# biagiom/spark-network-traffic-classifier

Measured on NVIDIA H100. Metric: flow-records/sec fit+transform, higher is better.
Workload: dtype u8 bins / uint32 histograms / f64 split scoring (f32 records)

## Files before the change

include/b200flow.h:

```cpp
#ifndef B200FLOW_H
#define B200FLOW_H

#include <stdint.h>

#ifdef __cplusplus
extern "C" {
#endif

#define B200FLOW_OK            0
#define B200FLOW_ERR_ARG      -1
#define B200FLOW_ERR_CUDA     -2
#define B200FLOW_ERR_LIMIT    -3

#define B200FLOW_F32 0
#define B200FLOW_F64 1

#define B200FLOW_SRC_F32    0
#define B200FLOW_SRC_F64    1
#define B200FLOW_SRC_I32    2
#define B200FLOW_SRC_INDEX  3
#define B200FLOW_SRC_ONEHOT 4

typedef struct b200flow_slot {
    int32_t kind;
    int32_t src_off;
    int32_t lut_off;
    int32_t lut_len;
    int32_t hot;
    int32_t reserved;
    double  mean;
    double  scale;
} b200flow_slot;

const char* b200flow_last_error(void);
int  b200flow_version(void);

int b200flow_category_counts(const void* records, int64_t n_rows, int32_t row_bytes,
                             int32_t src_off, int32_t K, int64_t* counts, void* stream);

int b200flow_category_counts_multi(const void* records, int64_t n_rows, int32_t row_bytes, int32_t n_cols,
                                   const int32_t* src_offs_host, const int32_t* Ks_host, int64_t* counts, void* stream);

int b200flow_encode(const void* records, int64_t n_rows, int32_t row_bytes,
                    const b200flow_slot* plan, int32_t n_out,
                    const int32_t* lut, int32_t lut_total,
                    int32_t label_off, int32_t label_lut_off, int32_t label_lut_len,
                    int32_t check_nan,
                    void* out, int32_t out_dtype, int32_t* label_out, uint8_t* valid_out,
                    void* stream);

int b200flow_sample_records(const void* records, int64_t n_rows, int32_t row_bytes,
                            const b200flow_slot* plan, int32_t F, const int32_t* lut, int32_t round_f32,
                            uint64_t seed, uint64_t keep_threshold, int64_t row_offset,
                            double* sample, int64_t cap, int32_t* n_sampled, void* stream);

int b200flow_encode_bins(const void* records, int64_t n_rows, int32_t row_bytes,
                         const b200flow_slot* plan, int32_t F, const int32_t* lut, int32_t lut_total,
                         int32_t label_off, int32_t label_lut_off, int32_t label_lut_len,
                         int32_t check_nan, int32_t round_f32,
                         int32_t thr_f32 ,
                         const double* thresholds, const int32_t* n_thr, const int32_t* arity, int32_t max_bins,
                         uint8_t* tp, int32_t tp_stride, int32_t* label_out, int32_t* bad, void* stream);

int b200flow_column_moments(const void* x, int32_t dtype, int64_t n_rows, int32_t D, int64_t ld,
                            const double* shift, double* sum, double* sumsq, void* stream);

int b200flow_sample_rows(const void* x, int32_t dtype, int64_t n_rows, int32_t F, int64_t ld,
                         uint64_t seed, uint64_t keep_threshold, int64_t row_offset,
                         double* sample, int64_t cap, int32_t* n_sampled, void* stream);

int b200flow_find_splits(double* sample, int64_t cap, int32_t n_s, int32_t F,
                         const int32_t* arity, int32_t max_bins,
                         double* thresholds, int32_t* n_thr,
                         const int32_t* n_s_dev ,
                         void* stream);

int b200flow_bin_rows(const void* x, int32_t dtype, int64_t n_rows, int32_t F, int64_t ld,
                      const double* thresholds, const int32_t* n_thr, const int32_t* arity,
                      int32_t max_bins, const int32_t* labels,
                      uint8_t* tp, int32_t tp_stride, int32_t* bad_rows, void* stream);

int b200flow_dedup_rows(const uint8_t* tp, int64_t n_rows, int32_t tp_stride, int32_t key_bytes,
                        int32_t* table, int32_t* minrow, int64_t table_cap, int32_t* slot_of, int32_t* rep,
                        int32_t* flag, int64_t* pos, int64_t* n_unique, int32_t* uid, uint8_t* tp_unique, void* stream);

int b200flow_bag_weights(uint64_t seed, int32_t T, int64_t row_offset, int64_t n_rows,
                         const uint32_t* poisson_cdf, const uint32_t* poisson_cdf_host,
                         const int32_t* uid, const int32_t* perm, int64_t n_unique, uint32_t* W, void* stream);

int b200flow_group_rows(const int32_t* uid, int64_t n_rows, int64_t n_unique, int32_t* gsize, int64_t* goff,
                        int32_t* cursor, int32_t* perm, int32_t* uperm, void* stream);

int b200flow_bag_count(const uint32_t* W, int32_t T, int64_t n_unique, int32_t* blk_cnt, void* stream);

int b200flow_bag_fill(const uint32_t* W, int32_t T, int64_t n_unique, const int64_t* blk_off, void* ent, void* stream);

int b200flow_exclusive_scan_i32_to_i64(const int32_t* in, int64_t n, int64_t* out,
                                       int64_t* total, void* stream);


int b200flow_feature_subsets(uint64_t seed, int32_t n_slots, const int32_t* slot_tree,
                             const uint32_t* slot_nid, int32_t F, int32_t m,
                             uint16_t* subset, void* stream);

int b200flow_hist_level(const uint8_t* tp, int32_t tp_stride, int32_t F,
                        const void* ent,
                        int32_t n_slots, const int64_t* seg_begin, const int64_t* seg_end,
                        const int64_t* chunk_off, int64_t n_chunks, int32_t chunk_rows,
                        const uint16_t* subset, int32_t m, int32_t n_bins, int32_t C,
                        uint32_t* hist, void* stream);

typedef struct b200flow_split {
    int32_t  feat;
    int32_t  kind;
    int32_t  bin_thr;
    int32_t  flags;
    double   gain;
    double   impurity;
    uint64_t mask[4];
} b200flow_split;

int b200flow_score_level(const uint32_t* hist, int32_t n_slots, const uint16_t* subset,
                         int32_t m, int32_t n_bins, int32_t C,
                         const int32_t* feat_bins, const int32_t* feat_kind,
                         int32_t level, int32_t max_depth, int32_t min_instances,
                         double min_info_gain,
                         b200flow_split* split, uint32_t* node_counts,
                         uint32_t* left_counts, uint32_t* right_counts, void* stream);

typedef struct b200flow_node {
    int32_t feat;
    int32_t kind_bin;
    int32_t left;
    uint32_t nid;
} b200flow_node;

int b200flow_grow_level(int32_t n_slots, const int32_t* slot_tree, const uint32_t* slot_nid,
                        const int32_t* slot_node, const b200flow_split* split,
                        const uint32_t* node_counts, const uint32_t* left_counts,
                        const uint32_t* right_counts, int32_t C,
                        b200flow_node* nodes, uint64_t* node_mask, uint32_t* pool_counts,
                        int32_t* node_tree, int64_t pool_capacity,
                        int32_t* next_tree, uint32_t* next_nid, int32_t* next_node,
                        int32_t* next_parent, int32_t* child_slot, int64_t* counters, void* stream);

int b200flow_partition_level(const uint8_t* tp, int32_t tp_stride,
                             const void* ent, void* ent_out,
                             int32_t n_slots, const int64_t* seg_begin, const int64_t* seg_end,
                             const int64_t* chunk_off, int64_t n_chunks, int32_t chunk_rows,
                             const b200flow_split* split, int32_t* cursors, void* stream);

int b200flow_route_hist_config(int32_t F, int32_t m, int32_t n_bins, int32_t C,
                               int32_t rec_bytes , int32_t* chunk_rows, int32_t* m_pass);
int b200flow_route_hist_level(const uint8_t* tp, int32_t tp_stride, int32_t F,
                              const int32_t* field_desc ,
                              const void* ent, void* ent_out,
                              int32_t n_slots, const int64_t* seg_begin, const int64_t* seg_end,
                              const int64_t* chunk_off, const int64_t* n_chunks_dev ,
                              int64_t n_chunks_max ,
                              int32_t chunk_rows,
                              const b200flow_split* split, const int32_t* child_slot, int32_t* cursors,
                              void* chunk_scratch ,
                              const uint16_t* subset_next, int32_t m, int32_t n_bins, int32_t C,
                              uint32_t* hist_next, int32_t flags, void* stream);

int b200flow_packed_layout(int32_t F, const int32_t* feat_bins, int32_t C, int32_t* desc, int32_t* rec_bytes);
int b200flow_pack_records(const uint8_t* tp, int32_t tp_stride, int64_t n_rows, int32_t F, const int32_t* desc,
                          int32_t rec_bytes, uint32_t* packed, void* stream);

int b200flow_plan_route(int32_t n_slots, const b200flow_split* split, const int64_t* seg_begin, const int64_t* seg_end,
                        int32_t chunk_rows, const int32_t* slot_node, double* node_gain, int32_t* n_chunks,
                        int32_t* cursors , void* stream);

int b200flow_next_segments(int32_t n_next , const int64_t* n_next_dev ,
                           const int32_t* next_parent,
                           const int64_t* seg_begin, const int64_t* seg_end,
                           const int32_t* cursors, int64_t* next_begin, int64_t* next_end,
                           void* stream);

int b200flow_finalize_forest(int64_t n_nodes, const uint32_t* pool_counts, int32_t C,
                             double* leaf_prob, void* stream);

int b200flow_predict(const uint8_t* tp, int32_t tp_stride, int64_t n_rows,
                     const b200flow_node* nodes, const uint64_t* node_mask,
                     const double* leaf_prob, const uint32_t* pool_counts,
                     int32_t T, int32_t C, int32_t dt_mode,
                     const void* top_nodes , int32_t top_levels,
                     double* raw, double* prob, double* pred, void* stream);

int b200flow_build_top_nodes(const b200flow_node* nodes, const int32_t* node_tree, int64_t n_nodes, int32_t T,
                             int32_t top_levels, void* top, void* stream);

int b200flow_gather_rows(const void* src, int32_t row_bytes, const int32_t* idx, int64_t n_rows, void* out, void* stream);

int b200flow_confusion(const double* pred, const double* label, int64_t n_rows, int32_t C,
                       int64_t* cm, void* stream);

int b200flow_predict_grid_confusion(const uint8_t* tp, int32_t tp_stride, int32_t F, int64_t n_rows, const int32_t* mult,
                                    const b200flow_node* nodes, const uint64_t* node_mask, const double* leaf_prob,
                                    const uint32_t* pool_counts, int32_t T, int32_t C, int32_t dt_mode,
                                    const void* top_nodes, int32_t top_levels, const int32_t* tree_cuts_host,
                                    int32_t n_tree_cuts, const int32_t* depth_cuts_host, int32_t n_depth_cuts,
                                    int32_t cm_side, int32_t max_depth_cuts_per_launch, int64_t* cm, void* stream);
int b200flow_predict_grid_scores(const uint8_t* tp, int32_t tp_stride, int32_t F, int64_t n_rows,
                                 const b200flow_node* nodes, const uint64_t* node_mask, const double* leaf_prob,
                                 const uint32_t* pool_counts, int32_t T, int32_t C, int32_t dt_mode,
                                 const void* top_nodes, int32_t top_levels, const int32_t* tree_cuts_host,
                                 int32_t n_tree_cuts, const int32_t* depth_cuts_host, int32_t n_depth_cuts,
                                 int32_t max_depth_cuts_per_launch, double* scores, void* stream);

int b200flow_binary_counts_scratch(int32_t S, int64_t n, int64_t* scratch_bytes);
int b200flow_binary_counts(const double* scores, int64_t score_stride, const int32_t* pos, const int32_t* neg,
                           int64_t count_stride, int32_t S, int64_t n, void* scratch, int64_t scratch_bytes,
                           double* d_score, int64_t* d_pos, int64_t* d_neg, int64_t cap, int64_t* n_distinct,
                           int64_t* n_nan, void* stream);
int b200flow_binary_curve(const double* d_score, const int64_t* d_pos, const int64_t* d_neg, int64_t cap,
                          const int64_t* n_distinct, int32_t S, int32_t num_bins, double* auc, double* c_score,
                          int64_t* c_tp, int64_t* c_fp, int64_t* c_n, double* work, void* stream);

int b200flow_kmeans_assign(const double* x, int64_t n_rows, int32_t D, int64_t ld, const double* centers, int32_t k,
                           int32_t* cluster, double* dist, void* stream);
int b200flow_group_sums_chunks(int64_t row_offset, int64_t n_rows, int64_t* n_chunks);
int b200flow_group_sums(const double* values, int64_t ld, const int32_t* ids, int64_t n_rows, int32_t W, int32_t G,
                        int64_t row_offset, double* partials, int64_t* counts, void* stream);
int b200flow_group_sums_chain(const double* partials, int64_t n_chunks, int32_t G, int32_t W, double* totals, void* stream);
int b200flow_kmeans_row_keys(uint64_t seed, int64_t row_offset, int64_t n_rows, int64_t* keys, void* stream);
int b200flow_kmeans_select(uint64_t seed, int64_t row_offset, int64_t n_rows, int32_t step, const double* cost, int32_t k,
                           double sum_cost, uint8_t* flag, void* stream);
int b200flow_silhouette_rows(const double* x, int64_t n_rows, int32_t D, int64_t ld, const double* norms, const int32_t* cluster,
                             const double* Y, const double* psi, const int64_t* N, int32_t G, double* out, void* stream);

int b200flow_mlp_config(const int32_t* layers, int32_t n_layers, int64_t* n_params, int64_t* smem_bytes);
int b200flow_mlp_loss_grad(const void* x, int32_t x_dtype, int64_t n_rows, int64_t ld, const int32_t* labels,
                           const int32_t* layers, int32_t n_layers, const double* weights, int64_t row_offset,
                           double* partials, void* stream);
int b200flow_mlp_forward(const void* x, int32_t x_dtype, int64_t n_rows, int64_t ld, const int32_t* layers, int32_t n_layers,
                         const double* weights, double* raw, void* stream);

int b200flow_random_split(uint64_t seed, int64_t row_offset, int64_t n_rows,
                          const double* cum_bounds_host, int32_t n_splits, uint8_t* split_id,
                          void* stream);

int b200flow_compact_rows(const void* rows, int64_t n_rows, int32_t row_bytes,
                          const uint8_t* flag, int32_t want, void* out_rows,
                          int64_t* scratch, int64_t* n_kept, void* stream);

#define B200FLOW_CSV_NULL   0
#define B200FLOW_CSV_INT32  1
#define B200FLOW_CSV_INT64  2
#define B200FLOW_CSV_DOUBLE 3
#define B200FLOW_CSV_STRING 4
typedef struct b200flow_csv_col {
    int32_t type;
    int32_t rec_off;
    int32_t str_index;
    int32_t reserved;
} b200flow_csv_col;

int b200flow_csv_count_lines(const uint8_t* text, int64_t n_bytes, int32_t* counts, unsigned long long* flags, void* stream);
int b200flow_csv_line_starts(const uint8_t* text, int64_t n_bytes, const int64_t* bases, int64_t* row_starts, void* stream);
int b200flow_csv_infer(const uint8_t* text, int64_t n_bytes, const int64_t* row_starts, int64_t n_rows, int32_t n_cols,
                       int32_t flags, int32_t* col_class, int32_t* col_null, unsigned long long* bad, void* stream);
int b200flow_csv_dictionary(const uint8_t* text, int64_t n_bytes, const int64_t* row_starts, int64_t n_rows, int32_t n_cols,
                            int32_t flags, const b200flow_csv_col* cols, unsigned long long* keys, long long* pos_len,
                            int32_t cap_log2, unsigned long long* bad, void* stream);
int b200flow_csv_parse(const uint8_t* text, int64_t n_bytes, const int64_t* row_starts, int64_t n_rows, int32_t n_cols,
                       int32_t flags, const b200flow_csv_col* cols, const unsigned long long* keys, const long long* pos_len,
                       const int32_t* slot_code, int32_t cap_log2, void* records, int32_t row_bytes, unsigned long long* bad,
                       void* stream);

#ifdef __cplusplus
}
#endif
#endif
```

spark-network-traffic-classifier_b200/b200flow/_lib.py:

```python
import ctypes as C
import os

import numpy as np
import torch

_HERE = os.path.dirname(os.path.abspath(__file__))
LIB_PATH = os.path.join(_HERE, "libb200flow.so")

F32, F64 = 0, 1
SRC_F32, SRC_F64, SRC_I32, SRC_INDEX, SRC_ONEHOT = 0, 1, 2, 3, 4

SLOT_DTYPE = np.dtype([("kind", "<i4"), ("src_off", "<i4"), ("lut_off", "<i4"), ("lut_len", "<i4"),
                       ("hot", "<i4"), ("reserved", "<i4"), ("mean", "<f8"), ("scale", "<f8")])
SPLIT_DTYPE = np.dtype([("feat", "<i4"), ("kind", "<i4"), ("bin_thr", "<i4"), ("flags", "<i4"),
                        ("gain", "<f8"), ("impurity", "<f8"), ("mask", "<u8", (4,))])
NODE_DTYPE = np.dtype([("feat", "<i4"), ("kind_bin", "<i4"), ("left", "<i4"), ("nid", "<u4")])
assert SLOT_DTYPE.itemsize == 40 and SPLIT_DTYPE.itemsize == 64 and NODE_DTYPE.itemsize == 16


class B200FlowError(RuntimeError):
    pass


class UnsupportedParamError(B200FlowError, ValueError):
    """a parameter value MLlib accepts but the CUDA path does not implement (entropy impurity, maxBins > 256, ...): a
    ValueError, so the pyspark shim reports it as IllegalArgumentException; CUDA/runtime failures stay B200FlowError."""


_P, _I32, _I64, _U64, _F64 = C.c_void_p, C.c_int32, C.c_int64, C.c_uint64, C.c_double

_SIGNATURES = {
    "b200flow_category_counts": [_P, _I64, _I32, _I32, _I32, _P, _P],
    "b200flow_category_counts_multi": [_P, _I64, _I32, _I32, _P, _P, _P, _P],
    "b200flow_encode": [_P, _I64, _I32, _P, _I32, _P, _I32, _I32, _I32, _I32, _I32, _P, _I32, _P, _P, _P],
    "b200flow_sample_records": [_P, _I64, _I32, _P, _I32, _P, _I32, _U64, _U64, _I64, _P, _I64, _P, _P],
    "b200flow_encode_bins": [_P, _I64, _I32, _P, _I32, _P, _I32, _I32, _I32, _I32, _I32, _I32, _I32, _P, _P, _P, _I32, _P, _I32, _P, _P, _P],
    "b200flow_column_moments": [_P, _I32, _I64, _I32, _I64, _P, _P, _P, _P],
    "b200flow_sample_rows": [_P, _I32, _I64, _I32, _I64, _U64, _U64, _I64, _P, _I64, _P, _P],
    "b200flow_find_splits": [_P, _I64, _I32, _I32, _P, _I32, _P, _P, _P, _P],
    "b200flow_bin_rows": [_P, _I32, _I64, _I32, _I64, _P, _P, _P, _I32, _P, _P, _I32, _P, _P],
    "b200flow_dedup_rows": [_P, _I64, _I32, _I32, _P, _P, _I64, _P, _P, _P, _P, _P, _P, _P, _P],
    "b200flow_bag_weights": [_U64, _I32, _I64, _I64, _P, _P, _P, _P, _I64, _P, _P],
    "b200flow_group_rows": [_P, _I64, _I64, _P, _P, _P, _P, _P, _P],
    "b200flow_bag_count": [_P, _I32, _I64, _P, _P],
    "b200flow_bag_fill": [_P, _I32, _I64, _P, _P, _P],
    "b200flow_exclusive_scan_i32_to_i64": [_P, _I64, _P, _P, _P],
    "b200flow_feature_subsets": [_U64, _I32, _P, _P, _I32, _I32, _P, _P],
    "b200flow_hist_level": [_P, _I32, _I32, _P, _I32, _P, _P, _P, _I64, _I32, _P, _I32, _I32, _I32, _P, _P],
    "b200flow_score_level": [_P, _I32, _P, _I32, _I32, _I32, _P, _P, _I32, _I32, _I32, _F64, _P, _P, _P, _P, _P],
    "b200flow_grow_level": [_I32, _P, _P, _P, _P, _P, _P, _P, _I32, _P, _P, _P, _P, _I64, _P, _P, _P, _P, _P, _P, _P],
    "b200flow_route_hist_level": [_P, _I32, _I32, _P, _P, _P, _I32, _P, _P, _P, _P, _I64, _I32, _P, _P, _P, _P, _P, _I32, _I32,
                                  _I32, _P, _I32, _P],
    "b200flow_pack_records": [_P, _I32, _I64, _I32, _P, _I32, _P, _P],
    "b200flow_partition_level": [_P, _I32, _P, _P, _I32, _P, _P, _P, _I64, _I32, _P, _P, _P],
    "b200flow_plan_route": [_I32, _P, _P, _P, _I32, _P, _P, _P, _P, _P],
    "b200flow_next_segments": [_I32, _P, _P, _P, _P, _P, _P, _P, _P],
    "b200flow_finalize_forest": [_I64, _P, _I32, _P, _P],
    "b200flow_predict": [_P, _I32, _I64, _P, _P, _P, _P, _I32, _I32, _I32, _P, _I32, _P, _P, _P, _P],
    "b200flow_build_top_nodes": [_P, _P, _I64, _I32, _I32, _P, _P],
    "b200flow_gather_rows": [_P, _I32, _P, _I64, _P, _P],
    "b200flow_confusion": [_P, _P, _I64, _I32, _P, _P],
    "b200flow_predict_grid_confusion": [_P, _I32, _I32, _I64, _P, _P, _P, _P, _P, _I32, _I32, _I32, _P, _I32, _P, _I32, _P, _I32,
                                        _I32, _I32, _P, _P],
    "b200flow_predict_grid_scores": [_P, _I32, _I32, _I64, _P, _P, _P, _P, _I32, _I32, _I32, _P, _I32, _P, _I32, _P, _I32, _I32,
                                     _P],
    "b200flow_binary_counts": [_P, _I64, _P, _P, _I64, _I32, _I64, _P, _I64, _P, _P, _P, _I64, _P, _P, _P],
    "b200flow_binary_curve": [_P, _P, _P, _I64, _P, _I32, _I32, _P, _P, _P, _P, _P, _P, _P],
    "b200flow_kmeans_assign": [_P, _I64, _I32, _I64, _P, _I32, _P, _P, _P],
    "b200flow_group_sums": [_P, _I64, _P, _I64, _I32, _I32, _I64, _P, _P, _P],
    "b200flow_group_sums_chain": [_P, _I64, _I32, _I32, _P, _P],
    "b200flow_kmeans_row_keys": [_U64, _I64, _I64, _P, _P],
    "b200flow_kmeans_select": [_U64, _I64, _I64, _I32, _P, _I32, _F64, _P, _P],
    "b200flow_silhouette_rows": [_P, _I64, _I32, _I64, _P, _P, _P, _P, _P, _I32, _P, _P],
    "b200flow_mlp_loss_grad": [_P, _I32, _I64, _I64, _P, _P, _I32, _P, _I64, _P, _P],
    "b200flow_mlp_forward": [_P, _I32, _I64, _I64, _P, _I32, _P, _P, _P],
    "b200flow_random_split": [_U64, _I64, _I64, _P, _I32, _P, _P],
    "b200flow_compact_rows": [_P, _I64, _I32, _P, _I32, _P, _P, _P, _P],
    "b200flow_csv_count_lines": [_P, _I64, _P, _P, _P],
    "b200flow_csv_line_starts": [_P, _I64, _P, _P, _P],
    "b200flow_csv_infer": [_P, _I64, _P, _I64, _I32, _I32, _P, _P, _P, _P],
    "b200flow_csv_dictionary": [_P, _I64, _P, _I64, _I32, _I32, _P, _P, _P, _I32, _P, _P],
    "b200flow_csv_parse": [_P, _I64, _P, _I64, _I32, _I32, _P, _P, _P, _P, _I32, _P, _I32, _P, _P],
}
EXPORTS = sorted(list(_SIGNATURES) + ["b200flow_last_error", "b200flow_version", "b200flow_route_hist_config",
                                       "b200flow_packed_layout", "b200flow_binary_counts_scratch",
                                       "b200flow_group_sums_chunks", "b200flow_mlp_config"])

_lib = None
launches = 0
_KERNELS_PER_CALL = {"b200flow_grow_level": 3, "b200flow_compact_rows": 3, "b200flow_route_hist_level": 2, "b200flow_dedup_rows": 5, "b200flow_group_rows": 3}


def load():
    global _lib
    if _lib is None:
        if not os.path.exists(LIB_PATH):
            raise B200FlowError("libb200flow.so is not built (%s missing): run `python -c 'import __graft_entry__ as g; "
                                "g.build()'` or `make -C spark-network-traffic-classifier_b200/csrc`. There is no CPU "
                                "fallback for the product path." % LIB_PATH)
        lib = C.CDLL(LIB_PATH)
        for name, args in _SIGNATURES.items():
            fn = getattr(lib, name)
            fn.argtypes = args
            fn.restype = C.c_int
        lib.b200flow_last_error.restype = C.c_char_p
        lib.b200flow_version.restype = C.c_int
        lib.b200flow_route_hist_config.argtypes = [_I32] * 5 + [C.POINTER(_I32), C.POINTER(_I32)]
        lib.b200flow_route_hist_config.restype = C.c_int
        lib.b200flow_packed_layout.argtypes = [_I32, _P, _I32, _P, C.POINTER(_I32)]
        lib.b200flow_packed_layout.restype = C.c_int
        lib.b200flow_binary_counts_scratch.argtypes = [_I32, _I64, C.POINTER(_I64)]
        lib.b200flow_binary_counts_scratch.restype = C.c_int
        lib.b200flow_group_sums_chunks.argtypes = [_I64, _I64, C.POINTER(_I64)]
        lib.b200flow_group_sums_chunks.restype = C.c_int
        lib.b200flow_mlp_config.argtypes = [_P, _I32, C.POINTER(_I64), C.POINTER(_I64)]
        lib.b200flow_mlp_config.restype = C.c_int
        _lib = lib
    return _lib


def route_hist_config(F, m, n_bins, n_classes, rec_bytes=0):
    ch, mp = _I32(0), _I32(0)
    ok = load().b200flow_route_hist_config(int(F), int(m), int(n_bins), int(n_classes), int(rec_bytes), C.byref(ch), C.byref(mp))
    return (int(ch.value), int(mp.value)) if ok else None


def packed_layout(feat_bins, n_classes):
    fb = np.ascontiguousarray(feat_bins, dtype=np.int32)
    desc = np.zeros(fb.shape[0] + 1, np.int32)
    rb = _I32(0)
    lib = load()
    if lib.b200flow_packed_layout(int(fb.shape[0]), fb.ctypes.data, int(n_classes), desc.ctypes.data, C.byref(rb)) != 0:
        raise B200FlowError("b200flow_packed_layout failed: %s" % lib.b200flow_last_error().decode())
    return desc, int(rb.value)


def binary_counts_scratch(S, n):
    out = _I64(0)
    lib = load()
    if lib.b200flow_binary_counts_scratch(int(S), int(n), C.byref(out)) != 0:
        raise B200FlowError("b200flow_binary_counts_scratch failed: %s" % lib.b200flow_last_error().decode())
    return int(out.value)


def group_sums_chunks(row_offset, n_rows):
    out = _I64(0)
    lib = load()
    if lib.b200flow_group_sums_chunks(int(row_offset), int(n_rows), C.byref(out)) != 0:
        raise B200FlowError("b200flow_group_sums_chunks failed: %s" % lib.b200flow_last_error().decode())
    return int(out.value)


def mlp_config(layers):
    la = np.ascontiguousarray(layers, dtype=np.int32)
    P, sm = _I64(0), _I64(0)
    lib = load()
    if lib.b200flow_mlp_config(la.ctypes.data, int(la.shape[0]), C.byref(P), C.byref(sm)) != 0:
        raise UnsupportedParamError("layers %s: %s" % (list(map(int, la)), lib.b200flow_last_error().decode()))
    return int(P.value), int(sm.value)


def ptr(t):
    if t is None:
        return None
    if not t.is_cuda:
        raise B200FlowError("b200flow kernels need CUDA tensors (got %s); there is no CPU fallback" % t.device)
    if not t.is_contiguous():
        raise B200FlowError("b200flow kernels need contiguous tensors")
    return t.data_ptr()


def stream():
    return torch.cuda.current_stream().cuda_stream


def call(name, *args):
    global launches
    lib = load()
    rc = getattr(lib, name)(*args, stream())
    launches += _KERNELS_PER_CALL.get(name, 1)
    if rc != 0:
        raise B200FlowError("%s failed (%d): %s" % (name, rc, lib.b200flow_last_error().decode()))


def h2d(a, device):
    t = torch.from_numpy(np.ascontiguousarray(a))
    if torch.device(device).type != "cuda":
        return t.clone()
    return t.pin_memory().to(device, non_blocking=True)


def require_cuda():
    if not torch.cuda.is_available():
        raise B200FlowError("no CUDA device: the b200flow product path has no CPU fallback")
    load()


def dtype_code(t):
    if t.dtype == torch.float32:
        return F32
    if t.dtype == torch.float64:
        return F64
    raise B200FlowError("dense matrices must be float32 or float64, got %s" % t.dtype)
```

spark-network-traffic-classifier_b200/b200flow/forest.py:

```python
import math
from dataclasses import dataclass

import numpy as np
import torch

from . import _lib
from ._lib import NODE_DTYPE, SPLIT_DTYPE, B200FlowError, UnsupportedParamError, call, ptr

import os as _os
CHUNK_ROWS = 2048
FUSED = True
TOP_LEVELS = int(_os.environ.get("B200FLOW_TOP_LEVELS", "8"))
DEDUP = True
_PIN = True
PROFILE = None


def _timed(name, fn, *args):
    if PROFILE is None:
        return call(fn, *args)
    e0, e1 = torch.cuda.Event(enable_timing=True), torch.cuda.Event(enable_timing=True)
    e0.record()
    call(fn, *args)
    e1.record()
    PROFILE.setdefault(name, []).append((e0, e1))


def profile_totals():
    torch.cuda.synchronize()
    return {k: (len(v), sum(a.elapsed_time(b) for a, b in v)) for k, v in (PROFILE or {}).items()
            if not k.startswith("_")}


ENTRY_BOUND_BYTES = 8 << 30
HIST_BUDGET_BYTES = int(_os.environ.get("B200FLOW_HIST_BUDGET_GB", "10")) << 30
RS_MIN_BYTES = int(_os.environ.get("B200FLOW_RS_MIN_BYTES", str(8 << 20)))
RS_CHUNKS = int(_os.environ.get("B200FLOW_RS_CHUNKS", "1"))


@dataclass
class ForestParams:
    num_trees: int = 20
    max_depth: int = 5
    max_bins: int = 32
    min_instances_per_node: int = 1
    min_info_gain: float = 0.0
    feature_subset_strategy: str = "auto"
    subsampling_rate: float = 1.0
    impurity: str = "gini"
    seed: int = 0
    bootstrap: bool = True


def tp_stride(F):
    return (F + 1 + 63) // 64 * 64


def poisson_cdf_table(rate=1.0):
    out = np.empty(32, np.uint32)
    term = math.exp(-rate); cdf = 0.0
    for k in range(32):
        cdf += term
        out[k] = min(int(math.floor(cdf * 4294967296.0)), 0xFFFFFFFF)
        term = term * rate / (k + 1)
    if out[30] != 0xFFFFFFFF:
        raise UnsupportedParamError("subsamplingRate %.3f too large: bag weights must stay below 31" % rate)
    return out


def build_metadata(n_rows, F, num_classes, arity, max_bins, num_trees, strategy="auto"):
    arity = np.asarray(arity, np.int32)
    mpb = int(min(max_bins, n_rows))
    if mpb > 256:
        raise UnsupportedParamError("maxBins > 256 is not supported (bins are stored as uint8)")
    if arity.size and int(arity.max()) > mpb:
        raise ValueError("DecisionTree requires maxBins (= %d) to be at least as large as the number of values in each "
                         "categorical feature, but a categorical feature has %d values. Consider removing this and other "
                         "categorical features with a large number of values, or add more training examples."
                         % (mpb, int(arity.max())))
    if arity.size and int(arity.max()) > 255:
        raise UnsupportedParamError("a categorical feature with %d categories is not supported: bins are stored as uint8, and "
                                    "with 256 categories no bin is left for a value unseen at fit time (at most 255)"
                                    % int(arity.max()))
    kind = np.zeros(F, np.int32)
    U = int(math.floor(math.log(mpb // 2 + 1) / math.log(2.0) + 1)) if num_classes > 2 else 0
    for f in range(F):
        if arity[f] > 1:
            kind[f] = 2 if (num_classes > 2 and arity[f] <= U) else 1
        elif arity[f] == 1:
            kind[f] = 1
    s = str(strategy)
    if s == "auto":
        s = "all" if num_trees == 1 else "sqrt"
    if s == "all": m = F
    elif s == "sqrt": m = int(math.ceil(math.sqrt(F)))
    elif s == "log2": m = max(1, int(math.ceil(math.log(F) / math.log(2))))
    elif s == "onethird": m = int(math.ceil(F / 3.0))
    else:
        try:
            v = float(s)
        except ValueError:
            raise ValueError("Supported featureSubsetStrategy values: auto, all, onethird, sqrt, log2, (0.0-1.0], [1-n]; got %r" % strategy)
        m = int(v) if ("." not in s and v >= 1) else int(math.ceil(v * F))
    return mpb, kind, max(1, min(m, F))


def pack_records(tp, F, field_desc, rec_bytes):
    packed = torch.empty((max(tp.shape[0], 1), rec_bytes), dtype=torch.uint8, device=tp.device)
    call("b200flow_pack_records", ptr(tp), tp.shape[1], tp.shape[0], F, ptr(field_desc), rec_bytes, ptr(packed))
    return packed


def dedup_rows(tp, key_bytes, sync=True):
    n, stride = tp.shape
    dev = tp.device
    cap_tab = 1
    while cap_tab < 2 * n:
        cap_tab <<= 1
    table = torch.empty(cap_tab, dtype=torch.int32, device=dev); minrow = torch.empty(cap_tab, dtype=torch.int32, device=dev)
    slot_of = torch.empty(n, dtype=torch.int32, device=dev); rep = torch.empty(n, dtype=torch.int32, device=dev)
    flag = torch.empty(n, dtype=torch.int32, device=dev); pos = torch.empty(n + 1, dtype=torch.int64, device=dev)
    uid = torch.empty(n, dtype=torch.int32, device=dev); total = torch.zeros(1, dtype=torch.int64, device=dev)
    tpu = torch.empty_like(tp)
    _timed("dedup_rows", "b200flow_dedup_rows", ptr(tp), n, stride, key_bytes, ptr(table), ptr(minrow), cap_tab, ptr(slot_of), ptr(rep),
           ptr(flag), ptr(pos), ptr(total), ptr(uid), ptr(tpu))
    if not sync:
        return tpu, uid, total
    U = int(total.item())
    return tpu[:U], uid, U


def _i32(a, dev):
    return _lib.h2d(np.ascontiguousarray(a, np.int32), dev)


class InvalidRowsError(ValueError):
    """NaN / null numeric cells or unseen dictionary codes met while assembling rows (VectorAssembler / StringIndexerModel
    handleInvalid="error"); raised when the fused record path meets them — Spark raises at the same point: the action."""


class _DenseSource:

    def __init__(self, x, labels=None):
        self.x, self.labels = x, (labels.to(torch.int32).contiguous() if labels is not None else None)
        self.n, self.F = x.shape
        self.device = x.device

    def sample(self, seed, keep, row_offset, sample, cap, n_s_dev):
        call("b200flow_sample_rows", ptr(self.x), _lib.dtype_code(self.x), self.n, self.F, self.x.stride(0), seed, keep, int(row_offset),
             ptr(sample), cap, ptr(n_s_dev))

    def bin(self, thresholds, n_thr, arity_dev, mpb, bad, want_label_out=False):
        stride = tp_stride(self.F)
        tp = torch.empty((self.n, stride), dtype=torch.uint8, device=self.device)
        _timed("bin_rows", "b200flow_bin_rows", ptr(self.x), _lib.dtype_code(self.x), self.n, self.F, self.x.stride(0), ptr(thresholds), ptr(n_thr),
               ptr(arity_dev), mpb, ptr(self.labels), ptr(tp), stride, ptr(bad[0:1]))
        return tp, self.labels


class _RecordSource:

    def __init__(self, rec, plan, round_f32=False, with_label=True):
        if rec.dtype != torch.uint8 or rec.dim() != 2 or rec.shape[1] != plan.schema.row_bytes:
            raise ValueError("records must be uint8 [n, %d]" % plan.schema.row_bytes)
        self.rec, self.plan, self.round_f32 = rec, plan, 1 if round_f32 else 0
        self.n, self.F = rec.shape[0], plan.n_out
        self.device = rec.device
        self.with_label = with_label and plan.label is not None

    def _thr_f32(self, arity_dev):
        if self.round_f32:
            return 1
        return 1 if all(s[0] in (_lib.SRC_F32, _lib.SRC_INDEX, _lib.SRC_ONEHOT) and s[5] == 0.0 and s[6] == 1.0 for s in self.plan.slots) else 0

    def sample(self, seed, keep, row_offset, sample, cap, n_s_dev):
        _, slots, lut_t, _ = self.plan._device_tables(self.device)
        call("b200flow_sample_records", ptr(self.rec), self.n, self.plan.schema.row_bytes, ptr(slots), self.F, ptr(lut_t), self.round_f32,
             seed, keep, int(row_offset), ptr(sample), cap, ptr(n_s_dev))

    def bin(self, thresholds, n_thr, arity_dev, mpb, bad, want_label_out=False):
        _, slots, lut_t, lut_total = self.plan._device_tables(self.device)
        stride = tp_stride(self.F)
        tp = torch.empty((self.n, stride), dtype=torch.uint8, device=self.device)
        loff, llo, lln = self.plan.label if self.with_label else (-1, 0, 0)
        lab = torch.empty(self.n, dtype=torch.int32, device=self.device) if (want_label_out and self.with_label) else None
        _timed("encode_bins", "b200flow_encode_bins", ptr(self.rec), self.n, self.plan.schema.row_bytes, ptr(slots), self.F, ptr(lut_t), lut_total,
               loff, llo, lln, int(self.plan.check_nan), self.round_f32, self._thr_f32(arity_dev), ptr(thresholds), ptr(n_thr), ptr(arity_dev), mpb, ptr(tp), stride,
               ptr(lab), ptr(bad))
        return tp, lab


class ForestModel:

    def __init__(self, T, C, F, arity, max_bins, thresholds, n_thr, nodes, node_mask, pool_counts, node_tree,
                 leaf_prob, node_gain, n_nodes, dt_mode):
        self.T, self.C, self.F, self.max_bins, self.dt_mode = T, C, F, max_bins, dt_mode
        self.arity = np.asarray(arity, np.int32)
        self.thresholds, self.n_thr = thresholds, n_thr
        self.nodes, self.node_mask, self.pool_counts = nodes, node_mask, pool_counts
        self.node_tree, self.leaf_prob, self.node_gain, self.n_nodes = node_tree, leaf_prob, node_gain, n_nodes
        self._arity_dev = _i32(self.arity, thresholds.device)

    def bin(self, x, labels=None):
        n, F = x.shape
        if F != self.F:
            raise ValueError("expected %d features, got %d" % (self.F, F))
        bad = torch.zeros(2, dtype=torch.int32, device=x.device)
        tp, _ = _DenseSource(x, labels).bin(self.thresholds, self.n_thr, self._arity_dev, self.max_bins, bad)
        return tp, bad[0:1]

    def _top_table(self):
        if TOP_LEVELS <= 0:
            return None, 0
        if getattr(self, "_top", None) is None:
            self._top = torch.zeros((self.T << TOP_LEVELS, 4), dtype=torch.int32, device=self.nodes.device)
            call("b200flow_build_top_nodes", ptr(self.nodes), ptr(self.node_tree), self.n_nodes, self.T, TOP_LEVELS, ptr(self._top))
        return self._top, TOP_LEVELS

    def predict_binned(self, tp, want_raw=True, want_prob=True):
        n = tp.shape[0]
        dev = tp.device
        raw = torch.empty((n, self.C), dtype=torch.float64, device=dev) if want_raw else None
        prob = torch.empty((n, self.C), dtype=torch.float64, device=dev) if want_prob else None
        pred = torch.empty(n, dtype=torch.float64, device=dev)
        top, K = self._top_table()
        _timed("predict", "b200flow_predict", ptr(tp), tp.shape[1], n, ptr(self.nodes), ptr(self.node_mask), ptr(self.leaf_prob),
             ptr(self.pool_counts), self.T, self.C, 1 if self.dt_mode else 0, ptr(top), K, ptr(raw), ptr(prob), ptr(pred))
        return raw, prob, pred

    def predict(self, x, want_raw=True, want_prob=True):
        tp, _ = self.bin(x)
        return self._predict_tp(tp, want_raw, want_prob)

    def predict_records(self, rec, plan, want_raw=True, want_prob=True, round_f32=False, want_label=False, on_invalid="ignore"):
        src = _RecordSource(rec, plan, round_f32, with_label=want_label)
        if src.F != self.F:
            raise ValueError("expected %d features, got %d" % (self.F, src.F))
        bad = torch.zeros(2, dtype=torch.int32, device=rec.device)
        tp, lab = src.bin(self.thresholds, self.n_thr, self._arity_dev, self.max_bins, bad, want_label_out=want_label)
        out = self._predict_tp(tp, want_raw, want_prob, bad if on_invalid == "error" else None)
        return out + (lab,)

    def _predict_tp(self, tp, want_raw=True, want_prob=True, bad=None):
        n = tp.shape[0]
        if not DEDUP or n == 0:
            if bad is not None and int(bad[1].item()):
                raise InvalidRowsError("%d NaN/null cells or unseen labels in the rows to transform" % int(bad[1].item()))
            return self.predict_binned(tp, want_raw, want_prob)
        tpu, uid, u_dev = dedup_rows(tp, self.F, sync=False)
        head = (torch.cat([u_dev, bad.to(torch.int64)]) if bad is not None else u_dev).cpu()
        if bad is not None and int(head[2]):
            raise InvalidRowsError("%d NaN/null cells or unseen labels in the rows to transform" % int(head[2]))
        U = int(head[0])
        raw_u, prob_u, pred_u = self.predict_binned(tpu[:U], want_raw, want_prob)

        def spread(src, width):
            if src is None:
                return None
            out = torch.empty((n, width) if width > 1 else (n,), dtype=torch.float64, device=tp.device)
            call("b200flow_gather_rows", ptr(src), 8 * width, ptr(uid), n, ptr(out))
            return out
        return spread(raw_u, self.C), spread(prob_u, self.C), spread(pred_u, 1)

    def grid_confusion(self, x_or_records, tree_cuts, depth_cuts, labels=None, plan=None, round_f32=False, cm_side=None,
                       group=None, max_depth_cuts_per_launch=0):
        from . import dist as bdist
        tree_cuts = np.ascontiguousarray(sorted(set(int(t) for t in tree_cuts)), np.int32)
        depth_cuts = np.ascontiguousarray(sorted(set(int(d) for d in depth_cuts)), np.int32)
        if plan is None:
            if labels is None:
                raise ValueError("grid_confusion: the dense path needs the labels")
            src = _DenseSource(x_or_records, labels)
        else:
            if plan.label is None:
                raise ValueError("grid_confusion: the encode plan has no label column (EncodePlan.set_label)")
            src = _RecordSource(x_or_records, plan, round_f32)
        if src.F != self.F:
            raise ValueError("expected %d features, got %d" % (self.F, src.F))
        S = max(self.C, int(cm_side or 0))
        dev = src.device
        cm = torch.zeros((len(tree_cuts), len(depth_cuts), S, S), dtype=torch.int64, device=dev)
        n = src.n
        if n > 0:
            bad = torch.zeros(2, dtype=torch.int32, device=dev)
            tp, _ = src.bin(self.thresholds, self.n_thr, self._arity_dev, self.max_bins, bad)
            tpu, uid, U = dedup_rows(tp, self.F + 1)
            gsize = torch.empty(U, dtype=torch.int32, device=dev); cursor = torch.empty(U, dtype=torch.int32, device=dev)
            goff = torch.empty(U + 1, dtype=torch.int64, device=dev)
            perm = torch.empty(n, dtype=torch.int32, device=dev); uperm = torch.empty(n, dtype=torch.int32, device=dev)
            _timed("group_rows", "b200flow_group_rows", ptr(uid), n, U, ptr(gsize), ptr(goff), ptr(cursor), ptr(perm), ptr(uperm))
            top, K = self._top_table()
            _timed("predict_grid", "b200flow_predict_grid_confusion", ptr(tpu), tpu.shape[1], self.F, U, ptr(gsize), ptr(self.nodes),
                   ptr(self.node_mask), ptr(self.leaf_prob), ptr(self.pool_counts), self.T, self.C, 1 if self.dt_mode else 0,
                   ptr(top), K, tree_cuts.ctypes.data, len(tree_cuts), depth_cuts.ctypes.data, len(depth_cuts), S,
                   int(max_depth_cuts_per_launch), ptr(cm))
        return bdist.all_reduce_sum_(cm, group).cpu()

    GRID_SCORE_BUDGET = 2 << 30

    def grid_binary_metrics(self, x_or_records, tree_cuts, depth_cuts, labels=None, plan=None, num_bins=1000, group=None,
                            round_f32=False, max_depth_cuts_per_launch=0):
        from . import dist as bdist
        from .metrics import binary_metrics
        if self.C < 2:
            raise ValueError("grid_binary_metrics: the score is rawPrediction[1], the forest has %d class(es)" % self.C)
        tree_cuts = np.ascontiguousarray(sorted(set(int(t) for t in tree_cuts)), np.int32)
        depth_cuts = np.ascontiguousarray(sorted(set(int(d) for d in depth_cuts)), np.int32)
        if plan is None:
            if labels is None:
                raise ValueError("grid_binary_metrics: the dense path needs the labels")
            src = _DenseSource(x_or_records, labels)
        else:
            if plan.label is None:
                raise ValueError("grid_binary_metrics: the encode plan has no label column (EncodePlan.set_label)")
            src = _RecordSource(x_or_records, plan, round_f32)
        if src.F != self.F:
            raise ValueError("expected %d features, got %d" % (self.F, src.F))
        dev = src.device
        I, J = len(tree_cuts), len(depth_cuts)
        U = 0
        if src.n > 0:
            bad = torch.zeros(2, dtype=torch.int32, device=dev)
            tp, _ = src.bin(self.thresholds, self.n_thr, self._arity_dev, self.max_bins, bad)
            tpu, uid, U = dedup_rows(tp, self.F + 1)
            tpu = tpu.contiguous()
            gsize = torch.empty(U, dtype=torch.int32, device=dev); cursor = torch.empty(U, dtype=torch.int32, device=dev)
            goff = torch.empty(U + 1, dtype=torch.int64, device=dev)
            perm = torch.empty(src.n, dtype=torch.int32, device=dev); uperm = torch.empty(src.n, dtype=torch.int32, device=dev)
            _timed("group_rows", "b200flow_group_rows", ptr(uid), src.n, U, ptr(gsize), ptr(goff), ptr(cursor), ptr(perm), ptr(uperm))
            positive = tpu[:, self.F] >= 1
            pos = torch.where(positive, gsize, 0).contiguous()
            neg = torch.where(positive, 0, gsize).contiguous()
        else:
            pos = neg = torch.zeros(0, dtype=torch.int32, device=dev)
        mx = torch.tensor([U], dtype=torch.int64, device=dev)
        grp = group if group is not None else bdist.group()
        if grp is not None:
            import torch.distributed as dist
            bdist.all_reduce_(mx, grp, op=dist.ReduceOp.MAX)
        per_cut = J * max(int(mx.item()), 1) * 8
        step = max(1, min(I, self.GRID_SCORE_BUDGET // per_cut))
        out = np.empty((I, J, 2), np.float64)
        top, K = self._top_table()
        for i0 in range(0, I, step):
            cuts = np.ascontiguousarray(tree_cuts[i0:i0 + step])
            scores = torch.empty((len(cuts), J, U), dtype=torch.float64, device=dev)
            if U > 0:
                _timed("predict_grid", "b200flow_predict_grid_scores", ptr(tpu), tpu.shape[1], self.F, U, ptr(self.nodes),
                       ptr(self.node_mask), ptr(self.leaf_prob), ptr(self.pool_counts), self.T, self.C, 1 if self.dt_mode else 0,
                       ptr(top), K, cuts.ctypes.data, len(cuts), depth_cuts.ctypes.data, J, int(max_depth_cuts_per_launch),
                       ptr(scores))
            r = binary_metrics(scores.reshape(len(cuts) * J, U), pos=pos, neg=neg, num_bins=num_bins, group=grp)
            out[i0:i0 + len(cuts), :, 0] = np.asarray(r["areaUnderROC"]).reshape(len(cuts), J)
            out[i0:i0 + len(cuts), :, 1] = np.asarray(r["areaUnderPR"]).reshape(len(cuts), J)
        return out

    def export(self):
        n = self.n_nodes
        nodes = self.nodes[:n].cpu().numpy().view(NODE_DTYPE).reshape(-1)
        tree = self.node_tree[:n].cpu().numpy()
        counts = self.pool_counts[:n].cpu().numpy().view(np.uint32).astype(np.int64)
        mask = (self.node_mask[:n].cpu().numpy().view(np.uint64) if self.node_mask is not None
                else np.zeros((n, 4), np.uint64))
        gain = self.node_gain[:n].cpu().numpy()
        order = np.lexsort((nodes["nid"], tree))
        is_leaf = (nodes["feat"] < 0).astype(np.int32)
        kind = np.where(is_leaf == 1, 0, nodes["kind_bin"] >> 16).astype(np.int32)
        bin_thr = np.where(is_leaf == 1, 0, nodes["kind_bin"] & 0xffff).astype(np.int32)
        mask = np.where(is_leaf[:, None] == 1, 0, mask).astype(np.uint64)
        return dict(tree=tree[order], nid=nodes["nid"][order], feat=nodes["feat"][order], kind=kind[order],
                    bin_thr=bin_thr[order], is_leaf=is_leaf[order], gain=gain[order], mask=mask[order],
                    counts=counts[order])

    def feature_importances(self):
        ex = self.export()
        imp = np.zeros(self.F)
        for t in range(self.T):
            sel = (ex["tree"] == t) & (ex["is_leaf"] == 0)
            v = np.zeros(self.F)
            np.add.at(v, ex["feat"][sel], ex["gain"][sel] * ex["counts"][sel].sum(1))
            if v.sum() > 0:
                imp += v / v.sum()
        return imp / imp.sum() if imp.sum() > 0 else imp


def _gather_sample(sample, n_s, cap, F, group):
    import torch.distributed as dist
    world = dist.get_world_size(group)
    from . import dist as bdist
    counts = [int(c.item()) for c in bdist.all_gather_list(torch.tensor([n_s], dtype=torch.int64, device=sample.device), group)]
    mx = max(max(counts), 1)
    mine = torch.zeros((F, mx), dtype=torch.float64, device=sample.device)
    if n_s > 0:
        mine[:, :n_s] = sample.view(F, cap)[:, :n_s]
    parts = bdist.all_gather_list(mine, group)
    tot = sum(counts)
    new_cap = 1
    while new_cap < max(tot, 2):
        new_cap <<= 1
    out = torch.empty((F, new_cap), dtype=torch.float64, device=sample.device)
    pos = 0
    for p, c in zip(parts, counts):
        out[:, pos:pos + c] = p[:, :c]; pos += c
    return out.view(-1), tot, new_cap


def fit_forest(x, labels, num_classes, arity, params, row_offset=0, group=None):
    return _fit(_DenseSource(x, labels), num_classes, arity, params, row_offset, group)


def fit_forest_records(rec, plan, num_classes, arity, params, row_offset=0, group=None, round_f32=False):
    if plan.label is None:
        raise ValueError("fit_forest_records: the encode plan has no label column (EncodePlan.set_label)")
    return _fit(_RecordSource(rec, plan, round_f32), num_classes, arity, params, row_offset, group)


def _fit(src, num_classes, arity, params, row_offset=0, group=None):
    import torch.distributed as dist
    from . import dist as bdist
    _lib.require_cuda()
    p = params
    if p.impurity != "gini":
        raise UnsupportedParamError("impurity=%r: only 'gini' is implemented on the CUDA path" % p.impurity)
    if not (0 <= p.max_depth <= 30):
        raise ValueError("maxDepth must be in [0, 30], got %d" % p.max_depth)
    dev = src.device
    n, F = src.n, src.F
    C = int(num_classes)
    if not (1 <= C <= 256):
        raise ValueError("numClasses must be in [1, 256] (labels are stored as one byte), got %d" % C)
    T = int(p.num_trees)
    seed = int(p.seed) & 0xFFFFFFFFFFFFFFFF
    n_global = n
    if group is not None:
        t = torch.tensor([n], dtype=torch.int64, device=dev)
        bdist.all_reduce_(t, group)
        n_global = int(t.item())
    mpb, kind, m = build_metadata(n_global, F, C, arity, p.max_bins, T, p.feature_subset_strategy)
    arity = np.asarray(arity, np.int32)
    arity_dev = _i32(arity, dev)

    has_cont = bool((arity == 0).any())
    frac = min(1.0, max(mpb * mpb, 10000) / float(max(n_global, 1))) if has_cont else 1.0
    keep = int(frac * 4294967296.0)
    expect = n if frac >= 1.0 else int(n * frac + 6.0 * math.sqrt(max(n * frac, 1.0)) + 64)
    cap = 1
    while cap < max(min(expect, n), 2):
        cap <<= 1
    sample = torch.empty(F * cap, dtype=torch.float64, device=dev)
    n_s_dev = torch.zeros(1, dtype=torch.int32, device=dev)
    thresholds = torch.zeros((F, mpb - 1), dtype=torch.float64, device=dev)
    n_thr = torch.zeros(F, dtype=torch.int32, device=dev)
    if has_cont:
        src.sample(seed, keep, row_offset, sample, cap, n_s_dev)
        if group is not None:
            n_s = int(n_s_dev.item())
            if n_s > cap:
                raise B200FlowError("findSplits sample overflow (%d > %d)" % (n_s, cap))
            sample, n_s, cap = _gather_sample(sample, n_s, cap, F, group)
            call("b200flow_find_splits", ptr(sample), cap, n_s, F, ptr(arity_dev), mpb, ptr(thresholds), ptr(n_thr), None)
        else:
            call("b200flow_find_splits", ptr(sample), cap, cap, F, ptr(arity_dev), mpb, ptr(thresholds), ptr(n_thr), ptr(n_s_dev))
    del sample

    stride = tp_stride(F)
    bad = torch.zeros(2, dtype=torch.int32, device=dev)
    tp, _ = src.bin(thresholds, n_thr, arity_dev, mpb, bad)
    feat_bins = torch.where(arity_dev > 0, arity_dev, n_thr + 1).to(torch.int32).contiguous()
    feat_kind = _i32(kind, dev)
    total = torch.zeros(1, dtype=torch.int64, device=dev)
    dedup = n > 0 and DEDUP
    if dedup:
        tp, uid, u_dev = dedup_rows(tp, F + 1, sync=False)
    else:
        uid, u_dev = None, torch.full((1,), n, dtype=torch.int64, device=dev)
    bagging = p.bootstrap and T > 1
    cdf_host = np.ascontiguousarray(poisson_cdf_table(p.subsampling_rate)) if bagging else None
    cdf = _lib.h2d(cdf_host.view(np.int32), dev) if bagging else None
    cap_nodes = max(4096, 4 * T, min(T << (min(p.max_depth, 18) + 1), 1 << 20))
    nodes = torch.zeros((cap_nodes, 16), dtype=torch.uint8, device=dev)
    use_mask = bool((kind > 0).any())
    node_mask = torch.zeros((cap_nodes, 4), dtype=torch.int64, device=dev) if use_mask else None
    pool_counts = torch.zeros((cap_nodes, C), dtype=torch.int32, device=dev)
    node_tree = torch.zeros(cap_nodes, dtype=torch.int32, device=dev)
    node_gain = torch.zeros(cap_nodes, dtype=torch.float64, device=dev)
    root = np.zeros(T, NODE_DTYPE); root["feat"] = -1; root["left"] = -1; root["nid"] = 1
    nodes[:T] = _lib.h2d(root.view(np.uint8).reshape(T, 16), dev)
    node_tree[:T] = torch.arange(T, dtype=torch.int32, device=dev)
    pool_size = T

    def grow_pool(need):
        nonlocal nodes, node_mask, pool_counts, node_tree, node_gain, cap_nodes
        if need <= cap_nodes:
            return
        new_cap = cap_nodes
        while new_cap < need:
            new_cap *= 2
        def ext(t, shape_tail):
            nt = torch.zeros((new_cap,) + shape_tail, dtype=t.dtype, device=dev)
            nt[:cap_nodes] = t
            return nt
        nodes = ext(nodes, (16,)); pool_counts = ext(pool_counts, (C,)); node_tree = ext(node_tree, ())
        node_gain = ext(node_gain, ())
        if node_mask is not None:
            node_mask = ext(node_mask, (4,))
        cap_nodes = new_cap

    head = torch.cat([bad.to(torch.int64), feat_bins.max().reshape(1).to(torch.int64), n_s_dev.to(torch.int64), u_dev,
                      feat_bins.to(torch.int64)]).cpu()
    if int(head[1]) != 0:
        raise InvalidRowsError("%d NaN/null cells or unseen labels in the training rows" % int(head[1]))
    if int(head[0]) != 0:
        raise ValueError("categorical feature value outside [0, arity) or non-integral in %d cells" % int(head[0]))
    if has_cont and group is None and int(head[3]) > cap:
        raise B200FlowError("findSplits sample overflow (%d > %d)" % (int(head[3]), cap))
    n_bins, U = int(head[2]), int(head[4])
    if dedup:
        tp = tp[:U]
    if tp.shape[0] == 0:
        tp = torch.zeros((1, stride), dtype=torch.uint8, device=dev)
    desc_host, rec_bytes = _lib.packed_layout(head[5:5 + F].numpy(), C) if FUSED else (None, 0)
    cfg = _lib.route_hist_config(F, m, n_bins, C, rec_bytes) if FUSED else None
    fused = cfg is not None
    route_ch, m_pass = cfg if fused else (CHUNK_ROWS, m)
    route_passes = -(-m // m_pass)
    hsz = m * n_bins * C
    rec_tp, rec_stride, field_desc = tp, stride, None
    if fused and rec_bytes:
        field_desc = _lib.h2d(desc_host, dev)
        rec_tp, rec_stride = pack_records(tp, F, field_desc, rec_bytes), rec_bytes
    nb = (U + 1023) // 1024
    W = torch.zeros(max(T * U, 1), dtype=torch.int32, device=dev)
    if n > 0:
        perm = uperm = None
        if uid is not None and bagging and U < n:
            gsize = torch.empty(U, dtype=torch.int32, device=dev); cursor = torch.empty(U, dtype=torch.int32, device=dev)
            goff = torch.empty(U + 1, dtype=torch.int64, device=dev)
            perm = torch.empty(n, dtype=torch.int32, device=dev); uperm = torch.empty(n, dtype=torch.int32, device=dev)
            _timed("group_rows", "b200flow_group_rows", ptr(uid), n, U, ptr(gsize), ptr(goff), ptr(cursor), ptr(perm), ptr(uperm))
        _timed("bag_weights", "b200flow_bag_weights", seed, T, int(row_offset), n, ptr(cdf),
               cdf_host.ctypes.data if bagging else None, ptr(uperm if perm is not None else uid), ptr(perm), U, ptr(W))
    blk_cnt = torch.zeros(max(T * nb, 1), dtype=torch.int32, device=dev)
    blk_off = torch.zeros(T * nb + 1, dtype=torch.int64, device=dev)
    if U > 0:
        call("b200flow_bag_count", ptr(W), T, U, ptr(blk_cnt))
    call("b200flow_exclusive_scan_i32_to_i64", ptr(blk_cnt), T * nb, ptr(blk_off), ptr(total))
    e_dev = total.clone()
    E = T * U if T * U * 16 <= ENTRY_BOUND_BYTES else int(total.item())
    ent = torch.empty((max(E, 1), 2), dtype=torch.int32, device=dev)
    ent2 = torch.empty_like(ent)
    if U > 0:
        call("b200flow_bag_fill", ptr(W), T, U, ptr(blk_off), ptr(ent))
    del W, uid

    slot_tree = torch.arange(T, dtype=torch.int32, device=dev)
    slot_nid = torch.ones(T, dtype=torch.int32, device=dev)
    slot_node = torch.arange(T, dtype=torch.int32, device=dev)
    idx = torch.arange(T, dtype=torch.int64, device=dev) * nb
    seg_begin = blk_off[idx].contiguous()
    seg_end = blk_off[idx + nb].contiguous()
    n_slots = T
    level = 0
    per_slot_hist = m * n_bins * C * 4
    group_slots = max(1, HIST_BUDGET_BYTES // per_slot_hist)
    stats = dict(levels=0, slots=0, entries=0, hist_launches=0, rows=n, unique_rows=U)

    stats["route_chunk"], stats["route_passes"] = route_ch if fused else 0, route_passes if fused else 0
    stats["record_format"], stats["record_bytes"] = ("packed", rec_bytes) if field_desc is not None else ("bytes", stride)

    def chunk_table(nch):
        off = torch.empty(nch.shape[0] + 1, dtype=torch.int64, device=dev)
        call("b200flow_exclusive_scan_i32_to_i64", ptr(nch), nch.shape[0], ptr(off), ptr(total))
        return off, int(total.item())

    def level_subsets(ns, s_tree, s_nid):
        sub = torch.empty((ns, m), dtype=torch.int16, device=dev)
        call("b200flow_feature_subsets", seed, ns, ptr(s_tree), ptr(s_nid), F, m, ptr(sub))
        return sub

    def plan_route(ns, split_, begin_, end_, total_out, s_node=None, gain_out=None, cursors_=None):
        nch = torch.empty(ns, dtype=torch.int32, device=dev)
        call("b200flow_plan_route", ns, ptr(split_), ptr(begin_), ptr(end_), route_ch, ptr(s_node), ptr(gain_out), ptr(nch), ptr(cursors_))
        roff = torch.empty(ns + 1, dtype=torch.int64, device=dev)
        call("b200flow_exclusive_scan_i32_to_i64", ptr(nch), ns, ptr(roff), ptr(total_out))
        if PROFILE is not None:
            PROFILE.setdefault("_route_entries", []).append(torch.where(nch > 0, end_ - begin_, torch.zeros_like(end_)).sum())
        return roff

    route_chunks_max = E // route_ch + 1

    world = dist.get_world_size(group) if group is not None else 1
    rank = dist.get_rank(group) if group is not None else 0
    REC = 64 + 12 * C
    use_rs = world > 1 and bdist.is_nccl(group)

    def score_sharded(h_full, gs, sub, lvl, split_, nc_, lc_, rc_):
        K = int(max(1, min(RS_CHUNKS, gs, (gs * hsz * 4) // max(RS_MIN_BYTES, 1))))
        bounds = [gs * i // K for i in range(K + 1)]
        ev0 = None
        if PROFILE is not None:
            ev0 = torch.cuda.Event(enable_timing=True); ev0.record()
        jobs = []
        for k in range(K):
            s0, g = bounds[k], bounds[k + 1] - bounds[k]
            per = -(-g // world)
            mine = torch.empty(per * hsz, dtype=torch.int32, device=dev)
            w = dist.reduce_scatter_tensor(mine, h_full[s0 * hsz:(s0 + world * per) * hsz], group=group, async_op=True)
            jobs.append((s0, g, per, mine, w))
        gathers = []
        for s0, g, per, mine, w in jobs:
            w.wait()
            lo = rank * per
            cnt = max(0, min(per, g - lo))
            local = torch.empty(per * REC, dtype=torch.uint8, device=dev)
            sec = [local[:per * 64], local[per * 64:per * (64 + 4 * C)], local[per * (64 + 4 * C):per * (64 + 8 * C)], local[per * (64 + 8 * C):]]
            if cnt > 0:
                _timed("score_level", "b200flow_score_level", ptr(mine), cnt, ptr(sub[s0 + lo:s0 + lo + cnt]), m, n_bins, C, ptr(feat_bins),
                       ptr(feat_kind), lvl, p.max_depth, int(p.min_instances_per_node), float(p.min_info_gain), ptr(sec[0]), ptr(sec[1]),
                       ptr(sec[2]), ptr(sec[3]))
            gathered = torch.empty((world, per * REC), dtype=torch.uint8, device=dev)
            gw = dist.all_gather_into_tensor(gathered, local, group=group, async_op=True)
            gathers.append((s0, per, gathered, gw))
        for s0, per, gathered, gw in gathers:
            gw.wait()
            o = 0
            for dst, width in ((split_, 64), (nc_.view(torch.uint8), 4 * C), (lc_.view(torch.uint8), 4 * C), (rc_.view(torch.uint8), 4 * C)):
                dst.view(-1)[s0 * width:(s0 + world * per) * width].view(world, per * width).copy_(gathered[:, o:o + per * width])
                o += per * width
        if ev0 is not None:
            ev1 = torch.cuda.Event(enable_timing=True); ev1.record()
            PROFILE.setdefault("level_exchange", []).append((ev0, ev1))

    def run_route(roff, rch_dev, n_parents, split_, child_slot_, cursors_, next_subset_, n_next_cap, route=True):
        hist_next = torch.zeros((n_next_cap + world - 1) * hsz, dtype=torch.int32, device=dev)
        cmax = route_chunks_max + n_parents
        scratch = torch.empty(cmax * 4, dtype=torch.int32, device=dev)
        _timed("route_hist_level", "b200flow_route_hist_level", ptr(rec_tp), rec_stride, F, ptr(field_desc), ptr(ent), ptr(ent2), n_parents,
               ptr(seg_begin), ptr(seg_end), ptr(roff), ptr(rch_dev), cmax, route_ch, ptr(split_), ptr(child_slot_), ptr(cursors_),
               ptr(scratch), ptr(next_subset_), m, n_bins, C, ptr(hist_next), 1 if route else 0)
        _lib.launches += route_passes - 1
        stats["hist_launches"] += route_passes
        return hist_next

    side_stream = torch.cuda.Stream(device=dev)
    host_cnt = torch.empty(5, dtype=torch.int64).pin_memory() if _PIN else None
    subset = level_subsets(n_slots, slot_tree, slot_nid)
    hist_ready = None
    counters = None
    if fused and n_slots * hsz * 4 <= HIST_BUDGET_BYTES:
        pseudo = np.zeros(T, SPLIT_DTYPE); pseudo["bin_thr"] = 255; pseudo["flags"] = 4
        pseudo_t = _lib.h2d(pseudo.view(np.uint8).reshape(T, 64), dev)
        child0 = torch.stack([torch.arange(T, dtype=torch.int32, device=dev),
                              torch.full((T,), -1, dtype=torch.int32, device=dev)], 1).contiguous().view(-1)
        cursors0 = torch.zeros(2 * T, dtype=torch.int32, device=dev)
        roff0 = plan_route(T, pseudo_t, seg_begin, seg_end, total)
        hist_full = run_route(roff0, total, T, pseudo_t, child0, cursors0, subset, T, route=False)
        hist_ready = hist_full[:T * hsz]
    while n_slots > 0:
        grow_pool(pool_size + 2 * n_slots)
        lens = (seg_end - seg_begin) if hist_ready is None else None
        n_alloc = n_slots + world - 1
        split = torch.empty((n_alloc, 64), dtype=torch.uint8, device=dev)
        node_counts = torch.empty((n_alloc, C), dtype=torch.int32, device=dev)
        left_counts = torch.empty((n_alloc, C), dtype=torch.int32, device=dev)
        right_counts = torch.empty((n_alloc, C), dtype=torch.int32, device=dev)
        chunk_off = None
        if hist_ready is None:
            nch = ((lens + (CHUNK_ROWS - 1)) // CHUNK_ROWS).to(torch.int32).contiguous()
            chunk_off, n_chunks = chunk_table(nch)
        groups = [(0, n_slots)] if hist_ready is not None else \
            [(g0, min(n_slots, g0 + group_slots)) for g0 in range(0, n_slots, group_slots)]
        for g0, g1 in groups:
            gs = g1 - g0
            if hist_ready is not None:
                h = hist_ready
            else:
                h = torch.zeros(gs * hsz, dtype=torch.int32, device=dev)
                if g0 == 0 and g1 == n_slots:
                    coff, gch = chunk_off, n_chunks
                else:
                    coff = (chunk_off[g0:g1 + 1] - chunk_off[g0]).contiguous()
                    gch = int((chunk_off[g1] - chunk_off[g0]).item())
                _timed("hist_level", "b200flow_hist_level", ptr(tp), stride, F, ptr(ent), gs,
                       ptr(seg_begin[g0:g1]), ptr(seg_end[g0:g1]), ptr(coff), gch, CHUNK_ROWS, ptr(subset[g0:g1]), m, n_bins, C, ptr(h))
                stats["hist_launches"] += 1
                if PROFILE is not None:
                    PROFILE.setdefault("_hist_entries", []).append(lens[g0:g1].sum())
            if use_rs and hist_ready is not None and gs * hsz * 4 >= RS_MIN_BYTES:
                score_sharded(hist_full, gs, subset, level, split, node_counts, left_counts, right_counts)
                del h
                continue
            if group is not None:
                if PROFILE is not None:
                    ev0 = torch.cuda.Event(enable_timing=True); ev0.record()
                bdist.all_reduce_(h, group)
                if PROFILE is not None:
                    ev1 = torch.cuda.Event(enable_timing=True); ev1.record()
                    PROFILE.setdefault("level_exchange", []).append((ev0, ev1))
            _timed("score_level", "b200flow_score_level", ptr(h), gs, ptr(subset[g0:g1]), m, n_bins, C, ptr(feat_bins), ptr(feat_kind),
                   level, p.max_depth, int(p.min_instances_per_node), float(p.min_info_gain), ptr(split[g0:g1]),
                   ptr(node_counts[g0:g1]), ptr(left_counts[g0:g1]), ptr(right_counts[g0:g1]))
            del h
        split, node_counts, left_counts, right_counts = split[:n_slots], node_counts[:n_slots], left_counts[:n_slots], right_counts[:n_slots]
        hist_ready = None
        nblk = (n_slots + 255) // 256
        if counters is None or counters.numel() < 8 + nblk + 1:
            fresh = torch.zeros(8 + 2 * nblk + 1024, dtype=torch.int64, device=dev)
            if counters is None:
                fresh[0:1].fill_(pool_size)
            else:
                fresh[:8] = counters[:8]
            counters = fresh
        next_tree = torch.empty(2 * n_slots, dtype=torch.int32, device=dev)
        next_nid = torch.empty(2 * n_slots, dtype=torch.int32, device=dev)
        next_node = torch.empty(2 * n_slots, dtype=torch.int32, device=dev)
        next_parent = torch.empty(2 * n_slots, dtype=torch.int32, device=dev)
        child_slot = torch.empty(2 * n_slots, dtype=torch.int32, device=dev)
        _timed("grow_level", "b200flow_grow_level", n_slots, ptr(slot_tree), ptr(slot_nid), ptr(slot_node), ptr(split), ptr(node_counts),
               ptr(left_counts), ptr(right_counts), C, ptr(nodes), ptr(node_mask), ptr(pool_counts), ptr(node_tree),
               cap_nodes, ptr(next_tree), ptr(next_nid), ptr(next_node), ptr(next_parent), ptr(child_slot), ptr(counters))
        n_cap = 2 * n_slots
        speculative = fused and n_cap * hsz * 4 <= HIST_BUDGET_BYTES and level + 1 < p.max_depth
        if not speculative:
            node_gain[slot_node.long()] = split.view(torch.float64)[:, 2]
        if speculative:
            cursors = torch.empty(2 * n_slots, dtype=torch.int32, device=dev)
            roff = plan_route(n_slots, split, seg_begin, seg_end, counters[4:5], slot_node, node_gain, cursors)
            ev_planned = torch.cuda.Event(); ev_planned.record()
            with torch.cuda.stream(side_stream):
                side_stream.wait_event(ev_planned)
                cnt = counters[:5].to("cpu", non_blocking=True) if host_cnt is None else host_cnt.copy_(counters[:5], non_blocking=True)
                ev_read = torch.cuda.Event(); ev_read.record(side_stream)
            next_subset = level_subsets(n_cap, next_tree, next_nid)
            hist_next = run_route(roff, counters[4:5], n_slots, split, child_slot, cursors, next_subset, n_cap,
                                  route=level + 2 < p.max_depth)
            next_begin = torch.empty(n_cap, dtype=torch.int64, device=dev)
            next_end = torch.empty(n_cap, dtype=torch.int64, device=dev)
            call("b200flow_next_segments", n_cap, ptr(counters[1:2]), ptr(next_parent), ptr(seg_begin), ptr(seg_end), ptr(cursors),
                 ptr(next_begin), ptr(next_end))
            ev_read.synchronize()
        else:
            cnt = counters[:5].cpu()
        if int(cnt[2]) != 0:
            raise B200FlowError("node pool overflow (capacity %d)" % cap_nodes)
        pool_size, n_next = int(cnt[0]), int(cnt[1])
        stats["levels"] += 1; stats["slots"] += n_slots
        if n_next == 0:
            break
        next_tree, next_nid, next_node = next_tree[:n_next], next_nid[:n_next], next_node[:n_next]
        if speculative:
            hist_ready = hist_next[:n_next * hsz]
            hist_full = hist_next
            next_subset, next_begin, next_end = next_subset[:n_next], next_begin[:n_next], next_end[:n_next]
        else:
            next_subset = level_subsets(n_next, next_tree, next_nid)
            cursors = torch.zeros(2 * n_slots, dtype=torch.int32, device=dev)
            if chunk_off is None:
                lens = seg_end - seg_begin
                nch = ((lens + (CHUNK_ROWS - 1)) // CHUNK_ROWS).to(torch.int32).contiguous()
                chunk_off, n_chunks = chunk_table(nch)
            _timed("partition_level", "b200flow_partition_level", ptr(tp), stride, ptr(ent), ptr(ent2),
                   n_slots, ptr(seg_begin), ptr(seg_end), ptr(chunk_off), n_chunks, CHUNK_ROWS, ptr(split), ptr(cursors))
            next_begin = torch.empty(n_next, dtype=torch.int64, device=dev)
            next_end = torch.empty(n_next, dtype=torch.int64, device=dev)
            call("b200flow_next_segments", n_next, None, ptr(next_parent), ptr(seg_begin), ptr(seg_end), ptr(cursors),
                 ptr(next_begin), ptr(next_end))
        ent, ent2 = ent2, ent
        slot_tree, slot_nid, slot_node, subset = next_tree, next_nid, next_node, next_subset
        seg_begin, seg_end = next_begin, next_end
        n_slots = n_next
        level += 1

    leaf_prob = torch.empty((pool_size, C), dtype=torch.float64, device=dev)
    call("b200flow_finalize_forest", pool_size, ptr(pool_counts), C, ptr(leaf_prob))
    stats["entries"] = int(e_dev.item())
    model = ForestModel(T, C, F, arity, mpb, thresholds, n_thr, nodes, node_mask, pool_counts, node_tree, leaf_prob,
                        node_gain, pool_size, dt_mode=(T == 1 and not p.bootstrap))
    model.train_stats = stats
    model.feat_kind, model.feat_bins, model.n_bins, model.m = kind, feat_bins, n_bins, m
    return model


def confusion_matrix(pred, label, C):
    cm = torch.zeros((C, C), dtype=torch.int64, device=pred.device)
    call("b200flow_confusion", ptr(pred.contiguous()), ptr(label.contiguous()), pred.shape[0], C, ptr(cm))
    return cm


def metrics_from_confusion(cm, metric_label=0.0, beta=1.0):
    cm = np.asarray(cm, np.float64)
    N = cm.sum()
    sup = cm.sum(1); predl = cm.sum(0); tp = np.diag(cm)
    labs = sup > 0
    with np.errstate(divide="ignore", invalid="ignore"):
        p = np.where(predl > 0, tp / predl, 0.0)
        r = np.where(sup > 0, tp / sup, 0.0)
        f1 = np.where(p + r > 0, 2 * p * r / (p + r), 0.0)
        b2 = beta * beta
        fb = np.where(p + r > 0, (1 + b2) * p * r / (b2 * p + r), 0.0)
        fpr = (predl - tp) / (N - sup)
    w = sup / N if N else sup
    out = dict(accuracy=float(tp[labs].sum() / N) if N else 0.0,
               weightedPrecision=float((p * w)[labs].sum()), weightedRecall=float((r * w)[labs].sum()),
               f1=float((f1 * w)[labs].sum()), macroF1=float(f1[labs].mean()) if labs.any() else 0.0)
    out.update(weightedTruePositiveRate=out["weightedRecall"], weightedFalsePositiveRate=float((fpr * w)[labs].sum()),
               weightedFMeasure=float((fb * w)[labs].sum()),
               hammingLoss=float((N - tp.sum()) / N) if N else 0.0)
    ml = float(metric_label)
    li = int(ml) if np.isfinite(ml) and ml == int(ml) else -1
    if 0 <= li < cm.shape[0] and labs[li]:
        out.update(truePositiveRateByLabel=float(r[li]), falsePositiveRateByLabel=float(fpr[li]), precisionByLabel=float(p[li]),
                   recallByLabel=float(r[li]), fMeasureByLabel=float(fb[li]))
    return out
```

spark-network-traffic-classifier_b200/csrc/forest.cu:

```cuda
#include <float.h>
#include <stdlib.h>
#include <string.h>

#include "common.cuh"

namespace b200flow {

constexpr int kMaxSubset = 128;

__global__ void __launch_bounds__(128) feature_subsets_kernel(uint64_t seed, int n_slots, const int32_t* __restrict__ slot_tree,
                                                              const uint32_t* __restrict__ slot_nid, int F, int m,
                                                              uint16_t* subset) {
    int s = blockIdx.x * blockDim.x + threadIdx.x;
    if (s >= n_slots) return;
    uint16_t* out = subset + (int64_t)s * m;
    if (m >= F) { for (int i = 0; i < F; ++i) out[i] = (uint16_t)i; return; }
    uint16_t pos[kMaxSubset], val[kMaxSubset], pick[kMaxSubset];
    int nt = 0;
    const int tree = slot_tree[s]; const uint32_t nid = slot_nid[s];
    uint4 r = make_uint4(0, 0, 0, 0);
    for (int i = 0; i < m; ++i) {
        if ((i & 3) == 0) r = philox_keyed(seed, PURPOSE_FEAT, (uint32_t)tree, nid, (uint32_t)(i >> 2), 0u);
        uint32_t w = (i & 3) == 0 ? r.x : (i & 3) == 1 ? r.y : (i & 3) == 2 ? r.z : r.w;
        int j = i + (int)(w % (uint32_t)(F - i));
        int vi = i, vj = j, ki = -1, kj = -1;
        for (int k = 0; k < nt; ++k) { if (pos[k] == i) { vi = val[k]; ki = k; } if (pos[k] == j) { vj = val[k]; kj = k; } }
        pick[i] = (uint16_t)vj;
        if (j != i) {
            if (kj >= 0) val[kj] = (uint16_t)vi; else { pos[nt] = (uint16_t)j; val[nt] = (uint16_t)vi; ++nt; }
        }
        (void)ki;
    }
    for (int i = 1; i < m; ++i) {
        uint16_t x = pick[i]; int k = i - 1;
        while (k >= 0 && pick[k] > x) { pick[k + 1] = pick[k]; --k; }
        pick[k + 1] = x;
    }
    for (int i = 0; i < m; ++i) out[i] = pick[i];
}

__device__ __forceinline__ int find_slot(const int64_t* __restrict__ chunk_off, int n_slots, int64_t c) {
    int lo = 0, hi = n_slots;
    while (hi - lo > 1) { int mid = (lo + hi) >> 1; if (__ldg(chunk_off + mid) <= c) lo = mid; else hi = mid; }
    return lo;
}

__global__ void __launch_bounds__(256) hist_level_kernel(const uint8_t* __restrict__ tp, int stride, int F,
                                                         const b2f_entry* __restrict__ ent, int n_slots, const int64_t* __restrict__ seg_begin,
                                                         const int64_t* __restrict__ seg_end, const int64_t* __restrict__ chunk_off,
                                                         int chunk_rows, const uint16_t* __restrict__ subset, int m, int n_bins,
                                                         int C, int m_pass, uint32_t* hist) {
    extern __shared__ uint32_t sh_hist[];
    __shared__ int sh_feat[256];
    const int64_t c = blockIdx.x;
    const int s = find_slot(chunk_off, n_slots, c);
    const int64_t b = seg_begin[s] + (c - chunk_off[s]) * chunk_rows;
    const int64_t e = min(seg_end[s], b + chunk_rows);
    const int nbC = n_bins * C;
    for (int j = threadIdx.x; j < m; j += blockDim.x) sh_feat[j] = subset[(int64_t)s * m + j];
    uint32_t* gh = hist + (int64_t)s * m * nbC;
    for (int j0 = 0; j0 < m; j0 += m_pass) {
        const int mp = min(m_pass, m - j0);
        const int hsz = mp * nbC;
        __syncthreads();
        for (int i = threadIdx.x; i < hsz; i += blockDim.x) sh_hist[i] = 0;
        __syncthreads();
        for (int64_t i = b + threadIdx.x; i < e; i += blockDim.x) {
            const b2f_entry en = ent[i];
            const uint32_t w = en.y;
            const uint8_t* rec = tp + (int64_t)en.x * stride;
            const int lab = rec[F];
            for (int j = 0; j < mp; ++j) {
                const int bin = rec[sh_feat[j0 + j]];
                atomicAdd(&sh_hist[j * nbC + bin * C + lab], w);
            }
        }
        __syncthreads();
        for (int i = threadIdx.x; i < hsz; i += blockDim.x) {
            uint32_t v = sh_hist[i];
            if (v) atomicAdd(gh + (int64_t)j0 * nbC + i, v);
        }
    }
}

__device__ __forceinline__ double div_rn(double a, double b, double y) {
    const double q = __dmul_rn(a, y);
    return __fma_rn(__fma_rn(-b, q, a), y, q);
}

__device__ __forceinline__ double gini_u32(const uint32_t* c, int C, double tot) {
    if (tot == 0.0) return 0.0;
    const double y = __drcp_rn(tot);
    double imp = 1.0;
    for (int k = 0; k < C; ++k) { double f = div_rn((double)c[k], tot, y); imp -= f * f; }
    return imp;
}

__device__ __forceinline__ double split_gain(const uint32_t* L, const uint32_t* tot, int C, double parent_imp,
                                             int min_inst, double min_gain) {
    double lc = 0.0, rc = 0.0;
    for (int k = 0; k < C; ++k) { lc += (double)L[k]; rc += (double)(tot[k] - L[k]); }
    if (lc < (double)min_inst || rc < (double)min_inst) return -DBL_MAX;
    const double t = lc + rc;
    double gl = 1.0, gr = 1.0;
    if (lc == 0.0) gl = 0.0; else { const double y = __drcp_rn(lc); for (int k = 0; k < C; ++k) { double f = div_rn((double)L[k], lc, y); gl -= f * f; } }
    if (rc == 0.0) gr = 0.0; else { const double y = __drcp_rn(rc); for (int k = 0; k < C; ++k) { double f = div_rn((double)(tot[k] - L[k]), rc, y); gr -= f * f; } }
    const double yt = __drcp_rn(t);
    const double lw = div_rn(lc, t, yt), rw = div_rn(rc, t, yt);
    const double gain = parent_imp - lw * gl - rw * gr;
    if (gain < min_gain) return -DBL_MAX;
    return gain;
}

constexpr int kScoreThreads = 128;

__global__ void __launch_bounds__(kScoreThreads) score_level_kernel(
    const uint32_t* __restrict__ hist, int n_slots, const uint16_t* __restrict__ subset, int m, int n_bins, int C,
    const int32_t* __restrict__ feat_bins, const int32_t* __restrict__ feat_kind, int level, int max_depth, int min_inst,
    double min_gain, int batch, b200flow_split* split, uint32_t* node_counts, uint32_t* left_counts, uint32_t* right_counts) {
    extern __shared__ __align__(8) uint8_t sm_raw[];
    const int s = blockIdx.x;
    const int tid = threadIdx.x, w = warp_id(), lane = lane_id(), nw = kScoreThreads / 32;
    const int nbC = n_bins * C;
    uint32_t* tot = (uint32_t*)sm_raw;
    uint32_t* bestL = tot + C;
    const size_t per_warp = ((size_t)n_bins * 8 + (size_t)nbC * 4 + 7) & ~(size_t)7;
    uint8_t* wbase = (uint8_t*)(bestL + C);
    double* cen = (double*)(wbase + per_warp * w);
    uint32_t* raw = (uint32_t*)(cen + n_bins);
    uint32_t* cum_all = (uint32_t*)(wbase + per_warp * nw);
    int* order_all = (int*)(cum_all + (size_t)batch * nbC);
    uint8_t* cand_all = (uint8_t*)(order_all + (size_t)batch * n_bins);
    __shared__ int sh_ncand[64], sh_kind[64], sh_nb[64];
    __shared__ double sh_wg[kScoreThreads / 32];
    __shared__ int sh_wj[kScoreThreads / 32], sh_ws[kScoreThreads / 32];
    __shared__ double sh_best_gain; __shared__ int sh_best_j, sh_best_s, sh_best_kind;
    __shared__ unsigned long long sh_best_mask[4];

    const uint32_t* h0 = hist + (int64_t)s * m * nbC;
    if (tid == 0) { sh_best_gain = -DBL_MAX; sh_best_j = -1; sh_best_s = -1; sh_best_kind = 0; }
    double parent_imp = 0.0;

    for (int j0 = 0; j0 < m; j0 += batch) {
        const int nb_feats = min(batch, m - j0);
        {
            const uint32_t* src = h0 + (int64_t)j0 * nbC;
            const int nwords = nb_feats * nbC;
            for (int i = tid; i < nwords; i += kScoreThreads) cum_all[i] = __ldg(src + i);
        }
        __syncthreads();
        for (int jj = w; jj < nb_feats; jj += nw) {
            const int f = subset[(int64_t)s * m + j0 + jj];
            const int nb = feat_bins[f], kind = feat_kind[f];
            uint32_t* cum = cum_all + (size_t)jj * nbC;
            int* order = order_all + (size_t)jj * n_bins;
            if (lane == 0) { sh_kind[jj] = kind; sh_nb[jj] = nb; }
            if (kind == 1) {
                for (int i = lane; i < nb * C; i += 32) raw[i] = cum[i];
                __syncwarp();
                for (int c = lane; c < nb; c += 32) {
                    double cnt = 0.0;
                    for (int k = 0; k < C; ++k) cnt += (double)raw[c * C + k];
                    cen[c] = cnt == 0.0 ? DBL_MAX : (C > 2 ? gini_u32(raw + c * C, C, cnt) : (double)raw[c * C + 1]);
                }
                __syncwarp();
                for (int c = lane; c < nb; c += 32) {
                    const double ce = cen[c]; int rk = 0;
                    for (int c2 = 0; c2 < nb; ++c2) { const double o = cen[c2]; rk += (o < ce || (o == ce && c2 < c)) ? 1 : 0; }
                    order[rk] = c;
                }
                __syncwarp();
                for (int k = lane; k < C; k += 32) { uint32_t a = 0; for (int i = 0; i < nb; ++i) { a += raw[order[i] * C + k]; cum[i * C + k] = a; } }
            } else if (kind == 0) {
                if (C <= 16) {
                    const int nseg = 32 / C, seg_len = (nb + nseg - 1) / nseg;
                    const int k = lane % C, seg = lane / C;
                    const bool act = seg < nseg;
                    const int b0 = min(nb, seg * seg_len), b1 = act ? min(nb, b0 + seg_len) : b0;
                    uint32_t a = 0;
                    for (int b = b0; b < b1; ++b) a += cum[b * C + k];
                    uint32_t run = 0;
                    for (int s2 = 0; s2 < nseg; ++s2) { const uint32_t v = __shfl_sync(0xffffffffu, a, s2 * C + k); if (s2 < seg) run += v; }
                    for (int b = b0; b < b1; ++b) { run += cum[b * C + k]; cum[b * C + k] = run; }
                } else {
                    for (int k = lane; k < C; k += 32) { uint32_t a = 0; for (int b = 0; b < nb; ++b) { a += cum[b * C + k]; cum[b * C + k] = a; } }
                }
            }
            __syncwarp();
            if (j0 == 0 && jj == 0) {
                for (int k = lane; k < C; k += 32) {
                    uint32_t a;
                    if (kind == 2) { a = 0; for (int c = 0; c < nb; ++c) a += cum[c * C + k]; }
                    else a = cum[(nb - 1) * C + k];
                    tot[k] = a;
                }
            }
            uint8_t* cand = cand_all + (size_t)jj * n_bins;
            const int ns = kind == 2 ? (1 << (nb - 1)) - 1 : nb - 1;
            int n_cand = 0;
            for (int sp0 = 0; sp0 < ns; sp0 += 32) {
                const int sp = sp0 + lane;
                bool keep = sp < ns;
                if (keep && kind != 2 && sp > 0) {
                    keep = false;
                    for (int k = 0; k < C; ++k) keep |= cum[sp * C + k] != cum[(sp - 1) * C + k];
                }
                const uint32_t mk = __ballot_sync(0xffffffffu, keep);
                if (keep) cand[n_cand + __popc(mk & ((1u << lane) - 1u))] = (uint8_t)sp;
                n_cand += __popc(mk);
            }
            if (lane == 0) sh_ncand[jj] = n_cand;
        }
        __syncthreads();
        if (j0 == 0) {
            double pi = 0.0;
            if (lane == 0) { double ptot = 0.0; for (int k = 0; k < C; ++k) ptot += (double)tot[k]; pi = gini_u32(tot, C, ptot); }
            parent_imp = __shfl_sync(0xffffffffu, pi, 0);
        }
        int n_items = 0;
        for (int jj = 0; jj < nb_feats; ++jj) n_items += sh_ncand[jj];
        double tbest = -DBL_MAX; int tj = -1, ts = -1;
        for (int it = tid; it < n_items; it += kScoreThreads) {
            int jj = 0, o = 0;
            while (it >= o + sh_ncand[jj]) { o += sh_ncand[jj]; ++jj; }
            const int sp = cand_all[(size_t)jj * n_bins + (it - o)];
            const uint32_t* cum = cum_all + (size_t)jj * nbC;
            double g;
            if (sh_kind[jj] != 2) {
                g = split_gain(cum + sp * C, tot, C, parent_imp, min_inst, min_gain);
            } else {
                const unsigned bits = (unsigned)(sp + 1); const int nb = sh_nb[jj];
                double lc = 0.0, rc = 0.0;
                for (int k = 0; k < C; ++k) { uint32_t a = 0; for (int c = 0; c < nb; ++c) if ((bits >> c) & 1u) a += cum[c * C + k]; lc += (double)a; rc += (double)(tot[k] - a); }
                if (lc < (double)min_inst || rc < (double)min_inst) g = -DBL_MAX;
                else {
                    const double t = lc + rc; double gl = 1.0, gr = 1.0;
                    if (lc == 0.0) gl = 0.0; else { const double y = __drcp_rn(lc); for (int k = 0; k < C; ++k) { uint32_t a = 0; for (int c = 0; c < nb; ++c) if ((bits >> c) & 1u) a += cum[c * C + k]; const double fq = div_rn((double)a, lc, y); gl -= fq * fq; } }
                    if (rc == 0.0) gr = 0.0; else { const double y = __drcp_rn(rc); for (int k = 0; k < C; ++k) { uint32_t a = 0; for (int c = 0; c < nb; ++c) if ((bits >> c) & 1u) a += cum[c * C + k]; const double fq = div_rn((double)(tot[k] - a), rc, y); gr -= fq * fq; } }
                    const double yt = __drcp_rn(t);
                    const double lw = div_rn(lc, t, yt), rw = div_rn(rc, t, yt);
                    g = parent_imp - lw * gl - rw * gr;
                    if (g < min_gain) g = -DBL_MAX;
                }
            }
            if (g > tbest) { tbest = g; tj = j0 + jj; ts = sp; }
        }
        double g = tbest; int bj = tj, bs = ts;
#pragma unroll
        for (int o = 16; o > 0; o >>= 1) {
            const double og = __shfl_xor_sync(0xffffffffu, g, o); const int oj = __shfl_xor_sync(0xffffffffu, bj, o), os = __shfl_xor_sync(0xffffffffu, bs, o);
            if (oj >= 0 && (bj < 0 || og > g || (og == g && (oj < bj || (oj == bj && os < bs))))) { g = og; bj = oj; bs = os; }
        }
        if (lane == 0) { sh_wg[w] = g; sh_wj[w] = bj; sh_ws[w] = bs; }
        __syncthreads();
        if (tid == 0) {
            double bg = sh_best_gain; int gj = sh_best_j, gs = sh_best_s; bool improved = false;
            for (int q = 0; q < nw; ++q) {
                if (sh_wj[q] < 0) continue;
                if (sh_wg[q] > bg) { bg = sh_wg[q]; gj = sh_wj[q]; gs = sh_ws[q]; improved = true; }
                else if (improved && sh_wg[q] == bg && (sh_wj[q] < gj || (sh_wj[q] == gj && sh_ws[q] < gs))) { gj = sh_wj[q]; gs = sh_ws[q]; }
            }
            if (improved) {
                sh_best_gain = bg; sh_best_j = gj; sh_best_s = gs;
                const int jj = gj - j0; const int kind = sh_kind[jj], nb = sh_nb[jj];
                const uint32_t* cum = cum_all + (size_t)jj * nbC;
                sh_best_kind = kind;
                unsigned long long mk[4] = {0, 0, 0, 0};
                if (kind == 2) {
                    const unsigned bits = (unsigned)(gs + 1);
                    for (int k = 0; k < C; ++k) { uint32_t a = 0; for (int c = 0; c < nb; ++c) if ((bits >> c) & 1u) a += cum[c * C + k]; bestL[k] = a; }
                    mk[0] = bits;
                } else {
                    for (int k = 0; k < C; ++k) bestL[k] = cum[gs * C + k];
                    if (kind == 1) { const int* order = order_all + (size_t)jj * n_bins; for (int i = 0; i <= gs; ++i) { const int c = order[i]; mk[c >> 6] |= 1ull << (c & 63); } }
                }
                for (int q = 0; q < 4; ++q) sh_best_mask[q] = mk[q];
            }
        }
        __syncthreads();
    }
    const bool has = sh_best_j >= 0;
    for (int k = tid; k < C; k += kScoreThreads) {
        node_counts[(int64_t)s * C + k] = tot[k];
        const uint32_t l = has ? bestL[k] : 0u;
        left_counts[(int64_t)s * C + k] = l;
        right_counts[(int64_t)s * C + k] = has ? tot[k] - l : 0u;
    }
    if (tid == 0) {
        b200flow_split o;
        const double bg = sh_best_gain;
        o.gain = has ? bg : -DBL_MAX; o.impurity = parent_imp;
        const bool leaf = !(has && bg > 0.0) || level >= max_depth;
        int flags = leaf ? 1 : 0;
        o.feat = -1; o.kind = 0; o.bin_thr = 0;
        o.mask[0] = o.mask[1] = o.mask[2] = o.mask[3] = 0;
        if (!leaf) {
            o.feat = subset[(int64_t)s * m + sh_best_j]; o.kind = sh_best_kind == 0 ? 0 : 1; o.bin_thr = sh_best_s;
            for (int q = 0; q < 4; ++q) o.mask[q] = sh_best_mask[q];
            double lc = 0.0, rc = 0.0, gl = 1.0, gr = 1.0;
            for (int k = 0; k < C; ++k) { lc += (double)bestL[k]; rc += (double)(tot[k] - bestL[k]); }
            if (lc == 0.0) gl = 0.0; else for (int k = 0; k < C; ++k) { const double fq = (double)bestL[k] / lc; gl -= fq * fq; }
            if (rc == 0.0) gr = 0.0; else for (int k = 0; k < C; ++k) { const double fq = (double)(tot[k] - bestL[k]) / rc; gr -= fq * fq; }
            if (level + 1 == max_depth || gl == 0.0) flags |= 2;
            if (level + 1 == max_depth || gr == 0.0) flags |= 4;
        }
        o.flags = flags;
        split[s] = o;
    }
}

constexpr int kGrowBlock = 256;

__device__ __forceinline__ void grow_flags(const b200flow_split* __restrict__ split, int s, int n_slots, int* is_split, int* n_next) {
    int fl = s < n_slots ? split[s].flags : 1;
    *is_split = (fl & 1) ? 0 : 1;
    *n_next = (fl & 1) ? 0 : ((fl & 2) ? 0 : 1) + ((fl & 4) ? 0 : 1);
}

__global__ void __launch_bounds__(kGrowBlock) grow_count_kernel(int n_slots, const b200flow_split* __restrict__ split, int32_t* blk) {
    __shared__ int sh[2];
    if (threadIdx.x < 2) sh[threadIdx.x] = 0;
    __syncthreads();
    int is, nn; grow_flags(split, blockIdx.x * kGrowBlock + threadIdx.x, n_slots, &is, &nn);
    is = warp_sum(is); nn = warp_sum(nn);
    if (lane_id() == 0) { if (is) atomicAdd(&sh[0], is); if (nn) atomicAdd(&sh[1], nn); }
    __syncthreads();
    if (threadIdx.x < 2) blk[2 * blockIdx.x + threadIdx.x] = sh[threadIdx.x];
}

__global__ void __launch_bounds__(1024) grow_scan_kernel(int n_blocks, int32_t* blk, int64_t* counters, int64_t pool_capacity) {
    __shared__ int sh[33];
    __shared__ int carry[2];
    if (threadIdx.x < 2) carry[threadIdx.x] = 0;
    __syncthreads();
    for (int base = 0; base < n_blocks; base += 1024) {
        int i = base + threadIdx.x;
        int a = i < n_blocks ? blk[2 * i] : 0, b = i < n_blocks ? blk[2 * i + 1] : 0;
        int ta, tb;
        int ea = block_exclusive_scan(a, sh, &ta);
        __syncthreads();
        int eb = block_exclusive_scan(b, sh, &tb);
        if (i < n_blocks) { blk[2 * i] = carry[0] + ea; blk[2 * i + 1] = carry[1] + eb; }
        __syncthreads();
        if (threadIdx.x == 0) { carry[0] += ta; carry[1] += tb; }
        __syncthreads();
    }
    if (threadIdx.x == 0) {
        int64_t pool = counters[0];
        counters[3] = pool;
        int64_t grown = pool + 2 * (int64_t)carry[0];
        counters[2] = grown > pool_capacity ? 1 : 0;
        counters[0] = grown > pool_capacity ? pool : grown;
        counters[1] = grown > pool_capacity ? 0 : carry[1];
    }
}

__global__ void __launch_bounds__(kGrowBlock) grow_write_kernel(
    int n_slots, const int32_t* __restrict__ slot_tree, const uint32_t* __restrict__ slot_nid,
    const int32_t* __restrict__ slot_node, const b200flow_split* __restrict__ split,
    const uint32_t* __restrict__ node_counts, const uint32_t* __restrict__ left_counts,
    const uint32_t* __restrict__ right_counts, int C, b200flow_node* nodes, uint64_t* node_mask, uint32_t* pool_counts,
    int32_t* node_tree, const int32_t* __restrict__ blk, const int64_t* __restrict__ counters, int32_t* next_tree,
    uint32_t* next_nid, int32_t* next_node, int32_t* next_parent, int32_t* child_slot) {
    __shared__ int sh[33];
    if (counters[2]) return;
    const int s = blockIdx.x * kGrowBlock + threadIdx.x;
    int is, nn; grow_flags(split, s, n_slots, &is, &nn);
    int t0, t1;
    int e0 = block_exclusive_scan(is, sh, &t0);
    __syncthreads();
    int e1 = block_exclusive_scan(nn, sh, &t1);
    if (s >= n_slots) return;
    const b200flow_split sp = split[s];
    const int node = slot_node[s];
    const uint32_t nid = slot_nid[s];
    const int tree = slot_tree[s];
    b200flow_node nd;
    nd.nid = nid; nd.feat = -1; nd.kind_bin = 0; nd.left = -1;
    int csl = -1, csr = -1;
    for (int k = 0; k < C; ++k) pool_counts[(int64_t)node * C + k] = node_counts[(int64_t)s * C + k];
    if (is) {
        const int64_t child = counters[3] + 2 * ((int64_t)blk[2 * blockIdx.x] + e0);
        nd.feat = sp.feat; nd.kind_bin = (sp.kind << 16) | (sp.bin_thr & 0xffff); nd.left = (int32_t)child;
        if (node_mask) for (int q = 0; q < 4; ++q) node_mask[(int64_t)node * 4 + q] = sp.mask[q];
        b200flow_node ch; ch.feat = -1; ch.kind_bin = 0; ch.left = -1;
        ch.nid = nid * 2u;     nodes[child] = ch;
        ch.nid = nid * 2u + 1; nodes[child + 1] = ch;
        node_tree[child] = tree; node_tree[child + 1] = tree;
        for (int k = 0; k < C; ++k) {
            pool_counts[child * C + k] = left_counts[(int64_t)s * C + k];
            pool_counts[(child + 1) * C + k] = right_counts[(int64_t)s * C + k];
        }
        int64_t ns = (int64_t)blk[2 * blockIdx.x + 1] + e1;
        if (!(sp.flags & 2)) { next_tree[ns] = tree; next_nid[ns] = nid * 2u; next_node[ns] = (int32_t)child; next_parent[ns] = s * 2; csl = (int)ns; ++ns; }
        if (!(sp.flags & 4)) { next_tree[ns] = tree; next_nid[ns] = nid * 2u + 1; next_node[ns] = (int32_t)child + 1; next_parent[ns] = s * 2 + 1; csr = (int)ns; }
    }
    if (child_slot) { child_slot[2 * s] = csl; child_slot[2 * s + 1] = csr; }
    nodes[node] = nd;
}

__global__ void __launch_bounds__(256) plan_route_kernel(int n_slots, const b200flow_split* __restrict__ split,
                                                         const int64_t* __restrict__ seg_begin, const int64_t* __restrict__ seg_end,
                                                         int chunk_rows, const int32_t* __restrict__ slot_node, double* node_gain,
                                                         int32_t* n_chunks, int32_t* cursors) {
    const int s = blockIdx.x * blockDim.x + threadIdx.x;
    if (s >= n_slots) return;
    if (cursors) { cursors[2 * s] = 0; cursors[2 * s + 1] = 0; }
    const int flags = split[s].flags;
    const bool routed = !(flags & 1) && (flags & 6) != 6;
    const int64_t len = seg_end[s] - seg_begin[s];
    n_chunks[s] = routed ? (int32_t)((len + chunk_rows - 1) / chunk_rows) : 0;
    if (node_gain) node_gain[slot_node[s]] = split[s].gain;
}

constexpr int kPartPerThread = 8;

__global__ void __launch_bounds__(256) partition_level_kernel(
    const uint8_t* __restrict__ tp, int stride, const b2f_entry* __restrict__ ent, b2f_entry* ent_out, int n_slots,
    const int64_t* __restrict__ seg_begin, const int64_t* __restrict__ seg_end, const int64_t* __restrict__ chunk_off,
    int chunk_rows, const b200flow_split* __restrict__ split, int32_t* cursors) {
    const int64_t c = blockIdx.x;
    const int s = find_slot(chunk_off, n_slots, c);
    const b200flow_split sp = split[s];
    if (sp.flags & 1) return;
    const bool keepL = !(sp.flags & 2), keepR = !(sp.flags & 4);
    if (!keepL && !keepR) return;
    const int64_t sb = seg_begin[s], se = seg_end[s];
    const int64_t b = sb + (c - chunk_off[s]) * chunk_rows;
    const int64_t e = min(se, b + chunk_rows);
    const int lane = lane_id();
    b2f_entry ents[kPartPerThread]; uint32_t dec = 0;
    int nL = 0, nR = 0;
#pragma unroll
    for (int k = 0; k < kPartPerThread; ++k) {
        const int64_t i = b + threadIdx.x + (int64_t)k * blockDim.x;
        int d = 0; ents[k] = make_uint2(0u, 0u);
        if (i < e) {
            ents[k] = ent[i];
            const int bin = tp[(int64_t)ents[k].x * stride + sp.feat];
            const bool left = sp.kind == 0 ? (bin <= sp.bin_thr) : ((sp.mask[bin >> 6] >> (bin & 63)) & 1ull);
            d = left ? (keepL ? 1 : 0) : (keepR ? 2 : 0);
        }
        dec |= (uint32_t)d << (2 * k);
        nL += __popc(__ballot_sync(0xffffffffu, d == 1));
        nR += __popc(__ballot_sync(0xffffffffu, d == 2));
    }
    int baseL = 0, baseR = 0;
    if (lane == 0) { if (nL) baseL = atomicAdd(&cursors[2 * s], nL); if (nR) baseR = atomicAdd(&cursors[2 * s + 1], nR); }
    baseL = __shfl_sync(0xffffffffu, baseL, 0); baseR = __shfl_sync(0xffffffffu, baseR, 0);
#pragma unroll
    for (int k = 0; k < kPartPerThread; ++k) {
        const int d = (dec >> (2 * k)) & 3;
        const uint32_t mL = __ballot_sync(0xffffffffu, d == 1), mR = __ballot_sync(0xffffffffu, d == 2);
        const uint32_t lt = (1u << lane) - 1u;
        if (d == 1) ent_out[sb + baseL + __popc(mL & lt)] = ents[k];
        else if (d == 2) ent_out[se - 1 - (baseR + __popc(mR & lt))] = ents[k];
        baseL += __popc(mL); baseR += __popc(mR);
    }
}

#ifndef B2F_EVICT_FIRST
#define B2F_EVICT_FIRST 1
#endif
#ifndef B2F_GRAN
#define B2F_GRAN 16
#endif
constexpr int kGran = B2F_GRAN;
__host__ __device__ inline int route_granules(int F) { return (F + 1 + kGran - 1) / kGran; }
__host__ __device__ inline int route_pitch(int F) { return kGran == 16 ? route_granules(F) : (route_granules(F) | 1); }
constexpr bool kEvictFirst = B2F_EVICT_FIRST != 0;

constexpr int kPackedMaxBytes = 64;
__device__ __forceinline__ int packed_swizzle_words(int i, int nq) {
    return nq == 2 ? ((i >> 2) & 1) << 2 : nq == 4 ? ((i >> 1) & 3) << 2 : 0;
}

struct RouteChunk { int32_t slot; int32_t n; long long begin; };

__global__ void route_chunks_kernel(const int64_t* __restrict__ chunk_off, int n_slots, const int64_t* __restrict__ n_chunks_dev,
                                    const int64_t* __restrict__ seg_begin, const int64_t* __restrict__ seg_end, int CH,
                                    RouteChunk* out) {
    int64_t c = (int64_t)blockIdx.x * blockDim.x + threadIdx.x;
    if (c >= *n_chunks_dev) return;
    const int s = find_slot(chunk_off, n_slots, c);
    RouteChunk rc; rc.slot = s; rc.begin = seg_begin[s] + (c - chunk_off[s]) * CH;
    rc.n = (int)(min(seg_end[s], (int64_t)rc.begin + CH) - rc.begin);
    out[c] = rc;
}

struct RouteArgs {
    const uint8_t* tp; int stride; int F;
    const int32_t* field_desc;
    const b2f_entry* ent; b2f_entry* ent_out;
    const RouteChunk* chunks; const int64_t* n_chunks_dev;
    const int64_t* seg_begin; const int64_t* seg_end;
    const b200flow_split* split; const int32_t* child_slot; int32_t* cursors;
    const uint16_t* subset_next; int m_total;
    int j0; int m;
    int n_bins; int C; uint32_t* hist_next;
    int route;
};

__host__ __device__ inline size_t route_tab_bytes(int mp, bool packed) { return packed && mp <= 12 ? (size_t)2 * mp * 32 * 8 : 0; }

template <int M, int NW, int KS, int MERGE, int NQ>
__global__ void __launch_bounds__(NW * 32, NW == 8 ? 3 : (NW == 16 ? 2 : 1)) route_hist_level_kernel(const RouteArgs a) {
    extern __shared__ __align__(16) uint32_t sm_u32[];
    constexpr bool PACKED = NQ > 0;
    constexpr bool kTab = PACKED && M > 0 && MERGE == 2;
    constexpr int kThreads = NW * 32, kSub = KS * 32;
    constexpr int gran = PACKED ? 16 : kGran;
    const int m = M > 0 ? M : a.m;
    const int F = a.F;
    const int tid = threadIdx.x, lane = lane_id(), wid = warp_id();
    const int nq = PACKED ? NQ : route_granules(F);
    const int rs = PACKED ? NQ * 16 : route_pitch(F) * kGran;
    const int nbC = a.n_bins * a.C, hsz = m * nbC;
    const int tile_words = rs * kSub / 4;
    uint32_t* tile = sm_u32 + (size_t)wid * tile_words;
    uint32_t* sh_hist = sm_u32 + (size_t)NW * tile_words;
    int* sh_fpos = (int*)(sh_hist + 2 * hsz);
    uint2* sh_tab = (uint2*)(sh_fpos + 2 * m);
    __shared__ b200flow_split sh_split;
    __shared__ int sh_child[2], sh_route_field;

    const int64_t n_chunks = *a.n_chunks_dev;
    const int64_t c0 = n_chunks * blockIdx.x / gridDim.x, c1 = n_chunks * (blockIdx.x + 1) / gridDim.x;
    if (c0 >= c1) return;
    auto flush = [&]() {
        for (int side = 0; side < 2; ++side) {
            const int cs = sh_child[side];
            if (cs < 0) continue;
            uint32_t* gh = a.hist_next + ((int64_t)cs * a.m_total + a.j0) * nbC;
            uint32_t* sh = sh_hist + side * hsz;
            for (int i = tid; i < hsz; i += kThreads) { const uint32_t v = sh[i]; if (v) { atomicAdd(gh + i, v); sh[i] = 0; } }
        }
    };
    for (int i = tid; i < 2 * hsz; i += kThreads) sh_hist[i] = 0;
    auto desc_at = [&](int64_t c) { return c < c1 ? __ldg((const int4*)(a.chunks + c)) : make_int4(-1, 0, 0, 0); };
    auto count_of = [&](const int4& d) { return min(kSub, d.y - wid * kSub); };
    auto entries_of = [&](const int4& d, b2f_entry* x) {
        const int cn = count_of(d);
        const b2f_entry* ep = a.ent + (((long long)(uint32_t)d.z) | ((long long)d.w << 32)) + wid * kSub;
#pragma unroll
        for (int k = 0; k < KS; ++k) x[k] = lane + 32 * k < cn ? (kEvictFirst ? ld_evict_first_u2(ep + 32 * k + lane) : __ldg(ep + 32 * k + lane)) : make_uint2(0u, 0u);
    };
    constexpr int kNQ = PACKED ? NQ : 1;
    constexpr bool kPow2 = (kNQ & (kNQ - 1)) == 0;
    const int g_e0 = kPow2 ? lane / kNQ : 0, g_q0 = kPow2 ? lane % kNQ : 0;
    const int g_sw = packed_swizzle_words(g_e0, NQ) >> 2;
    const uint8_t* g_src = a.tp + g_q0 * 16;
    uint8_t* g_dst = (uint8_t*)tile + g_e0 * rs + (g_q0 ^ g_sw) * 16;
    const uint32_t inv_nq = (1u << 20) / (uint32_t)nq + 1u;
    auto issue_gather = [&](const int4& d, const b2f_entry* x) {
        const int cn = count_of(d);
        if (PACKED) {
#pragma unroll
            for (int it = 0; it < KS * kNQ; ++it) {
                const int k = it / kNQ;
                if (kPow2) {
                    const int e = it * (32 / kNQ) + g_e0;
                    const uint32_t r = __shfl_sync(0xffffffffu, x[k].x, e & 31);
                    if (e < cn) cp_async16(g_dst + it * 512, g_src + (size_t)r * (kNQ * 16));
                } else {
                    const int c = it * 32 + lane, e = c / kNQ, q = c - e * kNQ;
                    const uint32_t r = __shfl_sync(0xffffffffu, x[k].x, e & 31);
                    if (e < cn) cp_async16((uint8_t*)tile + e * rs + q * 16, a.tp + (size_t)r * (kNQ * 16) + q * 16);
                }
            }
        } else {
            for (int c = lane; c < kSub * nq; c += 32) {
                const int e = (int)(((uint32_t)c * inv_nq) >> 20), q = c - e * nq;
                uint32_t r = __shfl_sync(0xffffffffu, x[0].x, e & 31);
                if (KS == 2) { const uint32_t r1 = __shfl_sync(0xffffffffu, x[KS - 1].x, e & 31); r = e < 32 ? r : r1; }
                if (e < cn) {
                    uint8_t* dst = (uint8_t*)tile + e * rs + q * gran;
                    const uint8_t* src = a.tp + (int64_t)r * a.stride + q * gran;
                    if (gran == 16) cp_async16(dst, src); else if (gran == 8) cp_async8(dst, src); else cp_async4(dst, src);
                }
            }
        }
        cp_async_commit();
    };
    bool pending = false;
    b2f_entry p_e[KS]; uint32_t p_dec = 0; int p_bl = 0, p_br = 0; int64_t p_sb = 0, p_se = 0;
#pragma unroll
    for (int k = 0; k < KS; ++k) p_e[k] = make_uint2(0u, 0u);
    const uint32_t lt = (1u << lane) - 1u;
    auto write_pending = [&]() {
        int baseL = __shfl_sync(0xffffffffu, p_bl, 0), baseR = __shfl_sync(0xffffffffu, p_br, 0);
#pragma unroll
        for (int k = 0; k < KS; ++k) {
            const int d = (p_dec >> (2 * k)) & 3;
            const uint32_t mL = __ballot_sync(0xffffffffu, d == 1), mR = __ballot_sync(0xffffffffu, d == 2);
            if (d == 1) { if (kEvictFirst) st_evict_first_u2(a.ent_out + p_sb + baseL + __popc(mL & lt), p_e[k]); else a.ent_out[p_sb + baseL + __popc(mL & lt)] = p_e[k]; }
            else if (d == 2) { if (kEvictFirst) st_evict_first_u2(a.ent_out + p_se - 1 - (baseR + __popc(mR & lt)), p_e[k]); else a.ent_out[p_se - 1 - (baseR + __popc(mR & lt))] = p_e[k]; }
            baseL += __popc(mL); baseR += __popc(mR);
        }
        pending = false;
    };

    int4 d0 = desc_at(c0), d1 = desc_at(c0 + 1), d2 = desc_at(c0 + 2);
    b2f_entry e[KS], f[KS], g[KS];
    entries_of(d0, e);
    entries_of(d1, f);
    int cur_slot = -1;
    const int lab_pos = PACKED ? __ldg(a.field_desc + F) : F;
    const uint8_t* tile8 = (const uint8_t*)tile;
    auto field = [&](int i, int d) -> uint32_t {
        if (!PACKED) return tile8[d + i * rs];
        const uint32_t v = tile[i * (rs >> 2) + ((d & 0xff) ^ packed_swizzle_words(i, nq))];
        return (v >> ((d >> 8) & 0xff)) & (uint32_t)(d >> 16);
    };
    for (int64_t c = c0; c < c1; ++c) {
        entries_of(d2, g);
        const int4 d3 = desc_at(c + 3);
        issue_gather(d0, e);
        if (pending) write_pending();
        cp_async_wait_all();
        __syncwarp();
        const int s = d0.x;
        if (s != cur_slot) {
            __syncthreads();
            if (cur_slot >= 0) flush();
            __syncthreads();
            if (tid < 16) ((uint32_t*)&sh_split)[tid] = ((const uint32_t*)(a.split + s))[tid];
            if (tid < 2) sh_child[tid] = a.child_slot[2 * s + tid];
            if (tid == 0) { const int fs = max(a.split[s].feat, 0); sh_route_field = PACKED ? a.field_desc[fs] : fs; }
            if (kTab) {
                constexpr int kM = M > 0 ? M : 1;
                for (int idx = tid; idx < 2 * kM * 32; idx += kThreads) {
                    const int side = idx / (kM * 32), t = idx / 32 % kM, ln = idx % 32, j = (ln % kM + t) % kM;
                    const int cs = a.child_slot[2 * s + side];
                    const int fidx = cs >= 0 ? a.subset_next[(int64_t)cs * a.m_total + a.j0 + j] : 0;
                    const uint32_t d = (uint32_t)__ldg(a.field_desc + fidx);
                    const uint32_t word = (d & 0xffu) ^ (uint32_t)packed_swizzle_words(ln, NQ);
                    sh_tab[idx] = make_uint2(word * 4u, ((d >> 8) & 31u) | ((d >> 16) << 8) | ((uint32_t)(side * hsz + j * nbC) << 16));
                }
            } else {
                for (int j = tid; j < 2 * m; j += kThreads) {
                    const int cs = a.child_slot[2 * s + (j >= m)];
                    const int fidx = cs >= 0 ? a.subset_next[(int64_t)cs * a.m_total + a.j0 + (j < m ? j : j - m)] : 0;
                    sh_fpos[j] = PACKED ? a.field_desc[fidx] : fidx;
                }
            }
            cur_slot = s;
            __syncthreads();
        }
        const int cnt = count_of(d0);
        if (cnt > 0) {
            const int cl = sh_child[0], cr = sh_child[1];
            const int fs = sh_route_field, kind = sh_split.kind, thr = sh_split.bin_thr;
            int nL = 0, nR = 0;
            uint32_t dec = 0;
#pragma unroll
            for (int k = 0; k < KS; ++k) {
                const int i = k * 32 + lane;
                int d = 0;
                if (i < cnt) {
                    const int bin = (int)field(i, fs);
                    const bool left = kind == 0 ? (bin <= thr) : ((sh_split.mask[bin >> 6] >> (bin & 63)) & 1ull);
                    d = left ? (cl >= 0 ? 1 : 0) : (cr >= 0 ? 2 : 0);
                }
                dec |= (uint32_t)d << (2 * k);
                const uint32_t mL = __ballot_sync(0xffffffffu, d == 1), mR = __ballot_sync(0xffffffffu, d == 2);
                nL += __popc(mL); nR += __popc(mR);
                if (d != 0) {
                    const uint32_t active = mL | mR;
                    const int side = d - 1;
                    const int* fpos = sh_fpos + side * m;
                    uint32_t* hist = sh_hist + side * hsz;
                    const uint32_t lab = field(i, lab_pos);
                    const uint32_t w = e[k].y;
                    if (M > 0 && MERGE == 1) {
                        const uint32_t tag = (lab << 8) | ((uint32_t)side << 16);
#pragma unroll
                        for (int j = 0; j < M; ++j) {
                            const int fp = fpos[j];
                            const uint32_t bin = field(i, fp);
                            const uint32_t key = bin | tag;
                            uint32_t* addr = &hist[j * nbC + bin * a.C + lab];
                            const int l0 = __ffs(active) - 1;
                            const bool top = key == __shfl_sync(active, key, l0);
                            const uint32_t sum = __reduce_add_sync(active, top ? w : 0u);
                            if (!top || lane == l0) atomicAdd(addr, top ? sum : w);
                        }
                    } else if (kTab) {
                        const uint2* tab = sh_tab + side * (M * 32) + lane;
                        const uint8_t* rec = (const uint8_t*)tile + i * rs;
                        uint32_t* hl = sh_hist + lab;
#pragma unroll
                        for (int t = 0; t < M; ++t) {
                            const uint2 dd = tab[t * 32];
                            const uint32_t v = *(const uint32_t*)(rec + dd.x);
                            const uint32_t bin = __funnelshift_r(v, 0u, dd.y) & ((dd.y >> 8) & 0xffu);
                            atomicAdd(hl + (dd.y >> 16) + bin * a.C, w);
                        }
                    } else if (M > 0 && MERGE == 2) {
                        int j = lane % M;
#pragma unroll
                        for (int t = 0; t < M; ++t) {
                            const int fp = fpos[j];
                            const uint32_t bin = field(i, fp);
                            atomicAdd(&hist[j * nbC + bin * a.C + lab], w);
                            j = j + 1 == M ? 0 : j + 1;
                        }
                    } else {
                        for (int j = 0; j < m; ++j) {
                            const int fp = fpos[j];
                            const uint32_t bin = field(i, fp);
                            atomicAdd(&hist[j * nbC + bin * a.C + lab], w);
                        }
                    }
                }
            }
            __syncwarp();
            if (a.route && (nL | nR)) {
                if (lane == 0) {
                    const unsigned long long old = atomicAdd((unsigned long long*)(a.cursors + 2 * s), (unsigned long long)(uint32_t)nL | ((unsigned long long)(uint32_t)nR << 32));
                    p_bl = (int)(uint32_t)old; p_br = (int)(uint32_t)(old >> 32);
                }
#pragma unroll
                for (int k = 0; k < KS; ++k) p_e[k] = e[k];
                p_dec = dec; p_sb = a.seg_begin[s]; p_se = a.seg_end[s];
                pending = true;
            }
        }
        d0 = d1; d1 = d2; d2 = d3;
#pragma unroll
        for (int k = 0; k < KS; ++k) { e[k] = f[k]; f[k] = g[k]; }
    }
    if (pending) write_pending();
    cp_async_wait_all();
    __syncthreads();
    flush();
}

struct RouteCfg { int nw, ks, m_pass, per_sm; size_t smem; };
constexpr size_t kSmemPerSM = 227 * 1024;
constexpr size_t kSmemCtaOverhead = 1024 + 128;

static size_t route_hist_smem(int rs, bool packed, int mp, int n_bins, int C, int nw, int ks) {
    return (size_t)nw * ks * 32 * rs + 2 * (size_t)mp * n_bins * C * 4 + 2 * (size_t)mp * 4 + route_tab_bytes(mp, packed) + 64;
}
static int route_max_ctas(int nw) { return nw == 8 ? 3 : (nw == 16 ? 2 : 1); }

static bool route_cfg(int F, int rs, bool packed, int m, int n_bins, int C, RouteCfg* out) {
    static const int cand[5][2] = {{8, 2}, {8, 1}, {16, 2}, {16, 1}, {32, 1}};
    int force_nw = 0, force_ks = 0;
    { const char* e = getenv("B200FLOW_ROUTE_SHAPE"); if (e && sscanf(e, "%dx%d", &force_nw, &force_ks) != 2) force_nw = force_ks = 0; }
    if (F <= 0 || F > 255 || m <= 0 || n_bins <= 0 || C <= 0) return false;
    auto fits = [&](int mp, int nw, int ks) { return route_hist_smem(rs, packed, mp, n_bins, C, nw, ks) + kSmemCtaOverhead <= kSmemPerSM; };
    int mp = m;
    while (mp >= 1 && !fits(mp, 8, 1)) --mp;
    if (mp < 1) return false;
    const int passes = (m + mp - 1) / mp;
    mp = (m + passes - 1) / passes;
    int best = -1; long best_key = -1;
    for (int i = 0; i < 5; ++i) {
        const int nw = cand[i][0], ks = cand[i][1];
        if (force_nw > 0 && (nw != force_nw || ks != force_ks)) continue;
        if (!fits(mp, nw, ks)) continue;
        const size_t smem = route_hist_smem(rs, packed, mp, n_bins, C, nw, ks);
        int per_sm = (int)(kSmemPerSM / (smem + kSmemCtaOverhead));
        if (per_sm > route_max_ctas(nw)) per_sm = route_max_ctas(nw);
        const int warps = per_sm * nw > 32 ? 32 : per_sm * nw;
        const long key = ((long)(warps * ks < 48 ? warps * ks : 48) << 20) + ((long)(1023 - nw * ks) << 10) + warps;
        if (key > best_key) { best_key = key; best = i; }
    }
    if (best < 0) return false;
    out->nw = cand[best][0]; out->ks = cand[best][1]; out->m_pass = mp;
    out->smem = route_hist_smem(rs, packed, mp, n_bins, C, out->nw, out->ks);
    out->per_sm = (int)(kSmemPerSM / (out->smem + kSmemCtaOverhead));
    if (out->per_sm > route_max_ctas(out->nw)) out->per_sm = route_max_ctas(out->nw);
    return true;
}

static int route_hist_variant() {
    const char* e = getenv("B200FLOW_ROUTE_VARIANT");
    if (e && !strcmp(e, "merge")) return 1;
    if (e && !strcmp(e, "generic")) return 0;
    return 2;
}

template <int NW, int KS, int NQ>
static cudaError_t route_launch(int M, int merge, unsigned grid_cap, size_t smem, int per_sm_hint, int waves, int64_t n_chunks_max,
                                const RouteArgs& a, cudaStream_t st) {
    cudaError_t e = cudaSuccess;
#define B2F_ROUTE_GO(KERNEL)                                                                                                   \
    {                                                                                                                          \
        e = cudaFuncSetAttribute(KERNEL, cudaFuncAttributeMaxDynamicSharedMemorySize, (int)smem);                             \
        if (e != cudaSuccess) return e;                                                                                        \
        int per_sm = 0;                                                                                                        \
        e = cudaOccupancyMaxActiveBlocksPerMultiprocessor(&per_sm, KERNEL, NW * 32, smem);                                    \
        if (e != cudaSuccess) return e;                                                                                        \
        if (per_sm < 1) per_sm = per_sm_hint > 0 ? per_sm_hint : 1;                                                            \
        const int64_t want = (int64_t)kNumSMs * per_sm * waves;                                                                \
        unsigned grid = (unsigned)(n_chunks_max < want ? n_chunks_max : want);                                                 \
        if (grid_cap && grid > grid_cap) grid = grid_cap;                                                                      \
        KERNEL<<<grid, NW * 32, smem, st>>>(a);                                                                                \
    }
#define B2F_ROUTE_CASE(MM)                                                                                                     \
    case MM:                                                                                                                   \
        if (merge == 1) B2F_ROUTE_GO((route_hist_level_kernel<MM, NW, KS, 1, NQ>))                                         \
        else if (merge == 2) B2F_ROUTE_GO((route_hist_level_kernel<MM, NW, KS, 2, NQ>))                                    \
        else B2F_ROUTE_GO((route_hist_level_kernel<0, NW, KS, 0, NQ>))                                                     \
        break;
    switch (M) {
        B2F_ROUTE_CASE(1) B2F_ROUTE_CASE(2) B2F_ROUTE_CASE(3) B2F_ROUTE_CASE(4) B2F_ROUTE_CASE(5) B2F_ROUTE_CASE(6)
        B2F_ROUTE_CASE(7) B2F_ROUTE_CASE(8) B2F_ROUTE_CASE(9) B2F_ROUTE_CASE(10) B2F_ROUTE_CASE(11) B2F_ROUTE_CASE(12)
        default: B2F_ROUTE_GO((route_hist_level_kernel<0, NW, KS, 0, NQ>)) break;
    }
#undef B2F_ROUTE_CASE
#undef B2F_ROUTE_GO
    return cudaGetLastError();
}

template <int NQ>
static cudaError_t route_shape(const RouteCfg& cfg, int M, int merge, size_t smem, int waves, int64_t n_chunks_max, const RouteArgs& a,
                               cudaStream_t st) {
    if (cfg.nw == 8 && cfg.ks == 2) return route_launch<8, 2, NQ>(M, merge, 0, smem, cfg.per_sm, waves, n_chunks_max, a, st);
    if (cfg.nw == 8) return route_launch<8, 1, NQ>(M, merge, 0, smem, cfg.per_sm, waves, n_chunks_max, a, st);
    if (cfg.nw == 16 && cfg.ks == 2) return route_launch<16, 2, NQ>(M, merge, 0, smem, cfg.per_sm, waves, n_chunks_max, a, st);
    if (cfg.nw == 16) return route_launch<16, 1, NQ>(M, merge, 0, smem, cfg.per_sm, waves, n_chunks_max, a, st);
    return route_launch<32, 1, NQ>(M, merge, 0, smem, cfg.per_sm, waves, n_chunks_max, a, st);
}

__global__ void next_segments_kernel(int n_next, const int64_t* __restrict__ n_next_dev, const int32_t* __restrict__ next_parent,
                                     const int64_t* __restrict__ seg_begin, const int64_t* __restrict__ seg_end,
                                     const int32_t* __restrict__ cursors, int64_t* next_begin, int64_t* next_end) {
    int i = blockIdx.x * blockDim.x + threadIdx.x;
    if (i >= n_next || (n_next_dev && i >= *n_next_dev)) return;
    const int p = next_parent[i], ps = p >> 1;
    if ((p & 1) == 0) { next_begin[i] = seg_begin[ps]; next_end[i] = seg_begin[ps] + cursors[2 * ps]; }
    else { next_begin[i] = seg_end[ps] - cursors[2 * ps + 1]; next_end[i] = seg_end[ps]; }
}

__global__ void finalize_forest_kernel(int64_t n_nodes, const uint32_t* __restrict__ pool_counts, int C, double* leaf_prob) {
    int64_t i = (int64_t)blockIdx.x * blockDim.x + threadIdx.x;
    if (i >= n_nodes) return;
    double tot = 0.0;
    for (int k = 0; k < C; ++k) tot += (double)pool_counts[i * C + k];
    for (int k = 0; k < C; ++k) leaf_prob[i * C + k] = tot != 0.0 ? (double)pool_counts[i * C + k] / tot : 0.0;
}

}

using namespace b200flow;

extern "C" int b200flow_feature_subsets(uint64_t seed, int32_t n_slots, const int32_t* slot_tree, const uint32_t* slot_nid,
                                        int32_t F, int32_t m, uint16_t* subset, void* stream) {
    B2F_REQUIRE(slot_tree && slot_nid && subset && F > 0 && F < 65536 && m > 0 && m <= F, "feature_subsets: bad arguments");
    B2F_REQUIRE(m == F || m <= kMaxSubset, "feature_subsets: subset size %d > %d not supported", m, kMaxSubset);
    if (n_slots <= 0) return B200FLOW_OK;
    feature_subsets_kernel<<<(n_slots + 127) / 128, 128, 0, (cudaStream_t)stream>>>(seed, n_slots, slot_tree, slot_nid, F, m, subset);
    return check_launch("feature_subsets");
}

extern "C" int b200flow_hist_level(const uint8_t* tp, int32_t tp_stride, int32_t F, const void* ent,
                                   int32_t n_slots, const int64_t* seg_begin, const int64_t* seg_end, const int64_t* chunk_off,
                                   int64_t n_chunks, int32_t chunk_rows, const uint16_t* subset, int32_t m, int32_t n_bins,
                                   int32_t C, uint32_t* hist, void* stream) {
    B2F_REQUIRE(tp && ent && seg_begin && seg_end && chunk_off && subset && hist, "hist_level: null pointer");
    B2F_REQUIRE(m > 0 && m <= 256 && n_bins > 0 && n_bins <= 256 && C > 0 && C <= 256 && chunk_rows > 0, "hist_level: bad shape");
    const size_t per_feat = (size_t)n_bins * C * 4;
    B2F_REQUIRE(per_feat <= 200 * 1024, "hist_level: one feature's histogram (%zu B) exceeds shared memory", per_feat);
    int m_pass = (int)((64 * 1024) / per_feat);
    if (m_pass < 1) m_pass = 1;
    if (m_pass > m) m_pass = m;
    size_t smem = per_feat * m_pass;
    if (n_slots <= 0 || n_chunks <= 0) return B200FLOW_OK;
    B2F_REQUIRE(n_chunks < ((int64_t)1 << 31), "hist_level: too many chunks");
    cudaError_t e = cudaFuncSetAttribute(hist_level_kernel, cudaFuncAttributeMaxDynamicSharedMemorySize, (int)smem);
    if (e != cudaSuccess) { set_error("hist_level: %s", cudaGetErrorString(e)); return B200FLOW_ERR_CUDA; }
    hist_level_kernel<<<(unsigned)n_chunks, 256, smem, (cudaStream_t)stream>>>(tp, tp_stride, F, (const b2f_entry*)ent, n_slots, seg_begin,
                                                                             seg_end, chunk_off, chunk_rows, subset, m, n_bins, C, m_pass, hist);
    return check_launch("hist_level");
}

extern "C" int b200flow_score_level(const uint32_t* hist, int32_t n_slots, const uint16_t* subset, int32_t m, int32_t n_bins,
                                    int32_t C, const int32_t* feat_bins, const int32_t* feat_kind, int32_t level, int32_t max_depth,
                                    int32_t min_instances, double min_info_gain, b200flow_split* split, uint32_t* node_counts,
                                    uint32_t* left_counts, uint32_t* right_counts, void* stream) {
    B2F_REQUIRE(hist && subset && feat_bins && feat_kind && split && node_counts && left_counts && right_counts, "score_level: null pointer");
    B2F_REQUIRE(m > 0 && n_bins > 0 && n_bins <= 256 && C > 0 && C <= 256, "score_level: bad shape");
    if (n_slots <= 0) return B200FLOW_OK;
    const size_t per_feat = (size_t)n_bins * C * 4 + (size_t)n_bins * 4 + (size_t)n_bins;
    const size_t per_warp = ((size_t)n_bins * 8 + (size_t)n_bins * C * 4 + 7) & ~(size_t)7;
    const size_t fixed = (size_t)2 * C * 4 + 16 + per_warp * (kScoreThreads / 32) + 16;
    int batch = m < 64 ? m : 64;
    while (batch > 1 && fixed + per_feat * batch > 160 * 1024) --batch;
    const size_t smem = fixed + per_feat * batch;
    B2F_REQUIRE(smem <= 200 * 1024, "score_level: scratch exceeds shared memory");
    cudaError_t e = cudaFuncSetAttribute(score_level_kernel, cudaFuncAttributeMaxDynamicSharedMemorySize, (int)smem);
    if (e != cudaSuccess) { set_error("score_level: %s", cudaGetErrorString(e)); return B200FLOW_ERR_CUDA; }
    score_level_kernel<<<n_slots, kScoreThreads, smem, (cudaStream_t)stream>>>(hist, n_slots, subset, m, n_bins, C, feat_bins, feat_kind, level,
                                                                              max_depth, min_instances, min_info_gain, batch, split,
                                                                              node_counts, left_counts, right_counts);
    return check_launch("score_level");
}

extern "C" int b200flow_grow_level(int32_t n_slots, const int32_t* slot_tree, const uint32_t* slot_nid, const int32_t* slot_node,
                                   const b200flow_split* split, const uint32_t* node_counts, const uint32_t* left_counts,
                                   const uint32_t* right_counts, int32_t C, b200flow_node* nodes, uint64_t* node_mask,
                                   uint32_t* pool_counts, int32_t* node_tree, int64_t pool_capacity, int32_t* next_tree,
                                   uint32_t* next_nid, int32_t* next_node, int32_t* next_parent, int32_t* child_slot,
                                   int64_t* counters, void* stream) {
    B2F_REQUIRE(slot_tree && slot_nid && slot_node && split && node_counts && left_counts && right_counts && nodes && pool_counts &&
                    node_tree && next_tree && next_nid && next_node && next_parent && counters, "grow_level: null pointer");
    if (n_slots <= 0) return B200FLOW_OK;
    const int nb = (n_slots + kGrowBlock - 1) / kGrowBlock;
    int32_t* blk = (int32_t*)(counters + 8);
    grow_count_kernel<<<nb, kGrowBlock, 0, (cudaStream_t)stream>>>(n_slots, split, blk);
    grow_scan_kernel<<<1, 1024, 0, (cudaStream_t)stream>>>(nb, blk, counters, pool_capacity);
    grow_write_kernel<<<nb, kGrowBlock, 0, (cudaStream_t)stream>>>(n_slots, slot_tree, slot_nid, slot_node, split, node_counts, left_counts,
                                                                  right_counts, C, nodes, node_mask, pool_counts, node_tree, blk, counters,
                                                                  next_tree, next_nid, next_node, next_parent, child_slot);
    return check_launch("grow_level");
}

extern "C" int b200flow_plan_route(int32_t n_slots, const b200flow_split* split, const int64_t* seg_begin, const int64_t* seg_end,
                                   int32_t chunk_rows, const int32_t* slot_node, double* node_gain, int32_t* n_chunks, int32_t* cursors,
                                   void* stream) {
    if (n_slots <= 0) return B200FLOW_OK;
    B2F_REQUIRE(split && seg_begin && seg_end && n_chunks && chunk_rows > 0 && (!node_gain || slot_node), "plan_route: bad arguments");
    plan_route_kernel<<<(n_slots + 255) / 256, 256, 0, (cudaStream_t)stream>>>(n_slots, split, seg_begin, seg_end, chunk_rows, slot_node, node_gain, n_chunks, cursors);
    return check_launch("plan_route");
}

extern "C" int b200flow_partition_level(const uint8_t* tp, int32_t tp_stride, const void* ent, void* ent_out, int32_t n_slots,
                                        const int64_t* seg_begin, const int64_t* seg_end, const int64_t* chunk_off, int64_t n_chunks,
                                        int32_t chunk_rows, const b200flow_split* split, int32_t* cursors, void* stream) {
    B2F_REQUIRE(tp && ent && ent_out && seg_begin && seg_end && chunk_off && split && cursors, "partition_level: null pointer");
    B2F_REQUIRE(chunk_rows > 0 && chunk_rows <= 256 * kPartPerThread, "partition_level: chunk_rows must be <= %d", 256 * kPartPerThread);
    if (n_slots <= 0 || n_chunks <= 0) return B200FLOW_OK;
    partition_level_kernel<<<(unsigned)n_chunks, 256, 0, (cudaStream_t)stream>>>(tp, tp_stride, (const b2f_entry*)ent, (b2f_entry*)ent_out, n_slots, seg_begin, seg_end,
                                                                               chunk_off, chunk_rows, split, cursors);
    return check_launch("partition_level");
}

extern "C" int b200flow_next_segments(int32_t n_next, const int64_t* n_next_dev, const int32_t* next_parent, const int64_t* seg_begin,
                                      const int64_t* seg_end, const int32_t* cursors, int64_t* next_begin, int64_t* next_end, void* stream) {
    B2F_REQUIRE(next_parent && seg_begin && seg_end && cursors && next_begin && next_end, "next_segments: null pointer");
    if (n_next <= 0) return B200FLOW_OK;
    next_segments_kernel<<<(n_next + 255) / 256, 256, 0, (cudaStream_t)stream>>>(n_next, n_next_dev, next_parent, seg_begin, seg_end, cursors, next_begin, next_end);
    return check_launch("next_segments");
}

extern "C" int b200flow_finalize_forest(int64_t n_nodes, const uint32_t* pool_counts, int32_t C, double* leaf_prob, void* stream) {
    B2F_REQUIRE(pool_counts && leaf_prob && C > 0, "finalize_forest: bad arguments");
    if (n_nodes <= 0) return B200FLOW_OK;
    finalize_forest_kernel<<<(unsigned)((n_nodes + 255) / 256), 256, 0, (cudaStream_t)stream>>>(n_nodes, pool_counts, C, leaf_prob);
    return check_launch("finalize_forest");
}

extern "C" int b200flow_packed_layout(int32_t F, const int32_t* feat_bins, int32_t C, int32_t* desc, int32_t* rec_bytes) {
    B2F_REQUIRE(feat_bins && desc && rec_bytes && F > 0 && C > 0 && C <= 256, "packed_layout: bad arguments");
    *rec_bytes = 0;
    if (F > 255) return B200FLOW_OK;
    int width[256], order[256], used[256];
    auto bits = [](int v) { int b = 0; while (v > 0) { ++b; v >>= 1; } return b > 0 ? b : 1; };
    for (int f = 0; f <= F; ++f) {
        const int nb = f < F ? feat_bins[f] : C;
        B2F_REQUIRE(nb >= 1 && nb <= 256, "packed_layout: field %d has %d values", f, nb);
        width[f] = bits(nb - 1);
        order[f] = f;
    }
    for (int i = 1; i <= F; ++i) {
        const int f = order[i]; int k = i - 1;
        while (k >= 0 && width[order[k]] < width[f]) { order[k + 1] = order[k]; --k; }
        order[k + 1] = f;
    }
    int nw = 0;
    for (int i = 0; i <= F; ++i) {
        const int f = order[i];
        int w = 0;
        while (w < nw && used[w] + width[f] > 32) ++w;
        if (w == nw) used[nw++] = 0;
        desc[f] = w | (used[w] << 8) | (((1 << width[f]) - 1) << 16);
        used[w] += width[f];
    }
    const int bytes = (nw * 4 + 15) / 16 * 16;
    *rec_bytes = bytes <= kPackedMaxBytes && bytes + 16 <= route_pitch(F) * kGran ? bytes : 0;
    return B200FLOW_OK;
}

extern "C" int b200flow_route_hist_config(int32_t F, int32_t m, int32_t n_bins, int32_t C, int32_t rec_bytes, int32_t* chunk_rows,
                                          int32_t* m_pass) {
    RouteCfg cfg;
    if (rec_bytes < 0 || !route_cfg(F, rec_bytes > 0 ? rec_bytes : route_pitch(F) * kGran, rec_bytes > 0, m, n_bins, C, &cfg)) return 0;
    if (chunk_rows) *chunk_rows = cfg.nw * cfg.ks * 32;
    if (m_pass) *m_pass = cfg.m_pass;
    return 1;
}

extern "C" int b200flow_route_hist_level(const uint8_t* tp, int32_t tp_stride, int32_t F, const int32_t* field_desc,
                                         const void* ent, void* ent_out,
                                         int32_t n_slots, const int64_t* seg_begin, const int64_t* seg_end, const int64_t* chunk_off,
                                         const int64_t* n_chunks_dev, int64_t n_chunks_max, int32_t chunk_rows,
                                         const b200flow_split* split, const int32_t* child_slot,
                                         int32_t* cursors, void* chunk_scratch, const uint16_t* subset_next, int32_t m, int32_t n_bins,
                                         int32_t C, uint32_t* hist_next, int32_t flags, void* stream) {
    B2F_REQUIRE(tp && ent && seg_begin && seg_end && chunk_off && n_chunks_dev && split && child_slot && chunk_scratch &&
                    subset_next && hist_next, "route_hist_level: null pointer");
    const bool route = (flags & 1) != 0;
    B2F_REQUIRE(!route || (ent_out && cursors && ((uintptr_t)cursors & 7) == 0), "route_hist_level: routing needs ent_out and 8-byte aligned cursors");
    if (field_desc)
        B2F_REQUIRE((tp_stride & 15) == 0 && tp_stride > 0 && tp_stride <= kPackedMaxBytes && ((uintptr_t)tp & 15) == 0,
                    "route_hist_level: packed records must be 16-byte multiples up to %d bytes, 16-byte aligned", kPackedMaxBytes);
    else
        B2F_REQUIRE((tp_stride & 15) == 0 && tp_stride >= (F + 1 + 15) / 16 * 16 && ((uintptr_t)tp & 15) == 0, "route_hist_level: bad TreePoint stride/alignment");
    B2F_REQUIRE(((uintptr_t)chunk_scratch & 15) == 0, "route_hist_level: chunk_scratch must be 16-byte aligned");
    RouteCfg cfg;
    const int rs = field_desc ? tp_stride : route_pitch(F) * kGran;
    B2F_REQUIRE(route_cfg(F, rs, field_desc != nullptr, m, n_bins, C, &cfg), "route_hist_level: one feature's child histograms exceed shared memory (use partition_level + hist_level)");
    B2F_REQUIRE(chunk_rows == cfg.nw * cfg.ks * 32, "route_hist_level: chunk_rows must be the value of b200flow_route_hist_config (%d)", cfg.nw * cfg.ks * 32);
    if (n_slots <= 0 || n_chunks_max <= 0) return B200FLOW_OK;
    cudaStream_t st = (cudaStream_t)stream;
    RouteChunk* chunks = (RouteChunk*)chunk_scratch;
    route_chunks_kernel<<<(unsigned)((n_chunks_max + 255) / 256), 256, 0, st>>>(chunk_off, n_slots, n_chunks_dev, seg_begin,
                                                                             seg_end, chunk_rows, chunks);
    RouteArgs a;
    a.tp = tp; a.stride = tp_stride; a.F = F; a.field_desc = field_desc; a.ent = (const b2f_entry*)ent; a.ent_out = (b2f_entry*)ent_out; a.chunks = chunks; a.n_chunks_dev = n_chunks_dev;
    a.seg_begin = seg_begin; a.seg_end = seg_end; a.split = split; a.child_slot = child_slot; a.cursors = cursors;
    a.subset_next = subset_next; a.m_total = m; a.n_bins = n_bins; a.C = C; a.hist_next = hist_next;
    static int waves = -1;
    if (waves < 0) { const char* e = getenv("B200FLOW_ROUTE_WAVES"); waves = e ? atoi(e) : 2; if (waves < 1) waves = 1; }
    int merge = route_hist_variant();
    if (merge == 1 && C > 128) merge = 2;
    for (int j0 = 0, pass = 0; j0 < m; j0 += cfg.m_pass, ++pass) {
        a.j0 = j0; a.m = m - j0 < cfg.m_pass ? m - j0 : cfg.m_pass; a.route = (route && pass == 0) ? 1 : 0;
        const int M = a.m <= 12 ? a.m : 0;
        const size_t smem = route_hist_smem(rs, field_desc != nullptr, a.m, n_bins, C, cfg.nw, cfg.ks);
        cudaError_t e;
        switch (field_desc ? tp_stride / 16 : 0) {
            case 1: e = route_shape<1>(cfg, M, merge, smem, waves, n_chunks_max, a, st); break;
            case 2: e = route_shape<2>(cfg, M, merge, smem, waves, n_chunks_max, a, st); break;
            case 3: e = route_shape<3>(cfg, M, merge, smem, waves, n_chunks_max, a, st); break;
            case 4: e = route_shape<4>(cfg, M, merge, smem, waves, n_chunks_max, a, st); break;
            default: e = route_shape<0>(cfg, M, merge, smem, waves, n_chunks_max, a, st); break;
        }
        if (e != cudaSuccess) { set_error("route_hist_level: %s", cudaGetErrorString(e)); return B200FLOW_ERR_CUDA; }
    }
    return check_launch("route_hist_level");
}
```

Measured before the change: 156.8 million.

## Add warp-per-slot scoring, fuse subset draw into grow, recycle zeroed histograms

```diff
diff --git a/include/b200flow.h b/include/b200flow.h
--- a/include/b200flow.h
+++ b/include/b200flow.h
@@ -120,13 +120,16 @@
     uint64_t mask[4];
 } b200flow_split;
 
-int b200flow_score_level(const uint32_t* hist, int32_t n_slots, const uint16_t* subset,
+#define B200FLOW_SCORE_ZERO_HIST 1
+int b200flow_score_level(uint32_t* hist, int32_t n_slots, const uint16_t* subset,
                          int32_t m, int32_t n_bins, int32_t C,
                          const int32_t* feat_bins, const int32_t* feat_kind,
                          int32_t level, int32_t max_depth, int32_t min_instances,
                          double min_info_gain,
                          b200flow_split* split, uint32_t* node_counts,
-                         uint32_t* left_counts, uint32_t* right_counts, void* stream);
+                         uint32_t* left_counts, uint32_t* right_counts, int32_t flags, void* stream);
+
+int b200flow_score_level_variant(int32_t m, int32_t n_bins, int32_t C);
 
 typedef struct b200flow_node {
     int32_t feat;
@@ -142,7 +145,8 @@
                         b200flow_node* nodes, uint64_t* node_mask, uint32_t* pool_counts,
                         int32_t* node_tree, int64_t pool_capacity,
                         int32_t* next_tree, uint32_t* next_nid, int32_t* next_node,
-                        int32_t* next_parent, int32_t* child_slot, int64_t* counters, void* stream);
+                        int32_t* next_parent, int32_t* child_slot, int64_t* counters,
+                        uint64_t seed, int32_t F, int32_t m, uint16_t* next_subset, void* stream);
 
 int b200flow_partition_level(const uint8_t* tp, int32_t tp_stride,
                              const void* ent, void* ent_out,
diff --git a/spark-network-traffic-classifier_b200/b200flow/_lib.py b/spark-network-traffic-classifier_b200/b200flow/_lib.py
--- a/spark-network-traffic-classifier_b200/b200flow/_lib.py
+++ b/spark-network-traffic-classifier_b200/b200flow/_lib.py
@@ -47,8 +47,9 @@
     "b200flow_exclusive_scan_i32_to_i64": [_P, _I64, _P, _P, _P],
     "b200flow_feature_subsets": [_U64, _I32, _P, _P, _I32, _I32, _P, _P],
     "b200flow_hist_level": [_P, _I32, _I32, _P, _I32, _P, _P, _P, _I64, _I32, _P, _I32, _I32, _I32, _P, _P],
-    "b200flow_score_level": [_P, _I32, _P, _I32, _I32, _I32, _P, _P, _I32, _I32, _I32, _F64, _P, _P, _P, _P, _P],
-    "b200flow_grow_level": [_I32, _P, _P, _P, _P, _P, _P, _P, _I32, _P, _P, _P, _P, _I64, _P, _P, _P, _P, _P, _P, _P],
+    "b200flow_score_level": [_P, _I32, _P, _I32, _I32, _I32, _P, _P, _I32, _I32, _I32, _F64, _P, _P, _P, _P, _I32, _P],
+    "b200flow_grow_level": [_I32, _P, _P, _P, _P, _P, _P, _P, _I32, _P, _P, _P, _P, _I64, _P, _P, _P, _P, _P, _P, _U64, _I32, _I32,
+                            _P, _P],
     "b200flow_route_hist_level": [_P, _I32, _I32, _P, _P, _P, _I32, _P, _P, _P, _P, _I64, _I32, _P, _P, _P, _P, _P, _I32, _I32,
                                   _I32, _P, _I32, _P],
     "b200flow_pack_records": [_P, _I32, _I64, _I32, _P, _I32, _P, _P],
@@ -84,7 +85,7 @@
 }
 EXPORTS = sorted(list(_SIGNATURES) + ["b200flow_last_error", "b200flow_version", "b200flow_route_hist_config",
                                        "b200flow_packed_layout", "b200flow_binary_counts_scratch",
-                                       "b200flow_group_sums_chunks", "b200flow_mlp_config"])
+                                       "b200flow_group_sums_chunks", "b200flow_mlp_config", "b200flow_score_level_variant"])
 
 _lib = None
 launches = 0
@@ -115,6 +116,8 @@
         lib.b200flow_group_sums_chunks.restype = C.c_int
         lib.b200flow_mlp_config.argtypes = [_P, _I32, C.POINTER(_I64), C.POINTER(_I64)]
         lib.b200flow_mlp_config.restype = C.c_int
+        lib.b200flow_score_level_variant.argtypes = [_I32, _I32, _I32]
+        lib.b200flow_score_level_variant.restype = C.c_int
         _lib = lib
     return _lib
 
@@ -133,6 +136,10 @@
     if lib.b200flow_packed_layout(int(fb.shape[0]), fb.ctypes.data, int(n_classes), desc.ctypes.data, C.byref(rb)) != 0:
         raise B200FlowError("b200flow_packed_layout failed: %s" % lib.b200flow_last_error().decode())
     return desc, int(rb.value)
+
+
+def score_level_variant(m, n_bins, n_classes):
+    return "warp" if load().b200flow_score_level_variant(int(m), int(n_bins), int(n_classes)) else "cta"
 
 
 def binary_counts_scratch(S, n):
diff --git a/spark-network-traffic-classifier_b200/b200flow/forest.py b/spark-network-traffic-classifier_b200/b200flow/forest.py
--- a/spark-network-traffic-classifier_b200/b200flow/forest.py
+++ b/spark-network-traffic-classifier_b200/b200flow/forest.py
@@ -36,6 +36,11 @@
 HIST_BUDGET_BYTES = int(_os.environ.get("B200FLOW_HIST_BUDGET_GB", "10")) << 30
 RS_MIN_BYTES = int(_os.environ.get("B200FLOW_RS_MIN_BYTES", str(8 << 20)))
 RS_CHUNKS = int(_os.environ.get("B200FLOW_RS_CHUNKS", "1"))
+SCORE_ZERO_HIST = 1
+
+
+def _hist_recycle():
+    return _os.environ.get("B200FLOW_HIST_RECYCLE", "1") != "0"
 
 
 @dataclass
@@ -567,6 +572,7 @@
 
     stats["route_chunk"], stats["route_passes"] = route_ch if fused else 0, route_passes if fused else 0
     stats["record_format"], stats["record_bytes"] = ("packed", rec_bytes) if field_desc is not None else ("bytes", stride)
+    stats["score_variant"] = _lib.score_level_variant(m, n_bins, C)
 
     def chunk_table(nch):
         off = torch.empty(nch.shape[0] + 1, dtype=torch.int64, device=dev)
@@ -617,7 +623,7 @@
             if cnt > 0:
                 _timed("score_level", "b200flow_score_level", ptr(mine), cnt, ptr(sub[s0 + lo:s0 + lo + cnt]), m, n_bins, C, ptr(feat_bins),
                        ptr(feat_kind), lvl, p.max_depth, int(p.min_instances_per_node), float(p.min_info_gain), ptr(sec[0]), ptr(sec[1]),
-                       ptr(sec[2]), ptr(sec[3]))
+                       ptr(sec[2]), ptr(sec[3]), 0)
             gathered = torch.empty((world, per * REC), dtype=torch.uint8, device=dev)
             gw = dist.all_gather_into_tensor(gathered, local, group=group, async_op=True)
             gathers.append((s0, per, gathered, gw))
@@ -631,8 +637,24 @@
             ev1 = torch.cuda.Event(enable_timing=True); ev1.record()
             PROFILE.setdefault("level_exchange", []).append((ev0, ev1))
 
-    def run_route(roff, rch_dev, n_parents, split_, child_slot_, cursors_, next_subset_, n_next_cap, route=True):
-        hist_next = torch.zeros((n_next_cap + world - 1) * hsz, dtype=torch.int32, device=dev)
+    recycle = fused and not use_rs and _hist_recycle()
+    hist_bufs, hist_clean = [None, None], [0, 0]
+
+    def level_hist(n_next_cap, parity):
+        need = (n_next_cap + world - 1) * hsz
+        if not recycle:
+            return torch.zeros(need, dtype=torch.int32, device=dev)
+        if hist_bufs[parity] is None or hist_bufs[parity].numel() < need:
+            hist_bufs[parity] = torch.empty(max(need, min(4 * need, HIST_BUDGET_BYTES // 4)), dtype=torch.int32, device=dev)
+            hist_clean[parity] = 0
+        buf = hist_bufs[parity]
+        if hist_clean[parity] < need:
+            buf[hist_clean[parity]:need].zero_()
+            hist_clean[parity] = need
+        return buf[:need]
+
+    def run_route(roff, rch_dev, n_parents, split_, child_slot_, cursors_, next_subset_, n_next_cap, parity, route=True):
+        hist_next = level_hist(n_next_cap, parity)
         cmax = route_chunks_max + n_parents
         scratch = torch.empty(cmax * 4, dtype=torch.int32, device=dev)
         _timed("route_hist_level", "b200flow_route_hist_level", ptr(rec_tp), rec_stride, F, ptr(field_desc), ptr(ent), ptr(ent2), n_parents,
@@ -654,7 +676,7 @@
                               torch.full((T,), -1, dtype=torch.int32, device=dev)], 1).contiguous().view(-1)
         cursors0 = torch.zeros(2 * T, dtype=torch.int32, device=dev)
         roff0 = plan_route(T, pseudo_t, seg_begin, seg_end, total)
-        hist_full = run_route(roff0, total, T, pseudo_t, child0, cursors0, subset, T, route=False)
+        hist_full = run_route(roff0, total, T, pseudo_t, child0, cursors0, subset, T, 0, route=False)
         hist_ready = hist_full[:T * hsz]
     while n_slots > 0:
         grow_pool(pool_size + 2 * n_slots)
@@ -699,7 +721,8 @@
                     PROFILE.setdefault("level_exchange", []).append((ev0, ev1))
             _timed("score_level", "b200flow_score_level", ptr(h), gs, ptr(subset[g0:g1]), m, n_bins, C, ptr(feat_bins), ptr(feat_kind),
                    level, p.max_depth, int(p.min_instances_per_node), float(p.min_info_gain), ptr(split[g0:g1]),
-                   ptr(node_counts[g0:g1]), ptr(left_counts[g0:g1]), ptr(right_counts[g0:g1]))
+                   ptr(node_counts[g0:g1]), ptr(left_counts[g0:g1]), ptr(right_counts[g0:g1]),
+                   SCORE_ZERO_HIST if (recycle and hist_ready is not None) else 0)
             del h
         split, node_counts, left_counts, right_counts = split[:n_slots], node_counts[:n_slots], left_counts[:n_slots], right_counts[:n_slots]
         hist_ready = None
@@ -716,9 +739,11 @@
         next_node = torch.empty(2 * n_slots, dtype=torch.int32, device=dev)
         next_parent = torch.empty(2 * n_slots, dtype=torch.int32, device=dev)
         child_slot = torch.empty(2 * n_slots, dtype=torch.int32, device=dev)
+        next_subset = torch.empty((2 * n_slots, m), dtype=torch.int16, device=dev)
         _timed("grow_level", "b200flow_grow_level", n_slots, ptr(slot_tree), ptr(slot_nid), ptr(slot_node), ptr(split), ptr(node_counts),
                ptr(left_counts), ptr(right_counts), C, ptr(nodes), ptr(node_mask), ptr(pool_counts), ptr(node_tree),
-               cap_nodes, ptr(next_tree), ptr(next_nid), ptr(next_node), ptr(next_parent), ptr(child_slot), ptr(counters))
+               cap_nodes, ptr(next_tree), ptr(next_nid), ptr(next_node), ptr(next_parent), ptr(child_slot), ptr(counters),
+               seed, F, m, ptr(next_subset))
         n_cap = 2 * n_slots
         speculative = fused and n_cap * hsz * 4 <= HIST_BUDGET_BYTES and level + 1 < p.max_depth
         if not speculative:
@@ -731,8 +756,7 @@
                 side_stream.wait_event(ev_planned)
                 cnt = counters[:5].to("cpu", non_blocking=True) if host_cnt is None else host_cnt.copy_(counters[:5], non_blocking=True)
                 ev_read = torch.cuda.Event(); ev_read.record(side_stream)
-            next_subset = level_subsets(n_cap, next_tree, next_nid)
-            hist_next = run_route(roff, counters[4:5], n_slots, split, child_slot, cursors, next_subset, n_cap,
+            hist_next = run_route(roff, counters[4:5], n_slots, split, child_slot, cursors, next_subset, n_cap, (level + 1) & 1,
                                   route=level + 2 < p.max_depth)
             next_begin = torch.empty(n_cap, dtype=torch.int64, device=dev)
             next_end = torch.empty(n_cap, dtype=torch.int64, device=dev)
@@ -753,7 +777,7 @@
             hist_full = hist_next
             next_subset, next_begin, next_end = next_subset[:n_next], next_begin[:n_next], next_end[:n_next]
         else:
-            next_subset = level_subsets(n_next, next_tree, next_nid)
+            next_subset = next_subset[:n_next]
             cursors = torch.zeros(2 * n_slots, dtype=torch.int32, device=dev)
             if chunk_off is None:
                 lens = seg_end - seg_begin
diff --git a/spark-network-traffic-classifier_b200/csrc/forest.cu b/spark-network-traffic-classifier_b200/csrc/forest.cu
--- a/spark-network-traffic-classifier_b200/csrc/forest.cu
+++ b/spark-network-traffic-classifier_b200/csrc/forest.cu
@@ -8,16 +8,52 @@
 
 constexpr int kMaxSubset = 128;
 
-__global__ void __launch_bounds__(128) feature_subsets_kernel(uint64_t seed, int n_slots, const int32_t* __restrict__ slot_tree,
-                                                              const uint32_t* __restrict__ slot_nid, int F, int m,
-                                                              uint16_t* subset) {
-    int s = blockIdx.x * blockDim.x + threadIdx.x;
-    if (s >= n_slots) return;
-    uint16_t* out = subset + (int64_t)s * m;
+constexpr int kRegSubset = 16;
+
+__device__ __forceinline__ void draw_feature_subset_reg(uint64_t seed, int tree, uint32_t nid, int F, int m, uint16_t* out) {
+    int pos[kRegSubset], val[kRegSubset], pick[kRegSubset];
+    int nt = 0;
+    uint4 r = make_uint4(0, 0, 0, 0);
+#pragma unroll
+    for (int i = 0; i < kRegSubset; ++i) {
+        pos[i] = -1; val[i] = 0; pick[i] = 0;
+        if (i < m) {
+            if ((i & 3) == 0) r = philox_keyed(seed, PURPOSE_FEAT, (uint32_t)tree, nid, (uint32_t)(i >> 2), 0u);
+            const uint32_t w = (i & 3) == 0 ? r.x : (i & 3) == 1 ? r.y : (i & 3) == 2 ? r.z : r.w;
+            const int j = i + (int)(w % (uint32_t)(F - i));
+            int vi = i, vj = j, kj = -1;
+#pragma unroll
+            for (int k = 0; k < i; ++k) {
+                if (pos[k] == i) vi = val[k];
+                if (pos[k] == j) { vj = val[k]; kj = k; }
+            }
+            pick[i] = vj;
+            if (j != i) {
+#pragma unroll
+                for (int k = 0; k <= i; ++k) {
+                    if (kj >= 0 ? k == kj : k == nt) { pos[k] = kj >= 0 ? pos[k] : j; val[k] = vi; }
+                }
+                if (kj < 0) ++nt;
+            }
+        }
+    }
+#pragma unroll
+    for (int i = 0; i < kRegSubset; ++i) {
+        if (i < m) {
+            int rank = 0;
+#pragma unroll
+            for (int k = 0; k < kRegSubset; ++k) rank += (k < m && pick[k] < pick[i]) ? 1 : 0;
+            out[rank] = (uint16_t)pick[i];
+        }
+    }
+}
+
+template <bool REG>
+__device__ __forceinline__ void draw_feature_subset(uint64_t seed, int tree, uint32_t nid, int F, int m, uint16_t* out) {
     if (m >= F) { for (int i = 0; i < F; ++i) out[i] = (uint16_t)i; return; }
+    if (REG) { draw_feature_subset_reg(seed, tree, nid, F, m, out); return; }
     uint16_t pos[kMaxSubset], val[kMaxSubset], pick[kMaxSubset];
     int nt = 0;
-    const int tree = slot_tree[s]; const uint32_t nid = slot_nid[s];
     uint4 r = make_uint4(0, 0, 0, 0);
     for (int i = 0; i < m; ++i) {
         if ((i & 3) == 0) r = philox_keyed(seed, PURPOSE_FEAT, (uint32_t)tree, nid, (uint32_t)(i >> 2), 0u);
@@ -37,6 +73,15 @@
         pick[k + 1] = x;
     }
     for (int i = 0; i < m; ++i) out[i] = pick[i];
+}
+
+template <bool REG>
+__global__ void __launch_bounds__(128) feature_subsets_kernel(uint64_t seed, int n_slots, const int32_t* __restrict__ slot_tree,
+                                                              const uint32_t* __restrict__ slot_nid, int F, int m,
+                                                              uint16_t* subset) {
+    int s = blockIdx.x * blockDim.x + threadIdx.x;
+    if (s >= n_slots) return;
+    draw_feature_subset<REG>(seed, slot_tree[s], slot_nid[s], F, m, subset + (int64_t)s * m);
 }
 
 __device__ __forceinline__ int find_slot(const int64_t* __restrict__ chunk_off, int n_slots, int64_t c) {
@@ -92,6 +137,7 @@
     if (tot == 0.0) return 0.0;
     const double y = __drcp_rn(tot);
     double imp = 1.0;
+#pragma unroll 4
     for (int k = 0; k < C; ++k) { double f = div_rn((double)c[k], tot, y); imp -= f * f; }
     return imp;
 }
@@ -99,25 +145,190 @@
 __device__ __forceinline__ double split_gain(const uint32_t* L, const uint32_t* tot, int C, double parent_imp,
                                              int min_inst, double min_gain) {
     double lc = 0.0, rc = 0.0;
+#pragma unroll 4
     for (int k = 0; k < C; ++k) { lc += (double)L[k]; rc += (double)(tot[k] - L[k]); }
     if (lc < (double)min_inst || rc < (double)min_inst) return -DBL_MAX;
     const double t = lc + rc;
+    const double yl = __drcp_rn(lc), yr = __drcp_rn(rc), yt = __drcp_rn(t);
     double gl = 1.0, gr = 1.0;
-    if (lc == 0.0) gl = 0.0; else { const double y = __drcp_rn(lc); for (int k = 0; k < C; ++k) { double f = div_rn((double)L[k], lc, y); gl -= f * f; } }
-    if (rc == 0.0) gr = 0.0; else { const double y = __drcp_rn(rc); for (int k = 0; k < C; ++k) { double f = div_rn((double)(tot[k] - L[k]), rc, y); gr -= f * f; } }
-    const double yt = __drcp_rn(t);
+#pragma unroll 4
+    for (int k = 0; k < C; ++k) {
+        const double fl = div_rn((double)L[k], lc, yl), fr = div_rn((double)(tot[k] - L[k]), rc, yr);
+        gl -= fl * fl; gr -= fr * fr;
+    }
+    if (lc == 0.0) gl = 0.0;
+    if (rc == 0.0) gr = 0.0;
     const double lw = div_rn(lc, t, yt), rw = div_rn(rc, t, yt);
     const double gain = parent_imp - lw * gl - rw * gr;
     if (gain < min_gain) return -DBL_MAX;
     return gain;
 }
 
+
+__device__ int feature_candidates(uint32_t* cum, int* order, uint8_t* cand, double* cen, uint32_t* raw, int nb, int kind, int C) {
+    const int lane = lane_id();
+    if (kind == 1) {
+        for (int i = lane; i < nb * C; i += 32) raw[i] = cum[i];
+        __syncwarp();
+        for (int c = lane; c < nb; c += 32) {
+            double cnt = 0.0;
+            for (int k = 0; k < C; ++k) cnt += (double)raw[c * C + k];
+            cen[c] = cnt == 0.0 ? DBL_MAX : (C > 2 ? gini_u32(raw + c * C, C, cnt) : (double)raw[c * C + 1]);
+        }
+        __syncwarp();
+        for (int c = lane; c < nb; c += 32) {
+            const double ce = cen[c]; int rk = 0;
+            for (int c2 = 0; c2 < nb; ++c2) { const double o = cen[c2]; rk += (o < ce || (o == ce && c2 < c)) ? 1 : 0; }
+            order[rk] = c;
+        }
+        __syncwarp();
+        for (int k = lane; k < C; k += 32) {
+            uint32_t a = 0;
+#pragma unroll 4
+            for (int i = 0; i < nb; ++i) { a += raw[order[i] * C + k]; cum[i * C + k] = a; }
+        }
+    } else if (kind == 0) {
+        if (C <= 16) {
+            const int nseg = 32 / C, seg_len = (nb + nseg - 1) / nseg;
+            const int k = lane % C, seg = lane / C;
+            const bool act = seg < nseg;
+            const int b0 = min(nb, seg * seg_len), b1 = act ? min(nb, b0 + seg_len) : b0;
+            uint32_t a = 0;
+#pragma unroll 4
+            for (int b = b0; b < b1; ++b) a += cum[b * C + k];
+            uint32_t run = 0;
+            for (int s2 = 0; s2 < nseg; ++s2) { const uint32_t v = __shfl_sync(0xffffffffu, a, s2 * C + k); if (s2 < seg) run += v; }
+#pragma unroll 4
+            for (int b = b0; b < b1; ++b) { run += cum[b * C + k]; cum[b * C + k] = run; }
+        } else {
+            for (int k = lane; k < C; k += 32) { uint32_t a = 0; for (int b = 0; b < nb; ++b) { a += cum[b * C + k]; cum[b * C + k] = a; } }
+        }
+    }
+    __syncwarp();
+    const int ns = kind == 2 ? (1 << (nb - 1)) - 1 : nb - 1;
+    int n_cand = 0;
+    for (int sp0 = 0; sp0 < ns; sp0 += 32) {
+        const int sp = sp0 + lane;
+        bool keep = sp < ns;
+        if (keep && kind != 2 && sp > 0) {
+            keep = false;
+            for (int k = 0; k < C; ++k) keep |= cum[sp * C + k] != cum[(sp - 1) * C + k];
+        }
+        const uint32_t mk = __ballot_sync(0xffffffffu, keep);
+        if (keep) cand[n_cand + __popc(mk & ((1u << lane) - 1u))] = (uint8_t)sp;
+        n_cand += __popc(mk);
+    }
+    return n_cand;
+}
+
+__device__ __forceinline__ void feature_totals(const uint32_t* cum, int nb, int kind, int C, uint32_t* tot) {
+    for (int k = lane_id(); k < C; k += 32) {
+        uint32_t a;
+        if (kind == 2) { a = 0; for (int c = 0; c < nb; ++c) a += cum[c * C + k]; }
+        else a = cum[(nb - 1) * C + k];
+        tot[k] = a;
+    }
+}
+
+__device__ __forceinline__ double candidate_gain(const uint32_t* cum, int kind, int nb, int sp, const uint32_t* tot, int C,
+                                                 double parent_imp, int min_inst, double min_gain) {
+    if (kind != 2) return split_gain(cum + sp * C, tot, C, parent_imp, min_inst, min_gain);
+    const unsigned bits = (unsigned)(sp + 1);
+    double lc = 0.0, rc = 0.0;
+    for (int k = 0; k < C; ++k) { uint32_t a = 0; for (int c = 0; c < nb; ++c) if ((bits >> c) & 1u) a += cum[c * C + k]; lc += (double)a; rc += (double)(tot[k] - a); }
+    if (lc < (double)min_inst || rc < (double)min_inst) return -DBL_MAX;
+    const double t = lc + rc; double gl = 1.0, gr = 1.0;
+    const double yl = __drcp_rn(lc), yr = __drcp_rn(rc), yt = __drcp_rn(t);
+#pragma unroll 2
+    for (int k = 0; k < C; ++k) {
+        uint32_t a = 0; for (int c = 0; c < nb; ++c) if ((bits >> c) & 1u) a += cum[c * C + k];
+        const double fl = div_rn((double)a, lc, yl), fr = div_rn((double)(tot[k] - a), rc, yr);
+        gl -= fl * fl; gr -= fr * fr;
+    }
+    if (lc == 0.0) gl = 0.0;
+    if (rc == 0.0) gr = 0.0;
+    const double lw = div_rn(lc, t, yt), rw = div_rn(rc, t, yt);
+    const double g = parent_imp - lw * gl - rw * gr;
+    return g < min_gain ? -DBL_MAX : g;
+}
+
+__device__ __forceinline__ void eval_candidates(int first, int stride, int nf, const int* ncand, const int* kinds, const int* nbs,
+                                                const uint8_t* cand_all, const uint32_t* cum_all, int n_bins, int nbC,
+                                                const uint32_t* tot, int C, double parent_imp, int min_inst, double min_gain, int j0,
+                                                double& best, int& bj, int& bs) {
+    int n_items = 0;
+    for (int jj = 0; jj < nf; ++jj) n_items += ncand[jj];
+    for (int it = first; it < n_items; it += stride) {
+        int jj = 0, o = 0;
+        while (it >= o + ncand[jj]) { o += ncand[jj]; ++jj; }
+        const int sp = cand_all[(size_t)jj * n_bins + (it - o)];
+        const double g = candidate_gain(cum_all + (size_t)jj * nbC, kinds[jj], nbs[jj], sp, tot, C, parent_imp, min_inst, min_gain);
+        if (g > best) { best = g; bj = j0 + jj; bs = sp; }
+    }
+}
+
+__device__ __forceinline__ void warp_argmax(double& g, int& bj, int& bs) {
+#pragma unroll
+    for (int o = 16; o > 0; o >>= 1) {
+        const double og = __shfl_xor_sync(0xffffffffu, g, o); const int oj = __shfl_xor_sync(0xffffffffu, bj, o), os = __shfl_xor_sync(0xffffffffu, bs, o);
+        if (oj >= 0 && (bj < 0 || og > g || (og == g && (oj < bj || (oj == bj && os < bs))))) { g = og; bj = oj; bs = os; }
+    }
+}
+
+__device__ __forceinline__ void split_left(const uint32_t* cum, const int* order, int kind, int nb, int sp, int C, uint32_t* L,
+                                           unsigned long long* mask) {
+    unsigned long long mk[4] = {0, 0, 0, 0};
+    if (kind == 2) {
+        const unsigned bits = (unsigned)(sp + 1);
+        for (int k = 0; k < C; ++k) { uint32_t a = 0; for (int c = 0; c < nb; ++c) if ((bits >> c) & 1u) a += cum[c * C + k]; L[k] = a; }
+        mk[0] = bits;
+    } else {
+        for (int k = 0; k < C; ++k) L[k] = cum[sp * C + k];
+        if (kind == 1) for (int i = 0; i <= sp; ++i) { const int c = order[i]; mk[c >> 6] |= 1ull << (c & 63); }
+    }
+    for (int q = 0; q < 4; ++q) mask[q] = mk[q];
+}
+
+__device__ __forceinline__ void write_split(int s, bool has, double best_gain, double parent_imp, int feat, int kind, int sp,
+                                            const unsigned long long* mask, const uint32_t* bestL, const uint32_t* tot, int C,
+                                            int level, int max_depth, b200flow_split* split) {
+    b200flow_split o;
+    o.gain = has ? best_gain : -DBL_MAX; o.impurity = parent_imp;
+    const bool leaf = !(has && best_gain > 0.0) || level >= max_depth;
+    int flags = leaf ? 1 : 0;
+    o.feat = -1; o.kind = 0; o.bin_thr = 0;
+    o.mask[0] = o.mask[1] = o.mask[2] = o.mask[3] = 0;
+    if (!leaf) {
+        o.feat = feat; o.kind = kind == 0 ? 0 : 1; o.bin_thr = sp;
+        for (int q = 0; q < 4; ++q) o.mask[q] = mask[q];
+        double lc = 0.0, rc = 0.0, gl = 1.0, gr = 1.0;
+        for (int k = 0; k < C; ++k) { lc += (double)bestL[k]; rc += (double)(tot[k] - bestL[k]); }
+        if (lc == 0.0) gl = 0.0; else for (int k = 0; k < C; ++k) { const double fq = (double)bestL[k] / lc; gl -= fq * fq; }
+        if (rc == 0.0) gr = 0.0; else for (int k = 0; k < C; ++k) { const double fq = (double)(tot[k] - bestL[k]) / rc; gr -= fq * fq; }
+        if (level + 1 == max_depth || gl == 0.0) flags |= 2;
+        if (level + 1 == max_depth || gr == 0.0) flags |= 4;
+    }
+    o.flags = flags;
+    split[s] = o;
+}
+
+__device__ __forceinline__ void write_counts(int first, int stride, int s, bool has, const uint32_t* bestL, const uint32_t* tot, int C,
+                                             uint32_t* node_counts, uint32_t* left_counts, uint32_t* right_counts) {
+    for (int k = first; k < C; k += stride) {
+        node_counts[(int64_t)s * C + k] = tot[k];
+        const uint32_t l = has ? bestL[k] : 0u;
+        left_counts[(int64_t)s * C + k] = l;
+        right_counts[(int64_t)s * C + k] = has ? tot[k] - l : 0u;
+    }
+}
+
 constexpr int kScoreThreads = 128;
 
 __global__ void __launch_bounds__(kScoreThreads) score_level_kernel(
-    const uint32_t* __restrict__ hist, int n_slots, const uint16_t* __restrict__ subset, int m, int n_bins, int C,
+    uint32_t* hist, int n_slots, const uint16_t* __restrict__ subset, int m, int n_bins, int C,
     const int32_t* __restrict__ feat_bins, const int32_t* __restrict__ feat_kind, int level, int max_depth, int min_inst,
-    double min_gain, int batch, b200flow_split* split, uint32_t* node_counts, uint32_t* left_counts, uint32_t* right_counts) {
+    double min_gain, int batch, int zero_hist, b200flow_split* split, uint32_t* node_counts, uint32_t* left_counts,
+    uint32_t* right_counts) {
     extern __shared__ __align__(8) uint8_t sm_raw[];
     const int s = blockIdx.x;
     const int tid = threadIdx.x, w = warp_id(), lane = lane_id(), nw = kScoreThreads / 32;
@@ -137,79 +348,26 @@
     __shared__ double sh_best_gain; __shared__ int sh_best_j, sh_best_s, sh_best_kind;
     __shared__ unsigned long long sh_best_mask[4];
 
-    const uint32_t* h0 = hist + (int64_t)s * m * nbC;
+    uint32_t* h0 = hist + (int64_t)s * m * nbC;
     if (tid == 0) { sh_best_gain = -DBL_MAX; sh_best_j = -1; sh_best_s = -1; sh_best_kind = 0; }
     double parent_imp = 0.0;
 
     for (int j0 = 0; j0 < m; j0 += batch) {
         const int nb_feats = min(batch, m - j0);
         {
-            const uint32_t* src = h0 + (int64_t)j0 * nbC;
+            uint32_t* src = h0 + (int64_t)j0 * nbC;
             const int nwords = nb_feats * nbC;
-            for (int i = tid; i < nwords; i += kScoreThreads) cum_all[i] = __ldg(src + i);
+            for (int i = tid; i < nwords; i += kScoreThreads) cum_all[i] = src[i];
+            if (zero_hist) for (int i = tid; i < nwords; i += kScoreThreads) src[i] = 0;
         }
         __syncthreads();
         for (int jj = w; jj < nb_feats; jj += nw) {
             const int f = subset[(int64_t)s * m + j0 + jj];
             const int nb = feat_bins[f], kind = feat_kind[f];
             uint32_t* cum = cum_all + (size_t)jj * nbC;
-            int* order = order_all + (size_t)jj * n_bins;
-            if (lane == 0) { sh_kind[jj] = kind; sh_nb[jj] = nb; }
-            if (kind == 1) {
-                for (int i = lane; i < nb * C; i += 32) raw[i] = cum[i];
-                __syncwarp();
-                for (int c = lane; c < nb; c += 32) {
-                    double cnt = 0.0;
-                    for (int k = 0; k < C; ++k) cnt += (double)raw[c * C + k];
-                    cen[c] = cnt == 0.0 ? DBL_MAX : (C > 2 ? gini_u32(raw + c * C, C, cnt) : (double)raw[c * C + 1]);
-                }
-                __syncwarp();
-                for (int c = lane; c < nb; c += 32) {
-                    const double ce = cen[c]; int rk = 0;
-                    for (int c2 = 0; c2 < nb; ++c2) { const double o = cen[c2]; rk += (o < ce || (o == ce && c2 < c)) ? 1 : 0; }
-                    order[rk] = c;
-                }
-                __syncwarp();
-                for (int k = lane; k < C; k += 32) { uint32_t a = 0; for (int i = 0; i < nb; ++i) { a += raw[order[i] * C + k]; cum[i * C + k] = a; } }
-            } else if (kind == 0) {
-                if (C <= 16) {
-                    const int nseg = 32 / C, seg_len = (nb + nseg - 1) / nseg;
-                    const int k = lane % C, seg = lane / C;
-                    const bool act = seg < nseg;
-                    const int b0 = min(nb, seg * seg_len), b1 = act ? min(nb, b0 + seg_len) : b0;
-                    uint32_t a = 0;
-                    for (int b = b0; b < b1; ++b) a += cum[b * C + k];
-                    uint32_t run = 0;
-                    for (int s2 = 0; s2 < nseg; ++s2) { const uint32_t v = __shfl_sync(0xffffffffu, a, s2 * C + k); if (s2 < seg) run += v; }
-                    for (int b = b0; b < b1; ++b) { run += cum[b * C + k]; cum[b * C + k] = run; }
-                } else {
-                    for (int k = lane; k < C; k += 32) { uint32_t a = 0; for (int b = 0; b < nb; ++b) { a += cum[b * C + k]; cum[b * C + k] = a; } }
-                }
-            }
-            __syncwarp();
-            if (j0 == 0 && jj == 0) {
-                for (int k = lane; k < C; k += 32) {
-                    uint32_t a;
-                    if (kind == 2) { a = 0; for (int c = 0; c < nb; ++c) a += cum[c * C + k]; }
-                    else a = cum[(nb - 1) * C + k];
-                    tot[k] = a;
-                }
-            }
-            uint8_t* cand = cand_all + (size_t)jj * n_bins;
-            const int ns = kind == 2 ? (1 << (nb - 1)) - 1 : nb - 1;
-            int n_cand = 0;
-            for (int sp0 = 0; sp0 < ns; sp0 += 32) {
-                const int sp = sp0 + lane;
-                bool keep = sp < ns;
-                if (keep && kind != 2 && sp > 0) {
-                    keep = false;
-                    for (int k = 0; k < C; ++k) keep |= cum[sp * C + k] != cum[(sp - 1) * C + k];
-                }
-                const uint32_t mk = __ballot_sync(0xffffffffu, keep);
-                if (keep) cand[n_cand + __popc(mk & ((1u << lane) - 1u))] = (uint8_t)sp;
-                n_cand += __popc(mk);
-            }
-            if (lane == 0) sh_ncand[jj] = n_cand;
+            const int n_cand = feature_candidates(cum, order_all + (size_t)jj * n_bins, cand_all + (size_t)jj * n_bins, cen, raw, nb, kind, C);
+            if (j0 == 0 && jj == 0) feature_totals(cum, nb, kind, C, tot);
+            if (lane == 0) { sh_kind[jj] = kind; sh_nb[jj] = nb; sh_ncand[jj] = n_cand; }
         }
         __syncthreads();
         if (j0 == 0) {
@@ -217,40 +375,10 @@
             if (lane == 0) { double ptot = 0.0; for (int k = 0; k < C; ++k) ptot += (double)tot[k]; pi = gini_u32(tot, C, ptot); }
             parent_imp = __shfl_sync(0xffffffffu, pi, 0);
         }
-        int n_items = 0;
-        for (int jj = 0; jj < nb_feats; ++jj) n_items += sh_ncand[jj];
-        double tbest = -DBL_MAX; int tj = -1, ts = -1;
-        for (int it = tid; it < n_items; it += kScoreThreads) {
-            int jj = 0, o = 0;
-            while (it >= o + sh_ncand[jj]) { o += sh_ncand[jj]; ++jj; }
-            const int sp = cand_all[(size_t)jj * n_bins + (it - o)];
-            const uint32_t* cum = cum_all + (size_t)jj * nbC;
-            double g;
-            if (sh_kind[jj] != 2) {
-                g = split_gain(cum + sp * C, tot, C, parent_imp, min_inst, min_gain);
-            } else {
-                const unsigned bits = (unsigned)(sp + 1); const int nb = sh_nb[jj];
-                double lc = 0.0, rc = 0.0;
-                for (int k = 0; k < C; ++k) { uint32_t a = 0; for (int c = 0; c < nb; ++c) if ((bits >> c) & 1u) a += cum[c * C + k]; lc += (double)a; rc += (double)(tot[k] - a); }
-                if (lc < (double)min_inst || rc < (double)min_inst) g = -DBL_MAX;
-                else {
-                    const double t = lc + rc; double gl = 1.0, gr = 1.0;
-                    if (lc == 0.0) gl = 0.0; else { const double y = __drcp_rn(lc); for (int k = 0; k < C; ++k) { uint32_t a = 0; for (int c = 0; c < nb; ++c) if ((bits >> c) & 1u) a += cum[c * C + k]; const double fq = div_rn((double)a, lc, y); gl -= fq * fq; } }
-                    if (rc == 0.0) gr = 0.0; else { const double y = __drcp_rn(rc); for (int k = 0; k < C; ++k) { uint32_t a = 0; for (int c = 0; c < nb; ++c) if ((bits >> c) & 1u) a += cum[c * C + k]; const double fq = div_rn((double)(tot[k] - a), rc, y); gr -= fq * fq; } }
-                    const double yt = __drcp_rn(t);
-                    const double lw = div_rn(lc, t, yt), rw = div_rn(rc, t, yt);
-                    g = parent_imp - lw * gl - rw * gr;
-                    if (g < min_gain) g = -DBL_MAX;
-                }
-            }
-            if (g > tbest) { tbest = g; tj = j0 + jj; ts = sp; }
-        }
-        double g = tbest; int bj = tj, bs = ts;
-#pragma unroll
-        for (int o = 16; o > 0; o >>= 1) {
-            const double og = __shfl_xor_sync(0xffffffffu, g, o); const int oj = __shfl_xor_sync(0xffffffffu, bj, o), os = __shfl_xor_sync(0xffffffffu, bs, o);
-            if (oj >= 0 && (bj < 0 || og > g || (og == g && (oj < bj || (oj == bj && os < bs))))) { g = og; bj = oj; bs = os; }
-        }
+        double g = -DBL_MAX; int bj = -1, bs = -1;
+        eval_candidates(tid, kScoreThreads, nb_feats, sh_ncand, sh_kind, sh_nb, cand_all, cum_all, n_bins, nbC, tot, C, parent_imp,
+                        min_inst, min_gain, j0, g, bj, bs);
+        warp_argmax(g, bj, bs);
         if (lane == 0) { sh_wg[w] = g; sh_wj[w] = bj; sh_ws[w] = bs; }
         __syncthreads();
         if (tid == 0) {
@@ -262,51 +390,88 @@
             }
             if (improved) {
                 sh_best_gain = bg; sh_best_j = gj; sh_best_s = gs;
-                const int jj = gj - j0; const int kind = sh_kind[jj], nb = sh_nb[jj];
-                const uint32_t* cum = cum_all + (size_t)jj * nbC;
-                sh_best_kind = kind;
-                unsigned long long mk[4] = {0, 0, 0, 0};
-                if (kind == 2) {
-                    const unsigned bits = (unsigned)(gs + 1);
-                    for (int k = 0; k < C; ++k) { uint32_t a = 0; for (int c = 0; c < nb; ++c) if ((bits >> c) & 1u) a += cum[c * C + k]; bestL[k] = a; }
-                    mk[0] = bits;
-                } else {
-                    for (int k = 0; k < C; ++k) bestL[k] = cum[gs * C + k];
-                    if (kind == 1) { const int* order = order_all + (size_t)jj * n_bins; for (int i = 0; i <= gs; ++i) { const int c = order[i]; mk[c >> 6] |= 1ull << (c & 63); } }
-                }
-                for (int q = 0; q < 4; ++q) sh_best_mask[q] = mk[q];
+                const int jj = gj - j0;
+                sh_best_kind = sh_kind[jj];
+                split_left(cum_all + (size_t)jj * nbC, order_all + (size_t)jj * n_bins, sh_kind[jj], sh_nb[jj], gs, C, bestL, sh_best_mask);
             }
         }
         __syncthreads();
     }
     const bool has = sh_best_j >= 0;
-    for (int k = tid; k < C; k += kScoreThreads) {
-        node_counts[(int64_t)s * C + k] = tot[k];
-        const uint32_t l = has ? bestL[k] : 0u;
-        left_counts[(int64_t)s * C + k] = l;
-        right_counts[(int64_t)s * C + k] = has ? tot[k] - l : 0u;
-    }
-    if (tid == 0) {
-        b200flow_split o;
-        const double bg = sh_best_gain;
-        o.gain = has ? bg : -DBL_MAX; o.impurity = parent_imp;
-        const bool leaf = !(has && bg > 0.0) || level >= max_depth;
-        int flags = leaf ? 1 : 0;
-        o.feat = -1; o.kind = 0; o.bin_thr = 0;
-        o.mask[0] = o.mask[1] = o.mask[2] = o.mask[3] = 0;
-        if (!leaf) {
-            o.feat = subset[(int64_t)s * m + sh_best_j]; o.kind = sh_best_kind == 0 ? 0 : 1; o.bin_thr = sh_best_s;
-            for (int q = 0; q < 4; ++q) o.mask[q] = sh_best_mask[q];
-            double lc = 0.0, rc = 0.0, gl = 1.0, gr = 1.0;
-            for (int k = 0; k < C; ++k) { lc += (double)bestL[k]; rc += (double)(tot[k] - bestL[k]); }
-            if (lc == 0.0) gl = 0.0; else for (int k = 0; k < C; ++k) { const double fq = (double)bestL[k] / lc; gl -= fq * fq; }
-            if (rc == 0.0) gr = 0.0; else for (int k = 0; k < C; ++k) { const double fq = (double)(tot[k] - bestL[k]) / rc; gr -= fq * fq; }
-            if (level + 1 == max_depth || gl == 0.0) flags |= 2;
-            if (level + 1 == max_depth || gr == 0.0) flags |= 4;
-        }
-        o.flags = flags;
-        split[s] = o;
-    }
+    write_counts(tid, kScoreThreads, s, has, bestL, tot, C, node_counts, left_counts, right_counts);
+    if (tid == 0)
+        write_split(s, has, sh_best_gain, parent_imp, has ? subset[(int64_t)s * m + sh_best_j] : -1, sh_best_kind, sh_best_s, sh_best_mask,
+                    bestL, tot, C, level, max_depth, split);
+}
+
+constexpr int kScoreWarpsMax = 8;
+constexpr size_t kScoreWarpAutoBytes = 24 * 1024;
+
+__host__ __device__ inline size_t score_warp_bytes(int m, int n_bins, int C) {
+    const size_t nbC = (size_t)n_bins * C;
+    size_t b = ((size_t)m * nbC * 4 + 15) & ~(size_t)15;
+    b += (size_t)n_bins * 8 + nbC * 4 + (size_t)m * n_bins * 4 + (size_t)C * 8 + (size_t)m * 12 + (size_t)m * n_bins;
+    return (b + 15) & ~(size_t)15;
+}
+
+__global__ void __launch_bounds__(kScoreWarpsMax * 32) score_level_warp_kernel(
+    uint32_t* hist, int n_slots, const uint16_t* __restrict__ subset, int m, int n_bins, int C,
+    const int32_t* __restrict__ feat_bins, const int32_t* __restrict__ feat_kind, int level, int max_depth, int min_inst,
+    double min_gain, int zero_hist, b200flow_split* split, uint32_t* node_counts, uint32_t* left_counts, uint32_t* right_counts) {
+    extern __shared__ __align__(16) uint8_t sm_raw[];
+    const int lane = lane_id();
+    const int s = blockIdx.x * (blockDim.x >> 5) + warp_id();
+    if (s >= n_slots) return;
+    const int nbC = n_bins * C, words = m * nbC;
+    uint8_t* base = sm_raw + score_warp_bytes(m, n_bins, C) * warp_id();
+    uint32_t* cum_all = (uint32_t*)base;
+    double* cen = (double*)(base + (((size_t)words * 4 + 15) & ~(size_t)15));
+    uint32_t* raw = (uint32_t*)(cen + n_bins);
+    int* order_all = (int*)(raw + nbC);
+    uint32_t* tot = (uint32_t*)(order_all + (size_t)m * n_bins);
+    uint32_t* bestL = tot + C;
+    int* ncand = (int*)(bestL + C);
+    int* kinds = ncand + m;
+    int* nbs = kinds + m;
+    uint8_t* cand_all = (uint8_t*)(nbs + m);
+
+    uint32_t* src = hist + (int64_t)s * words;
+    const int vec = (words & 3) == 0 ? 4 : ((words & 1) == 0 ? 2 : 1);
+    if (vec == 4) for (int i = lane * 4; i < words; i += 128) cp_async16(cum_all + i, src + i);
+    else if (vec == 2) for (int i = lane * 2; i < words; i += 64) cp_async8(cum_all + i, src + i);
+    else for (int i = lane; i < words; i += 32) cp_async4(cum_all + i, src + i);
+    cp_async_commit();
+    for (int j = lane; j < m; j += 32) { const int f = subset[(int64_t)s * m + j]; kinds[j] = feat_kind[f]; nbs[j] = feat_bins[f]; }
+    cp_async_wait_all();
+    __syncwarp();
+    if (zero_hist) {
+        if (vec == 4) for (int i = lane * 4; i < words; i += 128) *(uint4*)(src + i) = make_uint4(0u, 0u, 0u, 0u);
+        else if (vec == 2) for (int i = lane * 2; i < words; i += 64) *(uint2*)(src + i) = make_uint2(0u, 0u);
+        else for (int i = lane; i < words; i += 32) src[i] = 0u;
+    }
+    for (int jj = 0; jj < m; ++jj) {
+        const int nb = nbs[jj], kind = kinds[jj];
+        uint32_t* cum = cum_all + (size_t)jj * nbC;
+        const int n_cand = feature_candidates(cum, order_all + (size_t)jj * n_bins, cand_all + (size_t)jj * n_bins, cen, raw, nb, kind, C);
+        if (jj == 0) feature_totals(cum, nb, kind, C, tot);
+        if (lane == 0) ncand[jj] = n_cand;
+    }
+    __syncwarp();
+    double pi = 0.0;
+    if (lane == 0) { double ptot = 0.0; for (int k = 0; k < C; ++k) ptot += (double)tot[k]; pi = gini_u32(tot, C, ptot); }
+    const double parent_imp = __shfl_sync(0xffffffffu, pi, 0);
+    double g = -DBL_MAX; int bj = -1, bs = -1;
+    eval_candidates(lane, 32, m, ncand, kinds, nbs, cand_all, cum_all, n_bins, nbC, tot, C, parent_imp, min_inst, min_gain, 0, g, bj, bs);
+    warp_argmax(g, bj, bs);
+    const bool has = bj >= 0;
+    if (lane == 0) {
+        unsigned long long mask[4] = {0, 0, 0, 0};
+        if (has) split_left(cum_all + (size_t)bj * nbC, order_all + (size_t)bj * n_bins, kinds[bj], nbs[bj], bs, C, bestL, mask);
+        write_split(s, has, g, parent_imp, has ? subset[(int64_t)s * m + bj] : -1, has ? kinds[bj] : 0, bs, mask, bestL, tot, C,
+                    level, max_depth, split);
+    }
+    __syncwarp();
+    write_counts(lane, 32, s, has, bestL, tot, C, node_counts, left_counts, right_counts);
 }
 
 constexpr int kGrowBlock = 256;
@@ -355,13 +520,15 @@
     }
 }
 
+template <bool REG>
 __global__ void __launch_bounds__(kGrowBlock) grow_write_kernel(
     int n_slots, const int32_t* __restrict__ slot_tree, const uint32_t* __restrict__ slot_nid,
     const int32_t* __restrict__ slot_node, const b200flow_split* __restrict__ split,
     const uint32_t* __restrict__ node_counts, const uint32_t* __restrict__ left_counts,
     const uint32_t* __restrict__ right_counts, int C, b200flow_node* nodes, uint64_t* node_mask, uint32_t* pool_counts,
     int32_t* node_tree, const int32_t* __restrict__ blk, const int64_t* __restrict__ counters, int32_t* next_tree,
-    uint32_t* next_nid, int32_t* next_node, int32_t* next_parent, int32_t* child_slot) {
+    uint32_t* next_nid, int32_t* next_node, int32_t* next_parent, int32_t* child_slot, uint64_t seed, int F, int m,
+    uint16_t* next_subset) {
     __shared__ int sh[33];
     if (counters[2]) return;
     const int s = blockIdx.x * kGrowBlock + threadIdx.x;
@@ -392,8 +559,15 @@
             pool_counts[(child + 1) * C + k] = right_counts[(int64_t)s * C + k];
         }
         int64_t ns = (int64_t)blk[2 * blockIdx.x + 1] + e1;
-        if (!(sp.flags & 2)) { next_tree[ns] = tree; next_nid[ns] = nid * 2u; next_node[ns] = (int32_t)child; next_parent[ns] = s * 2; csl = (int)ns; ++ns; }
-        if (!(sp.flags & 4)) { next_tree[ns] = tree; next_nid[ns] = nid * 2u + 1; next_node[ns] = (int32_t)child + 1; next_parent[ns] = s * 2 + 1; csr = (int)ns; }
+        if (!(sp.flags & 2)) {
+            next_tree[ns] = tree; next_nid[ns] = nid * 2u; next_node[ns] = (int32_t)child; next_parent[ns] = s * 2; csl = (int)ns;
+            if (next_subset) draw_feature_subset<REG>(seed, tree, nid * 2u, F, m, next_subset + ns * m);
+            ++ns;
+        }
+        if (!(sp.flags & 4)) {
+            next_tree[ns] = tree; next_nid[ns] = nid * 2u + 1; next_node[ns] = (int32_t)child + 1; next_parent[ns] = s * 2 + 1; csr = (int)ns;
+            if (next_subset) draw_feature_subset<REG>(seed, tree, nid * 2u + 1, F, m, next_subset + ns * m);
+        }
     }
     if (child_slot) { child_slot[2 * s] = csl; child_slot[2 * s + 1] = csr; }
     nodes[node] = nd;
@@ -853,7 +1027,10 @@
     B2F_REQUIRE(slot_tree && slot_nid && subset && F > 0 && F < 65536 && m > 0 && m <= F, "feature_subsets: bad arguments");
     B2F_REQUIRE(m == F || m <= kMaxSubset, "feature_subsets: subset size %d > %d not supported", m, kMaxSubset);
     if (n_slots <= 0) return B200FLOW_OK;
-    feature_subsets_kernel<<<(n_slots + 127) / 128, 128, 0, (cudaStream_t)stream>>>(seed, n_slots, slot_tree, slot_nid, F, m, subset);
+    if (m <= kRegSubset || m >= F)
+        feature_subsets_kernel<true><<<(n_slots + 127) / 128, 128, 0, (cudaStream_t)stream>>>(seed, n_slots, slot_tree, slot_nid, F, m, subset);
+    else
+        feature_subsets_kernel<false><<<(n_slots + 127) / 128, 128, 0, (cudaStream_t)stream>>>(seed, n_slots, slot_tree, slot_nid, F, m, subset);
     return check_launch("feature_subsets");
 }
 
@@ -878,13 +1055,53 @@
     return check_launch("hist_level");
 }
 
-extern "C" int b200flow_score_level(const uint32_t* hist, int32_t n_slots, const uint16_t* subset, int32_t m, int32_t n_bins,
+constexpr int kScoreWarpMinWaves = 4;
+static int score_warp_cfg(int m, int n_bins, int C, int n_slots, size_t* smem) {
+    const char* e = getenv("B200FLOW_SCORE_VARIANT");
+    const bool force_cta = e && !strcmp(e, "cta"), force_warp = e && !strcmp(e, "warp");
+    if (force_cta) return 0;
+    const size_t pw = score_warp_bytes(m, n_bins, C);
+    if (!force_warp && pw > kScoreWarpAutoBytes) return 0;
+    int best = 0, best_warps = 0;
+    for (int nw = kScoreWarpsMax; nw >= 1; nw >>= 1) {
+        if (pw * nw > 227 * 1024) continue;
+        const int ctas = (int)((228 * 1024) / (pw * nw + 1024));
+        const int warps = ctas * nw > 64 ? 64 : ctas * nw;
+        if (warps > best_warps) { best_warps = warps; best = nw; }
+    }
+    if (best == 0) return force_warp ? -1 : 0;
+    if (!force_warp && n_slots >= 0 && n_slots < kScoreWarpMinWaves * kNumSMs * best_warps) return 0;
+    *smem = pw * best;
+    return best;
+}
+
+extern "C" int b200flow_score_level_variant(int32_t m, int32_t n_bins, int32_t C) {
+    size_t smem = 0;
+    if (m <= 0 || n_bins <= 0 || C <= 0) return 0;
+    return score_warp_cfg(m, n_bins, C, -1, &smem) > 0 ? 1 : 0;
+}
+
+extern "C" int b200flow_score_level(uint32_t* hist, int32_t n_slots, const uint16_t* subset, int32_t m, int32_t n_bins,
                                     int32_t C, const int32_t* feat_bins, const int32_t* feat_kind, int32_t level, int32_t max_depth,
                                     int32_t min_instances, double min_info_gain, b200flow_split* split, uint32_t* node_counts,
-                                    uint32_t* left_counts, uint32_t* right_counts, void* stream) {
+                                    uint32_t* left_counts, uint32_t* right_counts, int32_t flags, void* stream) {
     B2F_REQUIRE(hist && subset && feat_bins && feat_kind && split && node_counts && left_counts && right_counts, "score_level: null pointer");
     B2F_REQUIRE(m > 0 && n_bins > 0 && n_bins <= 256 && C > 0 && C <= 256, "score_level: bad shape");
+    B2F_REQUIRE(((uintptr_t)hist & 15) == 0, "score_level: hist must be 16-byte aligned");
     if (n_slots <= 0) return B200FLOW_OK;
+    const int zero_hist = (flags & B200FLOW_SCORE_ZERO_HIST) ? 1 : 0;
+    size_t wsmem = 0;
+    const int nw = score_warp_cfg(m, n_bins, C, n_slots, &wsmem);
+    B2F_REQUIRE(nw >= 0, "score_level: B200FLOW_SCORE_VARIANT=warp, but one slot's scratch (%zu B) exceeds shared memory",
+                score_warp_bytes(m, n_bins, C));
+    if (nw > 0) {
+        cudaError_t e = cudaFuncSetAttribute(score_level_warp_kernel, cudaFuncAttributeMaxDynamicSharedMemorySize, (int)wsmem);
+        if (e != cudaSuccess) { set_error("score_level: %s", cudaGetErrorString(e)); return B200FLOW_ERR_CUDA; }
+        score_level_warp_kernel<<<(n_slots + nw - 1) / nw, nw * 32, wsmem, (cudaStream_t)stream>>>(
+            hist, n_slots, subset, m, n_bins, C, feat_bins, feat_kind, level, max_depth, min_instances, min_info_gain, zero_hist, split,
+            node_counts, left_counts, right_counts);
+        return check_launch("score_level");
+    }
     const size_t per_feat = (size_t)n_bins * C * 4 + (size_t)n_bins * 4 + (size_t)n_bins;
     const size_t per_warp = ((size_t)n_bins * 8 + (size_t)n_bins * C * 4 + 7) & ~(size_t)7;
     const size_t fixed = (size_t)2 * C * 4 + 16 + per_warp * (kScoreThreads / 32) + 16;
@@ -895,8 +1112,8 @@
     cudaError_t e = cudaFuncSetAttribute(score_level_kernel, cudaFuncAttributeMaxDynamicSharedMemorySize, (int)smem);
     if (e != cudaSuccess) { set_error("score_level: %s", cudaGetErrorString(e)); return B200FLOW_ERR_CUDA; }
     score_level_kernel<<<n_slots, kScoreThreads, smem, (cudaStream_t)stream>>>(hist, n_slots, subset, m, n_bins, C, feat_bins, feat_kind, level,
-                                                                              max_depth, min_instances, min_info_gain, batch, split,
-                                                                              node_counts, left_counts, right_counts);
+                                                                              max_depth, min_instances, min_info_gain, batch, zero_hist,
+                                                                              split, node_counts, left_counts, right_counts);
     return check_launch("score_level");
 }
 
@@ -905,17 +1122,20 @@
                                    const uint32_t* right_counts, int32_t C, b200flow_node* nodes, uint64_t* node_mask,
                                    uint32_t* pool_counts, int32_t* node_tree, int64_t pool_capacity, int32_t* next_tree,
                                    uint32_t* next_nid, int32_t* next_node, int32_t* next_parent, int32_t* child_slot,
-                                   int64_t* counters, void* stream) {
+                                   int64_t* counters, uint64_t seed, int32_t F, int32_t m, uint16_t* next_subset, void* stream) {
     B2F_REQUIRE(slot_tree && slot_nid && slot_node && split && node_counts && left_counts && right_counts && nodes && pool_counts &&
                     node_tree && next_tree && next_nid && next_node && next_parent && counters, "grow_level: null pointer");
+    B2F_REQUIRE(!next_subset || (F > 0 && F < 65536 && m > 0 && m <= F && (m == F || m <= kMaxSubset)),
+                "grow_level: bad feature subset shape (F %d, m %d)", F, m);
     if (n_slots <= 0) return B200FLOW_OK;
     const int nb = (n_slots + kGrowBlock - 1) / kGrowBlock;
     int32_t* blk = (int32_t*)(counters + 8);
     grow_count_kernel<<<nb, kGrowBlock, 0, (cudaStream_t)stream>>>(n_slots, split, blk);
     grow_scan_kernel<<<1, 1024, 0, (cudaStream_t)stream>>>(nb, blk, counters, pool_capacity);
-    grow_write_kernel<<<nb, kGrowBlock, 0, (cudaStream_t)stream>>>(n_slots, slot_tree, slot_nid, slot_node, split, node_counts, left_counts,
-                                                                  right_counts, C, nodes, node_mask, pool_counts, node_tree, blk, counters,
-                                                                  next_tree, next_nid, next_node, next_parent, child_slot);
+    auto* write = (!next_subset || m <= kRegSubset || m >= F) ? grow_write_kernel<true> : grow_write_kernel<false>;
+    write<<<nb, kGrowBlock, 0, (cudaStream_t)stream>>>(n_slots, slot_tree, slot_nid, slot_node, split, node_counts, left_counts, right_counts,
+                                                      C, nodes, node_mask, pool_counts, node_tree, blk, counters, next_tree, next_nid,
+                                                      next_node, next_parent, child_slot, seed, F, m, next_subset);
     return check_launch("grow_level");
 }
 
```

After: 158.7 million, median of 6. 1.01x the previous value.
